# paulmillr/noble-bls12-381

Measured on AMD Instinct MI355X. Metric: pairings/sec, higher is better.
Workload: dtype int64; 1 GPU; batch of 4096 independent BLS12-381 pairings per GPU (Miller loop + final exponentiation, inputs pre-validated, bit-exact vs reference), inputs/outputs resident in HBM; batch_per_gpu=4096, batches_in_flight=12

## Files before the change

include/nbls.h:

```cpp
#ifndef NBLS_H
#define NBLS_H
#include <stddef.h>
#include <stdint.h>
#ifdef __cplusplus
extern "C" {
#endif

typedef struct nbls_ctx nbls_ctx;

#define NBLS_OK 0
#define NBLS_EINVAL (-1)
#define NBLS_EHIP (-2)
#define NBLS_ENOSUP (-3)
#define NBLS_ENOGPU (-4)
#define NBLS_EDECODE (-5)

int nbls_init(int device_id, nbls_ctx** out);
void nbls_destroy(nbls_ctx* ctx);
const char* nbls_strerror(int code);
int nbls_last_hip_error(nbls_ctx* ctx);

int nbls_pairing_batch(nbls_ctx* ctx, size_t n, const uint8_t* g1_aff, const uint8_t* g2_aff, int with_final_exp, int validate,
                       uint8_t* out_fp12, int8_t* status);
int nbls_pairing_batch_dev(nbls_ctx* ctx, size_t n, const void* d_g1_aff, const void* d_g2_aff, int with_final_exp,
// ... 184 lines not shown
typedef struct nbls_kzg_fk20 nbls_kzg_fk20;
int  nbls_kzg_fk20_create(nbls_ctx* ctx, const nbls_kzg_monomial* monomial, unsigned log2_cell, nbls_kzg_fk20** out);
void nbls_kzg_fk20_destroy(nbls_kzg_fk20* fk);
int  nbls_kzg_fk20_params(const nbls_kzg_fk20* fk, unsigned* log2_n, unsigned* log2_cell);
int  nbls_kzg_compute_cells_and_proofs_fk20(nbls_ctx* ctx, const nbls_kzg_fk20* fk, size_t n, const uint8_t* blobs, uint8_t* out_cells,
                                            uint8_t* out_proofs48 , int8_t* status );
int  nbls_kzg_recover_cells_and_proofs_fk20(nbls_ctx* ctx, const nbls_kzg_fk20* fk, size_t n, const uint32_t* cell_offsets, const uint32_t* cell_index, const uint8_t* cells,
                                            uint8_t* out_cells, uint8_t* out_proofs48 , int8_t* status );

#define NBLS_ST_G16_C 30
typedef struct nbls_groth16_vk nbls_groth16_vk;
int  nbls_groth16_vk_create(nbls_ctx* ctx, size_t m, const uint8_t* alpha_g1_48, const uint8_t* beta_g2_96, const uint8_t* gamma_g2_96, const uint8_t* delta_g2_96,
                            const uint8_t* ic48 , int8_t* status , nbls_groth16_vk** out);
void nbls_groth16_vk_destroy(nbls_groth16_vk* vk);
int  nbls_groth16_vk_inputs(const nbls_groth16_vk* vk, size_t* m);
int  nbls_groth16_verify(nbls_ctx* ctx, const nbls_groth16_vk* vk, size_t n, const uint8_t* proofs192, const uint8_t* inputs32 , const uint8_t* seed32 ,
                         int* all_ok, int8_t* status );
int  nbls_groth16_prepare_inputs(nbls_ctx* ctx, const nbls_groth16_vk* vk, size_t n, const uint8_t* inputs32, uint8_t* out48 , int8_t* status );
int  nbls_groth16_input_sums(nbls_ctx* ctx, size_t n, size_t m, const uint8_t* inputs32, const uint8_t* weights32 , const int8_t* pre ,
                             uint8_t* out32 , int8_t* status );

int nbls_verify_batch_partial_dev(nbls_ctx* ctx, size_t n, const void* d_sig96 , const void* d_uniform256, const void* d_pk48,
                                  void* d_out_fp12, int* zero_flag, int8_t* pk_status , void* stream);

int nbls_miller_product_partial(nbls_ctx* ctx, size_t n, const uint8_t* g1_aff, const uint8_t* g2_aff, int validate, void** d_partial, int8_t* status);
int nbls_verify_batch_partial(nbls_ctx* ctx, size_t n, const uint8_t* sig96 , const uint8_t* msgs, const uint32_t* offsets, const uint8_t* pk48,
                              const uint8_t* dst, size_t dst_len, void** d_partial, int* zero_flag, int8_t* pk_status );
int nbls_miller_product_partial_into(nbls_ctx* ctx, size_t n, const uint8_t* g1_aff, const uint8_t* g2_aff, int validate, void* d_dst576, int8_t* status);
int nbls_verify_batch_partial_into(nbls_ctx* ctx, size_t n, const uint8_t* sig96 , const uint8_t* msgs, const uint32_t* offsets, const uint8_t* pk48,
                                   const uint8_t* dst, size_t dst_len, void* d_dst576, int* zero_flag, int8_t* pk_status );
const char* nbls_config_describe(void);
#define NBLS_ABI_VERSION 5
int nbls_abi_version(void);
int nbls_context_device(nbls_ctx* ctx);

int nbls_hw_queues(int* set_by_library);
typedef struct nbls_pool nbls_pool;
int nbls_pool_init(int device_id, int depth , nbls_pool** out);
void nbls_pool_destroy(nbls_pool* p);
int nbls_pool_depth(const nbls_pool* p);
nbls_ctx* nbls_pool_context(nbls_pool* p, int i);
int nbls_pool_next_slot(nbls_pool* p);
int nbls_pool_pairing_batch_dev(nbls_pool* p, size_t n, const void* d_g1, const void* d_g2, int with_final_exp, void* d_out, int* slot);
int nbls_pool_synchronize(nbls_pool* p);

typedef struct nbls_multi nbls_multi;
int nbls_init_multi(int n_devices, const int* device_ids, nbls_multi** out);
void nbls_destroy_multi(nbls_multi* m);
int nbls_multi_device_count(const nbls_multi* m);
nbls_ctx* nbls_multi_context(nbls_multi* m, int i);
int nbls_multi_peer_access(const nbls_multi* m, int i);
int nbls_multi_pairing_batch(nbls_multi* m, size_t n, const uint8_t* g1_aff, const uint8_t* g2_aff, int with_final_exp, int validate,
                             uint8_t* out_fp12, int8_t* status);
int nbls_multi_miller_product(nbls_multi* m, size_t n, const uint8_t* g1_aff, const uint8_t* g2_aff, int final_exp, int validate,
                              uint8_t* out_fp12, int8_t* status);
int nbls_multi_verify_batch(nbls_multi* m, size_t n, const uint8_t* sig96, const uint8_t* msgs, const uint32_t* offsets, const uint8_t* pk48,
                            const uint8_t* dst, size_t dst_len, int* ok);

int nbls_program_stats(nbls_ctx* ctx, int prog, uint32_t* out8);
int nbls_device_synchronize(nbls_ctx* ctx);
int nbls_placement_probe(nbls_ctx* ctx, size_t n, uint64_t* out_blocks);
int nbls_field_kernel_raw(nbls_ctx* ctx, int kind, int form, size_t n, const uint8_t* in_raw, uint8_t* out_raw);
#define NBLS_N_PROGRAMS 128
#define NBLS_TUNE_SPLIT_MILLER_MIN 1
#define NBLS_TUNE_HALVES_MIN 2
#define NBLS_TUNE_EXPC_MIN 3
#define NBLS_TUNE_CHAIN_MAX 4
#define NBLS_TUNE_VERIFY_CHUNKS 5
#define NBLS_TUNE_VERIFY_LAST_PCT 6
#define NBLS_TUNE_VERIFY_PIPE_MIN 7
#define NBLS_TUNE_SAC_MAX 8
#define NBLS_TUNE_PT_LS2_MAX 9
#define NBLS_TUNE_WIDE_MAX 10
#define NBLS_TUNE_H2C_NORM_MIN 11
#define NBLS_TUNE_INV_WIDE_MAX 12
#define NBLS_TUNE_LS_MAX 13
#define NBLS_TUNE_LS2_MAX 14
#define NBLS_TUNE_POLY_SLAB 15
#define NBLS_TUNE_MSMB_WINDOW 16
#define NBLS_TUNE_MSMB_BIG 17
#define NBLS_TUNE_MSMB_SLAB 18
#define NBLS_TUNE_CELLS_CHUNK 20
#define NBLS_TUNE_G16_CHUNK 22
int nbls_set_tuning(nbls_ctx* ctx, int key, long long value);
int nbls_program_count(void);
const char* nbls_program_name(int prog);
const char* nbls_program_kernel(nbls_ctx* ctx, int prog);
const char* nbls_extra_program_kernel(nbls_ctx* ctx, const char* name);
long long nbls_extra_program_launches(nbls_ctx* ctx, const char* name);
int nbls_aot_kernel_private_bytes(int k);
int nbls_timing_enable(nbls_ctx* ctx, int on);
int nbls_timing_read(nbls_ctx* ctx, float* ms , uint32_t* counts );

#ifdef __cplusplus
}
#endif
#endif
```

noble-bls12-381_amd/csrc/aot.h:

```cpp
#pragma once
#include <string>
#include <vector>
#include "vm.h"
#include "programs.h"

#define NBLS_AOT_PARTS 8
#define NBLS_AOT_KERNELS(X)                                                  \
  X(0, expx, P_EXPX, P_FE_MID1, P_FE_MID2, P_COUNT)                          \
  X(0, acc_fe, P_ACC_FE, P_ACC_RAW, P_ACC_BYTES, P_COUNT)                    \
  X(0, lines_pq, P_LINES_PQ, P_COUNT, P_COUNT, P_COUNT)                      \
  X(0, acc4_raw, P_ACC4_RAW, P_ACC8_RAW, P_ACC2_RAW, P_COUNT)                \
  X(1, fe_easy, P_FE_EASY, P_COUNT, P_COUNT, P_COUNT)                        \
  X(1, fe_final, P_FE_FINAL, P_COUNT, P_COUNT, P_COUNT)                      \
  X(1, miller_fe, P_MILLER_FE, P_MILLER_RAW, P_MILLER_BYTES, P_COUNT)        \
  X(1, mul2, P_MUL2, P_MUL2S, P_COUNT, P_COUNT)                             \
  X(1, norm, P_NORM_RAW, P_NORM_BYTES, P_RAW_TO_BYTES, P_COUNT)              \
  X(2, h2c_a, P_H2C_A, P_COUNT, P_COUNT, P_COUNT)                            \
  X(2, h2c_b, P_H2C_B1, P_H2C_B2, P_COUNT, P_COUNT)                          \
  X(2, h2c_c1, P_H2C_C1, P_H2C_C0, P_COUNT, P_COUNT)                         \
  X(2, h2c_c2, P_H2C_C2, P_COUNT, P_COUNT, P_COUNT)                          \
  X(2, g1_dec, P_G1_DEC_A, P_G1_DEC_B, P_COUNT, P_COUNT)                     \
  X(2, g2_dec, P_G2_DEC_A, P_G2_DEC_B, P_COUNT, P_COUNT)                     \
  X(2, g2_to_affine, P_G2_TO_AFFINE, P_G2_NORM, P_G2_TO_PROJ, P_G2_ADD2)     \
  X(3, g2_mul, P_G2_MUL, P_G2_MUL_W3, P_G2_MUL_GLS, P_G2_MUL_SAC)         \
  X(3, g1_mul, P_G1_MUL, P_G1_MUL_W3, P_G1_MUL_FIXED, P_G1_MUL64)               \
  X(4, g1_validate, P_G1_VALIDATE, P_COUNT, P_COUNT, P_COUNT)                \
  X(4, g2_validate, P_G2_VALIDATE, P_COUNT, P_COUNT, P_COUNT)                \
  X(4, g1_sum, P_G1_TO_PROJ, P_G1_ADD2, P_G1_NORM, P_G1_TO_AFFINE)           \
  X(5, g1_msm, P_G1_ADD_AB, P_G1_HORNER, P_G1_SHIFTADD, P_G1_MSM_PREP)       \
  X(5, g2_msm, P_G2_ADD_AB, P_G2_HORNER, P_G2_SHIFTADD, P_G2_MSM_PREP)       \
  X(6, lines_q, P_LINES_Q, P_ACC_Q, P_LINES_BYTES, P_LINES_FROM_BYTES)       \
  X(6, miller_raw2, P_MILLER_RAW2, P_COUNT, P_COUNT, P_COUNT)                \
  X(6, g2_dec192, P_G2_DEC_A192, P_G2_DEC_B192, P_G2_DEC_B_HEX, P_G2_SWAP)   \
  X(6, from_raw, P_G1_FROM_RAW, P_G2_FROM_RAW, P_G1_COMPRESS, P_G2_COMPRESS) \
  X(7, h2c1, P_H2C1_A, P_H2C1_B, P_ENC1_A, P_ENC1_B)                         \
  X(7, g1_clear, P_G1_CLEAR, P_COUNT, P_COUNT, P_COUNT)                      \
  X(7, enc2, P_ENC2_A, P_ENC2_B, P_COUNT, P_COUNT)                            \
  X(4, h2c_n, P_H2C_NA, P_H2C_NM, P_H2C_NB, P_COUNT)

#define NBLS_AOT_LS_KERNELS(X)                                                              \
  X(7, expx_ls, P_EXPX_LS, P_COUNT, P_COUNT, P_COUNT)                                      \
  X(3, miller_ls, P_MILLER_FE_LS, P_MILLER_RAW_LS, P_MILLER_BYTES_LS, P_COUNT)

#define NBLS_AOT_LS2_KERNELS(X)                                                             \
  X(4, expx_ls2, P_EXPX_LS2, P_COUNT, P_COUNT, P_COUNT)                                    \
  X(5, miller_ls2, P_MILLER_FE_LS2, P_MILLER_RAW_LS2, P_MILLER_BYTES_LS2, P_COUNT)                    \
  X(6, g2pt_ls2, P_H2C_C1_LS2, P_H2C_C2_LS2, P_G2_MUL_SAC_LS2, P_COUNT)

#define NBLS_AOT_EXTRA_KERNELS(X)                \
  X(1, poly_g1, XP_POLY_G1_16, XP_POLY_G1_256)  \
  X(7, poly_g2, XP_POLY_G2_16, XP_POLY_G2_256)  \
  X(2, dbladd_g1, XP_DBLADD_G1, XP_COUNT)       \
  X(3, dbladd_g2, XP_DBLADD_G2, XP_COUNT)       \
  X(5, lines_fe, XP_LINES_FE, XP_COUNT)

namespace nbls {

static const uint32_t AF_MULTSH = 1;
static const uint32_t AF_MULT3 = 2;
static const uint32_t AF_OFFS = 4;
static const uint32_t AF_WRED = 8;
static const uint32_t AF_HALVE = 16;
struct AotSig { uint32_t kind, p0, flags, t, sh0, sh1; };
static inline bool operator==(const AotSig& a, const AotSig& b) { return a.kind == b.kind && a.p0 == b.p0 && a.flags == b.flags && a.t == b.t && a.sh0 == b.sh0 && a.sh1 == b.sh1; }
struct AotStep { uint32_t x, y; };
static const int AOT_DOT_HDR = 2;
static inline uint32_t aot_dot_hdr_quads(uint32_t t) { return (AOT_DOT_HDR + t + 3) / 4; }
struct AotProgram {
  std::vector<AotSig> sigs;
  std::vector<uint32_t> sig_count;
  std::vector<AotStep> steps;
  std::vector<uint32_t> descs;
  uint32_t lds_bytes = 0;
};
static const int AOT_MAX_SEGS = 8;
struct AotSeg {
  const AotStep* steps; const uint32_t* descs; const uint32_t* consts;
  uint32_t nsteps, nconst, inst_bytes, slot_bytes, shared_consts, pad;
  IOBuf bufs[MAX_BUFS];
};
struct AotArgs {
  AotSeg seg[AOT_MAX_SEGS];
  uint32_t nseg, W, G, n_items, fair, pad;
  const uint32_t* qp_table; const uint32_t* item_index; const uint32_t* n_items_dev;
};
struct AotLayout;
std::string aot_translate(const Program& p, AotProgram& out);
std::string aot_translate_with(const Program& p, AotProgram& out, const AotLayout* layout);

}

// ... 7 lines not shown
```

noble-bls12-381_amd/csrc/aot_gen.cpp:

```cpp
#include <algorithm>
#include <cstdio>
#include <cstdlib>
#include <string>
#include <vector>
#include "aot.h"
#include "aot_layout.h"
#include "config.h"
using namespace nbls;
namespace nbls { const AotLayoutEntry* aot_layout_table(size_t* n) { *n = 0; return nullptr; } }

static int gen_layout(const char* path, long iters, const std::vector<std::string>& only) {
  FILE* f = fopen(path, "w");
  if (!f) { perror(path); return 1; }
  fprintf(f, "// aot_layout.inc -- GENERATED by `aot_gen --layout` (make -C csrc layout; aot_layout.cpp: search over per-instance slot permutations against the LDS bank model); do not edit.\n");
  fprintf(f, "// AOT_LAYOUT_POS(program, place of slot s of instance g at [g * slots + s]) ; AOT_LAYOUT_ROW(program, instances, slots, steps, hash of the compiled program)\n");
  const ProgId hot[] = {P_EXPX, P_FE_MID1, P_FE_MID2, P_ACC_FE, P_ACC_RAW, P_ACC_BYTES, P_LINES_PQ, P_ACC4_RAW, P_ACC8_RAW, P_ACC2_RAW, P_FE_EASY, P_FE_FINAL, P_MILLER_FE, P_MILLER_RAW, P_MILLER_BYTES,
                        P_MUL2, P_MUL2S, P_NORM_RAW, P_NORM_BYTES, P_LINES_Q, P_ACC_Q, P_MILLER_RAW2,
                        P_H2C_A, P_H2C_B1, P_H2C_B2, P_H2C_C0, P_H2C_C1, P_H2C_C2, P_G1_DEC_B, P_G2_DEC_B, P_G1_VALIDATE, P_G2_VALIDATE, P_G2_TO_AFFINE};
  auto place = [&](const Program& p) {
    if (!only.empty() && std::find(only.begin(), only.end(), p.name) == only.end()) return;
    if (!p.shared_consts || p.slots < 2) return;
    const AotLdsCost c0 = aot_layout_cost(p, AotLayout());
    if (c0.cycles == c0.floor) return;
    const long n = std::max<long>(iters / 2, std::min<long>(iters, iters * 1000 / (long)(c0.floor / 14 + 1)));
    const AotLayout l = aot_layout_search(p, n, 0x6e626c73u);
    if (l.empty()) return;
    const AotLdsCost c1 = aot_layout_cost(p, l);
    fprintf(f, "// %s: %u instances x %u slots of %u B; LDS read cycles per wavefront %lu -> %lu (conflicts %.3f -> %.3f of them), %ld swaps tried\n", p.name.c_str(), p.G, p.slots, p.slot_bytes, c0.cycles, c1.cycles,
            (double)(c0.cycles - c0.floor) / c0.cycles, (double)(c1.cycles - c1.floor) / c1.cycles, n);
    fprintf(f, "AOT_LAYOUT_POS(%s", p.name.c_str());
    for (uint32_t g = 0; g < p.G; g++) for (uint32_t s = 0; s < p.slots; s++) fprintf(f, ", %u", (unsigned)l.pos[g][s]);
    fprintf(f, ")\nAOT_LAYOUT_ROW(%s, %u, %u, %zu, 0x%08xu)\n", p.name.c_str(), p.G, p.slots, p.steps.size(), aot_program_hash(p));
    fflush(f);
  };
  for (ProgId id : hot) place(get_program(id));
  place(get_extra_program(XP_LINES_FE));
  fclose(f);
  return 0;
}
static int gen_hist() {
  auto emit = [&](const char* kernel, const std::vector<const Program*>& progs) {
    std::vector<AotSig> sigs; std::vector<std::vector<unsigned>> cnt(progs.size());
    for (size_t q = 0; q < progs.size(); q++) {
      AotProgram ap;
      if (!aot_translate(*progs[q], ap).empty()) continue;
      for (size_t i = 0; i < ap.sigs.size(); i++) {
        size_t k = 0; while (k < sigs.size() && !(sigs[k] == ap.sigs[i])) k++;
        if (k == sigs.size()) sigs.push_back(ap.sigs[i]);
        cnt[q].resize(std::max(cnt[q].size(), k + 1), 0); cnt[q][k] += ap.sig_count[i];
      }
    }
    for (size_t q = 0; q < progs.size(); q++) {
      printf("%s %s %u %zu", kernel, progs[q]->name.c_str(), progs[q]->G, progs[q]->steps.size());
      for (size_t k = 0; k < sigs.size(); k++) printf(" %u", k < cnt[q].size() ? cnt[q][k] : 0u);
      printf("\n");
    }
  };
#define HIST(PART, NAME, P0, P1, P2, P3) { std::vector<const Program*> progs; for (ProgId id : {P0, P1, P2, P3}) if (id != P_COUNT) progs.push_back(&get_program(id)); emit(#NAME, progs); }
  NBLS_AOT_KERNELS(HIST)
#undef HIST
#define HIST(PART, NAME, E0, E1) { std::vector<const Program*> progs; for (ExtraProg id : {E0, E1}) if (id != XP_COUNT) progs.push_back(&get_extra_program(id)); emit(#NAME, progs); }
  NBLS_AOT_EXTRA_KERNELS(HIST)
#undef HIST
  return 0;
}
int main(int argc, char** argv) {
  if (argc > 2 && std::string(argv[1]) == "--layout") return gen_layout(argv[2], argc > 3 ? atol(argv[3]) : 60000, std::vector<std::string>(argv + std::min(argc, 4), argv + argc));
  if (argc > 1 && std::string(argv[1]) == "--hist") return gen_hist();
  const char* path = argc > 1 ? argv[1] : "aot_sigs.inc";
  FILE* f = fopen(path, "w");
  if (!f) { perror(path); return 1; }
  fprintf(f, "// aot_sigs.inc -- GENERATED by aot_gen (aot_gen.cpp) from the compiled step programs; do not edit.\n");
  fprintf(f, "// X(id, kind, p0, flags, t, shape[0], shape[1], steps with this signature) -- aot.h AotSig: K_DOT (12): p0 product rounds, flags AF_*, t merged post-added terms;\n");
  fprintf(f, "// K_LIN (2): p0 added, t subtracted terms; K_LOAD (0) / K_STORE (3) / K_LOADW (4) / K_STOREW (5)\n");
  int rc = 0;
  auto emit = [&](const char* kernel, const std::vector<const Program*>& progs) {
    std::vector<AotSig> sigs; std::vector<unsigned> cnt; std::string names; size_t nsteps = 0, kb = 0;
    for (const Program* pp : progs) {
      const Program& p = *pp;
      AotProgram ap;
      const std::string e = aot_translate(p, ap);
      if (!e.empty()) { fprintf(stderr, "aot_gen: %s\n", e.c_str()); rc = 1; }
      for (size_t i = 0; i < ap.sigs.size(); i++) {
        size_t k = 0; while (k < sigs.size() && !(sigs[k] == ap.sigs[i])) k++;
        if (k == sigs.size()) { sigs.push_back(ap.sigs[i]); cnt.push_back(0); }
        cnt[k] += ap.sig_count[i];
      }
      names += (names.empty() ? "" : " + ") + p.name; nsteps += p.steps.size(); kb += ap.descs.size() * 4 / 1024;
    }
    fprintf(f, "// %s: %zu steps, %zu signatures, %zu KB of descriptors\n#define AOT_SIGS_%s(X)", names.c_str(), nsteps, sigs.size(), kb, kernel);
    for (size_t k = 0; k < sigs.size(); k++)
      fprintf(f, " \\\n  X(%zu, %u, %u, 0x%02x, %u, 0x%08xu, 0x%08xu, %u)", k, sigs[k].kind, sigs[k].p0, sigs[k].flags, sigs[k].t, sigs[k].sh0, sigs[k].sh1, cnt[k]);
    fprintf(f, "\n");
  };
#define GEN(PART, NAME, P0, P1, P2, P3)                                                            \
  {                                                                                                \
    std::vector<const Program*> progs;                                                             \
    for (ProgId id : {P0, P1, P2, P3}) if (id != P_COUNT) progs.push_back(&get_program(id));       \
    emit(#NAME, progs);                                                                            \
  }
  NBLS_AOT_KERNELS(GEN)
  NBLS_AOT_LS_KERNELS(GEN)
  NBLS_AOT_LS2_KERNELS(GEN)
#undef GEN
#define GEN(PART, NAME, E0, E1)                                                                    \
  {                                                                                                \
    std::vector<const Program*> progs;                                                             \
    for (ExtraProg id : {E0, E1}) if (id != XP_COUNT) progs.push_back(&get_extra_program(id));     \
    emit(#NAME, progs);                                                                            \
  }
  NBLS_AOT_EXTRA_KERNELS(GEN)
#undef GEN
  fclose(f);
  std::string ppath = path; { size_t k = ppath.rfind("aot_sigs.inc"); if (k != std::string::npos) ppath.replace(k, 12, "aot_parts.inc"); else ppath += ".parts"; }
  f = fopen(ppath.c_str(), "w");
  if (!f) { perror(ppath.c_str()); return 1; }
  fprintf(f, "// aot_parts.inc -- GENERATED by aot_gen from NBLS_AOT_KERNELS (aot.h); do not edit.\n");
  for (int part = 0; part < NBLS_AOT_PARTS; part++) {
    fprintf(f, "#if NBLS_AOT_PART == %d\n", part);
#define PARTS(PART, NAME, P0, P1, P2, P3) if (PART == part) fprintf(f, "AOT_KERNEL_BODY(%s)\n", #NAME);
    NBLS_AOT_KERNELS(PARTS)
#undef PARTS
#define PARTS(PART, NAME, P0, P1, P2, P3) if (PART == part) fprintf(f, "AOT_KERNEL_BODY_LS(%s)\n", #NAME);
    NBLS_AOT_LS_KERNELS(PARTS)
#undef PARTS
#define PARTS(PART, NAME, P0, P1, P2, P3) if (PART == part) fprintf(f, "AOT_KERNEL_BODY_LS2(%s)\n", #NAME);
    NBLS_AOT_LS2_KERNELS(PARTS)
#undef PARTS
#define PARTS(PART, NAME, E0, E1) if (PART == part) fprintf(f, "AOT_KERNEL_BODY(%s)\n", #NAME);
    NBLS_AOT_EXTRA_KERNELS(PARTS)
#undef PARTS
    fprintf(f, "#endif\n");
  }
  fclose(f);
  return rc;
}
```

noble-bls12-381_amd/csrc/aot_kernel.hip:

```cpp
#include <hip/hip_runtime.h>
#include <atomic>
#include <mutex>
#include "aot.h"
#include "aot_exec.h"
#include "aot_sigs.inc"

namespace nbls {

struct DevDesc {
  V4 q0, q1, q2;
  const V4* blk;
  __device__ __forceinline__ V4 quad(const u32 i) const { return i == 0 ? q0 : i == 1 ? q1 : i == 2 ? q2 : blk[64 * i]; }
};

__device__ __forceinline__ u32 aot_lane() {
  u32 l;
  asm volatile("v_mbcnt_lo_u32_b32 %0, -1, 0\n\tv_mbcnt_hi_u32_b32 %0, -1, %0" : "=v"(l));
  return l;
}
template <class Dispatch>
__device__ __forceinline__ void aot_body(const AotArgs& ka, Dispatch&& dispatch) {
  extern __shared__ __attribute__((aligned(16))) char smem[];
  char* lds = smem;
  const u32 lane = threadIdx.x;
// ... 49 lines not shown
#define NBLS_AOT_PART 0
#endif
#define AOT_DECL(PART, NAME, P0, P1, P2, P3) extern "C" __global__ void nbls_aot_##NAME(AotArgs ka);
NBLS_AOT_KERNELS(AOT_DECL)
NBLS_AOT_LS_KERNELS(AOT_DECL)
NBLS_AOT_LS2_KERNELS(AOT_DECL)
#define AOT_DECL_EXTRA(PART, NAME, E0, E1) extern "C" __global__ void nbls_aot_##NAME(AotArgs ka);
NBLS_AOT_EXTRA_KERNELS(AOT_DECL_EXTRA)
#define AOT_KERNEL_BODY(NAME) AOT_KERNEL_BODY_(NAME, AOT_CASE, NBLS_AOT_OCC)
#define AOT_KERNEL_BODY_LS(NAME) AOT_KERNEL_BODY_(NAME, AOT_CASE_LS, __attribute__((amdgpu_waves_per_eu(1, 2))))
#define AOT_KERNEL_BODY_LS2(NAME) AOT_KERNEL_BODY_(NAME, AOT_CASE_LS2, __attribute__((amdgpu_waves_per_eu(1, 2))))
#define AOT_KERNEL_BODY_(NAME, CASE, OCC)                                                                                                 \
  extern "C" __global__ void __launch_bounds__(64) OCC nbls_aot_##NAME(AotArgs ka) {                                           \
    aot_body(ka, [&](u32 sig, const DevDesc& d, char* lds, u32 item, bool live, const IOBuf* bufs) __attribute__((always_inline)) { \
      switch (sig) { AOT_SIGS_##NAME(CASE) default: break; }                                                                   \
    });                                                                                                                        \
  }
#include "aot_parts.inc"

#define AOT_ROW(ID, KIND, P0, FLAGS, T, SH0, SH1, CNT) {KIND, P0, FLAGS, T, SH0, SH1},
}

#if NBLS_AOT_PART == 0
namespace nbls {
#define AOT_TABLE(PART, NAME, P0, P1, P2, P3) static const AotSig sigs_##NAME[] = {AOT_SIGS_##NAME(AOT_ROW)};
NBLS_AOT_KERNELS(AOT_TABLE)
NBLS_AOT_LS_KERNELS(AOT_TABLE)
NBLS_AOT_LS2_KERNELS(AOT_TABLE)
#define AOT_TABLE_EXTRA(PART, NAME, E0, E1) static const AotSig sigs_##NAME[] = {AOT_SIGS_##NAME(AOT_ROW)};
NBLS_AOT_EXTRA_KERNELS(AOT_TABLE_EXTRA)
struct AotKernel { int prog_id[4]; const void* fn; const AotSig* sigs; unsigned nsigs; const char* name; };
#define AOT_ENTRY(PART, NAME, P0, P1, P2, P3) {{(int)P0, (int)P1, (int)P2, (int)P3}, (const void*)nbls_aot_##NAME, sigs_##NAME, (unsigned)(sizeof(sigs_##NAME) / sizeof(AotSig)), "nbls_aot_" #NAME},
#define AOT_XP(E) ((int)E == (int)XP_COUNT ? (int)P_COUNT : (int)P_COUNT + 1 + (int)E)
#define AOT_ENTRY_EXTRA(PART, NAME, E0, E1) {{AOT_XP(E0), AOT_XP(E1), (int)P_COUNT, (int)P_COUNT}, (const void*)nbls_aot_##NAME, sigs_##NAME, (unsigned)(sizeof(sigs_##NAME) / sizeof(AotSig)), "nbls_aot_" #NAME},
static const AotKernel g_kernels[] = {NBLS_AOT_KERNELS(AOT_ENTRY) NBLS_AOT_LS_KERNELS(AOT_ENTRY) NBLS_AOT_LS2_KERNELS(AOT_ENTRY) NBLS_AOT_EXTRA_KERNELS(AOT_ENTRY_EXTRA)};
static const int g_nkernels = (int)(sizeof(g_kernels) / sizeof(g_kernels[0]));

}

extern "C" int nbls_aot_index(int prog_id) {
  if (prog_id < 0 || prog_id >= (int)nbls::P_COUNT) return -1;
  for (int k = 0; k < nbls::g_nkernels; k++) for (int j = 0; j < 4; j++) if (nbls::g_kernels[k].prog_id[j] == prog_id) return k;
  return -1;
}
extern "C" int nbls_aot_extra_index(int extra_prog) {
  if (extra_prog < 0 || extra_prog >= (int)nbls::XP_COUNT) return -1;
  for (int k = 0; k < nbls::g_nkernels; k++) for (int j = 0; j < 4; j++) if (nbls::g_kernels[k].prog_id[j] == (int)nbls::P_COUNT + 1 + extra_prog) return k;
  return -1;
}
extern "C" int nbls_aot_private_bytes(int k) {
  if (k < 0 || k >= nbls::g_nkernels) return -1;
  hipFuncAttributes a;
  if (hipFuncGetAttributes(&a, nbls::g_kernels[k].fn) != hipSuccess) { (void)hipGetLastError(); return -2; }
  return (int)a.localSizeBytes;
}
extern "C" const char* nbls_aot_name(int k) { return k >= 0 && k < nbls::g_nkernels ? nbls::g_kernels[k].name : nullptr; }
extern "C" int nbls_aot_bind(int k, nbls::AotProgram* ap) {
  using namespace nbls;
  if (k < 0 || k >= g_nkernels || !ap) return -1;
  const AotKernel& K = g_kernels[k];
  std::vector<unsigned> map(ap->sigs.size());
  for (size_t i = 0; i < ap->sigs.size(); i++) {
    unsigned id = 0;
    while (id < K.nsigs && !(K.sigs[id] == ap->sigs[i])) id++;
    if (id == K.nsigs) return -1;
    map[i] = id;
  }
  for (auto& s : ap->steps) s.x = (s.x & ~0xffu) | map[s.x & 0xffu];
  return 0;
}
extern "C" int nbls_aot_launch(int k, const nbls::AotArgs* ka, unsigned lds_bytes, void* stream) {
  using namespace nbls;
  if (k < 0 || k >= g_nkernels) return -1;
  if (ka->n_items == 0) return 0;
  const unsigned blocks = (ka->n_items + ka->G - 1) / ka->G;
  static std::atomic<bool> attr_set[64];
  static std::mutex attr_mu;
  {
    int dev = 0;
    if (hipGetDevice(&dev) != hipSuccess || dev < 0 || dev >= 64) dev = 0;
    if (!attr_set[dev].load(std::memory_order_acquire)) {
      std::lock_guard<std::mutex> g(attr_mu);
      if (!attr_set[dev].load(std::memory_order_relaxed)) {
        for (int i = 0; i < g_nkernels; i++) (void)hipFuncSetAttribute(g_kernels[i].fn, hipFuncAttributeMaxDynamicSharedMemorySize, 160 * 1024);
        attr_set[dev].store(true, std::memory_order_release);
      }
    }
  }
  AotArgs a = *ka;
  a.fair = (blocks > 1024 && blocks <= 4096) ? 1u : 0u;
  void* args[] = {&a};
  const hipError_t e = hipLaunchKernel(g_kernels[k].fn, dim3(blocks), dim3(64), args, lds_bytes, (hipStream_t)stream);
  return e == hipSuccess ? (int)hipGetLastError() : (int)e;
}
#endif
```

noble-bls12-381_amd/csrc/aot_layout.inc:

```
AOT_LAYOUT_POS(expx, 10, 17, 29, 4, 3, 14, 6, 19, 5, 12, 11, 18, 24, 7, 9, 16, 26, 23, 22, 21, 0, 28, 1, 13, 8, 27, 2, 25, 15, 20, 1, 13, 26, 25, 17, 10, 23, 18, 9, 15, 3, 24, 29, 4, 22, 6, 21, 19, 2, 12, 0, 11, 7, 16, 8, 27, 14, 20, 28, 5, 24, 12, 6, 3, 8, 21, 16, 17, 4, 9, 18, 14, 1, 0, 10, 19, 22, 13, 27, 29, 23, 28, 26, 15, 25, 7, 5, 2, 11, 20, 29, 0, 5, 4, 11, 22, 24, 7, 12, 14, 9, 10, 23, 19, 2, 1, 13, 16, 8, 6, 15, 25, 18, 27, 17, 20, 28, 26, 21, 3, 16, 14, 25, 10, 19, 5, 22, 3, 18, 15, 20, 27, 11, 23, 13, 12, 0, 6, 24, 28, 2, 9, 21, 7, 4, 26, 1, 17, 8, 29)
AOT_LAYOUT_ROW(expx, 5, 30, 97, 0x7173e202u)
AOT_LAYOUT_POS(fe_mid1, 12, 24, 3, 26, 35, 6, 15, 9, 22, 31, 25, 16, 20, 17, 8, 5, 29, 7, 34, 14, 28, 23, 2, 33, 10, 27, 1, 19, 18, 0, 13, 21, 30, 11, 32, 4, 2, 23, 32, 30, 24, 17, 29, 6, 1, 12, 11, 19, 7, 14, 21, 10, 0, 22, 28, 13, 25, 20, 16, 3, 31, 33, 8, 26, 34, 27, 35, 15, 9, 4, 18, 5, 6, 4, 26, 13, 9, 31, 12, 14, 23, 28, 22, 17, 2, 35, 27, 24, 19, 33, 25, 16, 3, 34, 1, 20, 30, 8, 11, 21, 0, 5, 32, 10, 15, 29, 7, 18, 6, 2, 14, 4, 28, 21, 13, 10, 26, 23, 9, 32, 20, 25, 19, 0, 18, 30, 16, 31, 8, 12, 35, 29, 33, 27, 7, 22, 24, 5, 1, 11, 15, 3, 34, 17, 8, 17, 26, 27, 23, 34, 32, 0, 13, 7, 31, 33, 9, 22, 21, 15, 25, 3, 11, 6, 5, 29, 4, 2, 16, 10, 14, 19, 35, 12, 18, 28, 20, 30, 1, 24)
AOT_LAYOUT_ROW(fe_mid1, 5, 36, 11, 0x4d52c8d6u)
AOT_LAYOUT_POS(fe_mid2, 4, 2, 3, 13, 10, 7, 9, 11, 24, 26, 25, 21, 1, 27, 20, 14, 19, 18, 8, 32, 29, 6, 16, 35, 31, 22, 30, 12, 28, 33, 23, 5, 0, 34, 15, 17, 11, 29, 17, 4, 21, 12, 10, 34, 3, 32, 35, 14, 2, 0, 27, 25, 20, 28, 6, 23, 8, 26, 19, 5, 15, 16, 31, 1, 9, 30, 7, 24, 33, 13, 22, 18, 11, 33, 22, 3, 8, 13, 24, 12, 9, 15, 2, 28, 20, 34, 5, 31, 18, 25, 17, 26, 6, 7, 1, 32, 23, 21, 16, 10, 19, 27, 0, 14, 30, 35, 29, 4, 5, 27, 22, 0, 25, 23, 4, 2, 3, 34, 10, 20, 35, 33, 12, 26, 28, 7, 16, 19, 17, 32, 24, 15, 11, 29, 31, 13, 30, 8, 6, 1, 21, 18, 14, 9, 31, 2, 19, 21, 12, 20, 9, 7, 4, 25, 17, 10, 5, 14, 30, 16, 22, 13, 11, 0, 26, 6, 34, 29, 3, 18, 33, 8, 35, 15, 1, 28, 23, 32, 24, 27)
AOT_LAYOUT_ROW(fe_mid2, 5, 36, 11, 0x62a97a64u)
AOT_LAYOUT_POS(acc_fe, 22, 8, 3, 10, 20, 15, 0, 13, 18, 12, 14, 11, 9, 2, 16, 19, 7, 6, 5, 4, 1, 21, 23, 17, 18, 22, 15, 9, 17, 11, 20, 10, 5, 8, 0, 12, 14, 13, 3, 7, 2, 16, 19, 1, 4, 21, 6, 23, 0, 3, 8, 15, 11, 17, 23, 21, 5, 7, 6, 9, 4, 13, 12, 14, 1, 20, 2, 22, 16, 18, 10, 19, 16, 2, 18, 4, 11, 17, 6, 23, 10, 12, 9, 3, 8, 13, 14, 15, 0, 21, 19, 5, 20, 7, 22, 1, 12, 20, 11, 0, 18, 21, 6, 7, 9, 14, 13, 19, 2, 17, 3, 15, 10, 16, 5, 1, 22, 23, 4, 8)
AOT_LAYOUT_ROW(acc_fe, 5, 24, 173, 0xd36919acu)
AOT_LAYOUT_POS(acc_raw, 10, 1, 4, 13, 3, 22, 20, 21, 5, 12, 8, 0, 17, 7, 16, 2, 11, 6, 14, 9, 19, 18, 23, 15, 7, 1, 23, 6, 3, 0, 8, 21, 15, 9, 10, 22, 11, 13, 14, 16, 18, 17, 20, 19, 12, 2, 4, 5, 19, 18, 5, 10, 17, 2, 12, 7, 9, 20, 22, 23, 11, 4, 14, 13, 3, 15, 16, 1, 6, 8, 0, 21, 0, 21, 5, 9, 20, 8, 6, 1, 10, 14, 23, 4, 13, 17, 12, 15, 16, 3, 2, 11, 19, 7, 22, 18, 20, 11, 16, 8, 5, 10, 22, 15, 7, 14, 3, 21, 12, 0, 6, 19, 1, 2, 17, 18, 4, 9, 23, 13)
AOT_LAYOUT_ROW(acc_raw, 5, 24, 166, 0xd41b21c8u)
AOT_LAYOUT_POS(acc_bytes, 10, 1, 4, 13, 3, 22, 20, 21, 5, 12, 8, 0, 17, 7, 16, 2, 11, 6, 14, 9, 19, 18, 23, 15, 7, 1, 23, 6, 3, 0, 8, 21, 15, 9, 10, 22, 11, 13, 14, 16, 18, 17, 20, 19, 12, 2, 4, 5, 19, 18, 5, 10, 17, 2, 12, 7, 9, 20, 22, 23, 11, 4, 14, 13, 3, 15, 16, 1, 6, 8, 0, 21, 0, 21, 5, 9, 20, 8, 6, 1, 10, 14, 23, 4, 13, 17, 12, 15, 16, 3, 2, 11, 19, 7, 22, 18, 20, 11, 16, 8, 5, 10, 22, 15, 7, 14, 3, 21, 12, 0, 6, 19, 1, 2, 17, 18, 4, 9, 23, 13)
AOT_LAYOUT_ROW(acc_bytes, 5, 24, 167, 0x04619a33u)
AOT_LAYOUT_POS(lines_pq, 16, 2, 17, 24, 8, 14, 22, 6, 11, 9, 10, 23, 5, 21, 19, 3, 25, 0, 20, 18, 13, 1, 15, 12, 7, 4, 16, 15, 13, 3, 14, 23, 11, 2, 0, 25, 8, 17, 20, 10, 19, 4, 21, 1, 12, 5, 9, 18, 6, 7, 22, 24, 16, 1, 20, 8, 4, 25, 6, 9, 3, 11, 5, 12, 24, 23, 13, 2, 14, 19, 15, 0, 10, 21, 18, 17, 7, 22, 13, 22, 21, 10, 24, 5, 18, 9, 8, 20, 16, 19, 15, 25, 14, 2, 12, 1, 7, 3, 23, 0, 6, 4, 11, 17, 2, 17, 6, 16, 0, 10, 19, 7, 23, 25, 21, 11, 20, 13, 22, 14, 12, 1, 24, 4, 3, 5, 8, 9, 18, 15, 3, 20, 21, 0, 22, 15, 19, 6, 5, 17, 10, 16, 12, 25, 11, 13, 23, 18, 9, 1, 14, 24, 7, 8, 2, 4)
AOT_LAYOUT_ROW(lines_pq, 6, 26, 307, 0x7c311802u)
AOT_LAYOUT_POS(acc4_raw, 23, 0, 18, 10, 27, 6, 8, 11, 22, 25, 5, 19, 4, 16, 14, 28, 13, 15, 9, 2, 20, 7, 1, 21, 17, 26, 24, 29, 3, 12, 16, 24, 5, 18, 3, 11, 7, 14, 2, 25, 28, 13, 19, 12, 1, 20, 10, 9, 17, 0, 8, 21, 15, 6, 23, 29, 27, 4, 22, 26, 13, 17, 2, 6, 4, 19, 7, 22, 8, 28, 11, 14, 9, 15, 23, 29, 10, 5, 16, 25, 1, 12, 24, 21, 18, 20, 0, 26, 27, 3, 1, 7, 16, 10, 14, 9, 5, 28, 25, 6, 0, 27, 19, 29, 17, 12, 22, 2, 26, 21, 4, 24, 15, 3, 13, 23, 11, 20, 8, 18, 29, 12, 7, 1, 5, 15, 10, 6, 21, 13, 18, 2, 16, 25, 4, 22, 26, 0, 9, 19, 24, 20, 14, 8, 27, 28, 3, 17, 23, 11)
AOT_LAYOUT_ROW(acc4_raw, 5, 30, 472, 0xa9d029e3u)
AOT_LAYOUT_POS(acc8_raw, 1, 13, 4, 12, 0, 5, 22, 11, 8, 21, 16, 10, 15, 17, 14, 23, 2, 3, 9, 6, 19, 18, 20, 7, 20, 17, 1, 3, 4, 7, 22, 0, 15, 2, 14, 9, 12, 13, 5, 18, 11, 10, 21, 23, 19, 6, 16, 8, 10, 19, 13, 14, 18, 20, 21, 23, 3, 0, 2, 6, 16, 9, 12, 8, 22, 17, 7, 4, 1, 5, 15, 11, 19, 16, 6, 14, 9, 1, 5, 7, 18, 4, 23, 2, 11, 12, 10, 15, 13, 8, 0, 3, 17, 21, 22, 20, 19, 18, 9, 7, 4, 21, 6, 14, 20, 5, 8, 10, 11, 13, 16, 15, 17, 2, 0, 3, 12, 22, 23, 1)
AOT_LAYOUT_ROW(acc8_raw, 5, 24, 879, 0x655d1f0bu)
AOT_LAYOUT_POS(acc2_raw, 10, 1, 2, 12, 4, 11, 6, 14, 23, 13, 20, 3, 7, 5, 17, 0, 19, 21, 18, 15, 8, 16, 22, 9, 5, 0, 16, 23, 17, 4, 8, 7, 11, 1, 22, 15, 12, 14, 10, 2, 3, 9, 6, 20, 18, 21, 13, 19, 4, 18, 17, 0, 13, 23, 5, 19, 21, 22, 10, 11, 12, 15, 9, 8, 14, 2, 1, 3, 20, 6, 16, 7, 22, 21, 18, 17, 11, 9, 16, 23, 7, 0, 10, 4, 3, 12, 13, 15, 20, 2, 8, 1, 5, 6, 14, 19, 9, 20, 7, 12, 11, 21, 6, 16, 13, 14, 4, 3, 22, 0, 18, 10, 19, 1, 5, 15, 23, 8, 2, 17)
AOT_LAYOUT_ROW(acc2_raw, 5, 24, 267, 0xb30cd74du)
AOT_LAYOUT_POS(fe_easy, 10, 1, 36, 18, 38, 37, 12, 6, 29, 40, 9, 14, 24, 25, 33, 8, 11, 20, 22, 39, 2, 35, 15, 23, 3, 16, 41, 19, 21, 0, 26, 4, 5, 28, 30, 27, 13, 32, 31, 17, 34, 7, 5, 2, 31, 33, 6, 17, 32, 26, 25, 15, 10, 39, 12, 37, 23, 8, 13, 38, 29, 14, 0, 20, 9, 11, 27, 1, 22, 30, 16, 40, 3, 35, 34, 24, 19, 21, 41, 36, 7, 4, 18, 28, 19, 32, 35, 33, 10, 40, 15, 29, 25, 6, 24, 5, 1, 37, 8, 18, 7, 17, 41, 23, 22, 14, 11, 39, 31, 20, 36, 27, 12, 9, 26, 2, 16, 13, 34, 3, 28, 4, 38, 0, 21, 30, 31, 28, 10, 24, 34, 4, 27, 39, 32, 38, 3, 2, 20, 5, 40, 29, 1, 25, 21, 16, 30, 15, 19, 37, 41, 14, 8, 22, 0, 35, 33, 6, 12, 18, 11, 26, 9, 7, 23, 36, 13, 17)
AOT_LAYOUT_ROW(fe_easy, 4, 42, 24, 0x4d06dc2eu)
AOT_LAYOUT_POS(fe_final, 21, 38, 36, 13, 42, 16, 40, 22, 46, 14, 26, 7, 37, 8, 17, 18, 9, 28, 0, 10, 35, 33, 34, 15, 31, 4, 45, 24, 5, 19, 3, 39, 44, 25, 12, 29, 47, 41, 20, 27, 43, 11, 32, 1, 2, 6, 30, 23, 43, 23, 21, 26, 24, 31, 1, 33, 7, 39, 13, 12, 47, 29, 46, 15, 40, 10, 6, 44, 16, 14, 11, 9, 2, 18, 36, 34, 3, 45, 41, 4, 17, 37, 22, 38, 32, 27, 5, 30, 8, 25, 42, 28, 19, 20, 35, 0, 6, 5, 38, 8, 11, 22, 3, 23, 16, 24, 44, 21, 14, 27, 15, 12, 7, 47, 43, 25, 10, 4, 32, 30, 36, 31, 42, 9, 0, 26, 18, 13, 1, 34, 19, 40, 33, 20, 2, 17, 41, 46, 37, 35, 28, 29, 45, 39, 33, 8, 21, 41, 14, 45, 38, 2, 13, 39, 6, 4, 43, 5, 10, 9, 12, 22, 46, 15, 28, 47, 34, 36, 26, 0, 11, 31, 19, 35, 17, 24, 29, 40, 32, 18, 44, 23, 1, 25, 3, 16, 7, 20, 27, 42, 30, 37, 44, 31, 11, 35, 7, 12, 4, 17, 15, 30, 13, 47, 0, 26, 36, 34, 45, 29, 16, 8, 21, 14, 33, 39, 43, 18, 24, 46, 37, 42, 28, 3, 1, 9, 41, 23, 27, 2, 6, 32, 40, 22, 5, 25, 10, 19, 38, 20)
AOT_LAYOUT_ROW(fe_final, 5, 48, 59, 0x73c61872u)
AOT_LAYOUT_POS(miller_fe, 32, 33, 19, 8, 7, 37, 5, 29, 24, 6, 14, 22, 4, 16, 36, 27, 26, 25, 0, 23, 20, 2, 28, 13, 3, 12, 34, 11, 9, 30, 1, 31, 18, 10, 17, 35, 15, 21, 12, 37, 16, 30, 17, 6, 33, 11, 14, 9, 29, 25, 34, 32, 2, 23, 3, 20, 28, 1, 18, 19, 15, 5, 24, 31, 26, 7, 36, 13, 21, 27, 10, 35, 4, 8, 0, 22, 32, 6, 18, 19, 27, 37, 17, 10, 12, 13, 20, 24, 28, 8, 4, 30, 23, 35, 22, 11, 0, 1, 16, 36, 25, 2, 29, 26, 31, 15, 33, 9, 5, 14, 7, 3, 34, 21, 25, 3, 30, 37, 21, 34, 5, 29, 8, 12, 10, 15, 24, 31, 28, 6, 36, 17, 19, 20, 0, 9, 7, 4, 16, 23, 26, 14, 27, 11, 18, 32, 33, 22, 13, 1, 35, 2)
AOT_LAYOUT_ROW(miller_fe, 4, 38, 349, 0xd1b982e6u)
AOT_LAYOUT_POS(miller_raw, 32, 27, 36, 26, 7, 28, 23, 18, 2, 19, 25, 24, 16, 33, 30, 4, 21, 10, 37, 35, 0, 31, 9, 11, 12, 8, 1, 14, 29, 6, 34, 15, 3, 5, 13, 22, 20, 17, 11, 0, 3, 31, 17, 34, 18, 23, 7, 35, 21, 9, 30, 29, 14, 8, 16, 32, 27, 1, 36, 13, 6, 24, 19, 22, 26, 15, 28, 37, 33, 2, 4, 25, 12, 20, 10, 5, 28, 34, 16, 33, 27, 0, 3, 24, 30, 22, 18, 19, 26, 4, 10, 14, 13, 25, 5, 11, 17, 36, 6, 2, 1, 32, 20, 8, 7, 15, 31, 37, 21, 29, 23, 35, 9, 12, 32, 3, 36, 17, 5, 9, 37, 33, 20, 34, 10, 14, 8, 22, 35, 4, 15, 1, 30, 21, 19, 31, 26, 23, 29, 25, 16, 7, 6, 12, 2, 13, 0, 24, 18, 11, 27, 28)
AOT_LAYOUT_ROW(miller_raw, 4, 38, 342, 0x07887de8u)
AOT_LAYOUT_POS(miller_bytes, 26, 1, 6, 35, 7, 5, 36, 21, 34, 32, 37, 31, 28, 3, 33, 4, 29, 15, 25, 23, 16, 12, 22, 14, 8, 27, 10, 9, 20, 13, 2, 19, 11, 17, 18, 24, 0, 30, 26, 3, 18, 21, 1, 5, 33, 16, 14, 36, 19, 31, 11, 30, 22, 28, 8, 34, 32, 17, 20, 27, 35, 23, 25, 15, 10, 0, 12, 24, 2, 37, 29, 6, 13, 9, 4, 7, 1, 37, 25, 7, 11, 28, 3, 22, 29, 9, 24, 35, 32, 13, 26, 34, 15, 17, 4, 27, 20, 16, 8, 5, 36, 18, 0, 6, 14, 31, 23, 12, 10, 19, 30, 33, 2, 21, 10, 34, 20, 14, 5, 28, 37, 24, 8, 2, 35, 16, 17, 4, 15, 33, 27, 32, 22, 21, 31, 13, 3, 9, 6, 25, 29, 11, 7, 1, 12, 30, 18, 26, 23, 0, 19, 36)
AOT_LAYOUT_ROW(miller_bytes, 4, 38, 343, 0x27bc5877u)
AOT_LAYOUT_POS(fp12_mul2, 2, 25, 30, 6, 28, 10, 11, 29, 32, 5, 35, 12, 16, 21, 4, 26, 0, 13, 22, 15, 18, 14, 9, 33, 27, 1, 7, 24, 34, 19, 3, 20, 8, 31, 17, 23, 7, 29, 20, 27, 14, 12, 23, 15, 18, 0, 19, 30, 3, 1, 6, 16, 25, 35, 31, 11, 8, 4, 13, 21, 10, 33, 5, 34, 24, 32, 28, 26, 2, 22, 17, 9, 35, 12, 15, 32, 7, 31, 19, 1, 30, 13, 25, 27, 9, 18, 0, 23, 24, 33, 29, 5, 10, 4, 22, 34, 6, 14, 2, 20, 11, 16, 17, 8, 3, 21, 28, 26, 15, 4, 32, 0, 8, 1, 31, 3, 7, 22, 30, 5, 11, 23, 35, 12, 13, 20, 33, 25, 24, 6, 26, 2, 17, 29, 34, 14, 28, 27, 16, 18, 9, 21, 10, 19)
AOT_LAYOUT_ROW(fp12_mul2, 4, 36, 9, 0x431cfebau)
AOT_LAYOUT_POS(fp12_mul2s, 2, 25, 30, 6, 28, 10, 11, 29, 32, 5, 35, 12, 16, 21, 4, 26, 0, 13, 22, 15, 18, 14, 9, 33, 27, 1, 7, 24, 34, 19, 3, 20, 8, 31, 17, 23, 7, 29, 20, 27, 14, 12, 23, 15, 18, 0, 19, 30, 3, 1, 6, 16, 25, 35, 31, 11, 8, 4, 13, 21, 10, 33, 5, 34, 24, 32, 28, 26, 2, 22, 17, 9, 35, 12, 15, 32, 7, 31, 19, 1, 30, 13, 25, 27, 9, 18, 0, 23, 24, 33, 29, 5, 10, 4, 22, 34, 6, 14, 2, 20, 11, 16, 17, 8, 3, 21, 28, 26, 15, 4, 32, 0, 8, 1, 31, 3, 7, 22, 30, 5, 11, 23, 35, 12, 13, 20, 33, 25, 24, 6, 26, 2, 17, 29, 34, 14, 28, 27, 16, 18, 9, 21, 10, 19)
AOT_LAYOUT_ROW(fp12_mul2s, 4, 36, 9, 0xf99001aau)
AOT_LAYOUT_POS(norm_raw, 6, 0, 5, 11, 8, 10, 1, 3, 9, 2, 7, 4, 7, 5, 11, 8, 10, 4, 9, 2, 3, 1, 0, 6, 2, 1, 10, 3, 0, 7, 11, 6, 9, 8, 4, 5, 10, 4, 0, 9, 5, 6, 3, 1, 2, 11, 8, 7)
AOT_LAYOUT_ROW(norm_raw, 4, 12, 8, 0x663d5f87u)
AOT_LAYOUT_POS(norm_bytes, 2, 9, 11, 1, 3, 8, 10, 0, 7, 5, 6, 4, 2, 8, 3, 4, 11, 9, 10, 5, 1, 7, 6, 0, 1, 10, 8, 11, 7, 2, 3, 9, 5, 0, 6, 4, 11, 3, 4, 0, 5, 9, 10, 2, 6, 1, 7, 8)
AOT_LAYOUT_ROW(norm_bytes, 4, 12, 10, 0x4c284411u)
AOT_LAYOUT_POS(lines_q, 17, 5, 6, 18, 15, 19, 16, 22, 3, 9, 13, 7, 1, 11, 23, 20, 2, 21, 4, 12, 8, 14, 10, 0, 16, 8, 11, 0, 10, 2, 23, 13, 3, 9, 20, 19, 17, 14, 1, 18, 6, 5, 22, 21, 12, 4, 7, 15, 2, 8, 1, 0, 22, 14, 7, 15, 10, 4, 20, 16, 18, 21, 11, 3, 17, 12, 9, 19, 23, 13, 5, 6, 6, 16, 17, 4, 20, 13, 22, 18, 8, 10, 23, 21, 7, 15, 12, 1, 14, 9, 19, 2, 5, 0, 11, 3, 16, 21, 8, 1, 14, 4, 6, 18, 19, 20, 10, 22, 0, 17, 9, 13, 7, 23, 15, 12, 11, 3, 2, 5, 0, 22, 21, 16, 15, 19, 8, 4, 17, 2, 10, 1, 3, 13, 14, 20, 6, 5, 11, 12, 7, 18, 23, 9)
AOT_LAYOUT_ROW(lines_q, 6, 24, 310, 0xc51c7bb5u)
AOT_LAYOUT_POS(acc_q, 5, 10, 26, 18, 8, 6, 14, 22, 11, 28, 2, 12, 15, 20, 17, 3, 9, 27, 16, 31, 7, 4, 25, 13, 23, 30, 21, 24, 1, 0, 29, 19, 26, 27, 0, 9, 4, 1, 29, 8, 5, 15, 25, 23, 11, 21, 24, 14, 18, 3, 12, 7, 28, 16, 19, 2, 10, 6, 13, 22, 31, 20, 17, 30, 2, 10, 24, 17, 0, 13, 3, 26, 4, 7, 1, 31, 12, 16, 6, 9, 29, 30, 20, 21, 15, 5, 14, 11, 25, 19, 27, 23, 28, 18, 22, 8, 26, 10, 29, 14, 20, 23, 18, 31, 22, 24, 28, 13, 11, 3, 8, 30, 15, 19, 17, 9, 12, 1, 4, 16, 5, 0, 7, 25, 27, 6, 2, 21, 10, 26, 12, 11, 8, 16, 1, 23, 25, 5, 20, 14, 30, 22, 9, 18, 28, 2, 27, 6, 29, 7, 21, 3, 31, 24, 0, 17, 4, 13, 19, 15)
AOT_LAYOUT_ROW(acc_q, 5, 32, 202, 0xff0ad85bu)
AOT_LAYOUT_POS(miller_raw2, 18, 29, 19, 48, 44, 31, 11, 7, 67, 3, 58, 60, 51, 56, 33, 2, 8, 66, 42, 9, 4, 23, 6, 43, 50, 39, 54, 49, 53, 45, 25, 59, 28, 5, 26, 14, 55, 41, 16, 27, 30, 65, 68, 17, 47, 52, 36, 38, 15, 61, 10, 63, 24, 0, 12, 62, 35, 20, 34, 57, 40, 21, 64, 13, 32, 1, 22, 46, 37, 66, 35, 22, 57, 42, 54, 60, 62, 26, 46, 28, 44, 2, 40, 18, 27, 36, 10, 39, 11, 64, 25, 8, 59, 0, 29, 16, 55, 67, 65, 31, 9, 38, 61, 24, 68, 37, 45, 33, 51, 19, 7, 21, 63, 15, 41, 4, 50, 53, 23, 56, 49, 48, 34, 1, 3, 58, 20, 14, 43, 32, 5, 12, 17, 13, 47, 52, 6, 30, 29, 54, 49, 58, 2, 17, 9, 61, 53, 25, 44, 59, 5, 68, 8, 19, 14, 31, 57, 30, 60, 11, 20, 24, 32, 56, 23, 34, 3, 55, 0, 10, 38, 43, 18, 63, 27, 51, 35, 48, 26, 41, 50, 6, 13, 45, 64, 15, 36, 33, 40, 47, 39, 4, 62, 7, 37, 52, 21, 28, 46, 65, 42, 67, 16, 12, 22, 66, 1, 35, 64, 28, 48, 18, 20, 52, 44, 16, 24, 58, 41, 56, 26, 42, 29, 4, 63, 13, 40, 21, 67, 6, 2, 9, 34, 43, 23, 57, 19, 66, 0, 32, 15, 36, 31, 27, 55, 7, 49, 12, 53, 22, 60, 61, 33, 50, 51, 10, 65, 14, 11, 45, 62, 8, 39, 38, 5, 37, 46, 54, 17, 3, 59, 25, 1, 30, 68, 47)
AOT_LAYOUT_ROW(miller_raw2, 4, 69, 536, 0x0a10926cu)
AOT_LAYOUT_POS(h2c_a, 23, 10, 21, 7, 8, 5, 14, 24, 1, 19, 27, 16, 3, 18, 6, 26, 15, 0, 12, 2, 17, 22, 20, 11, 4, 9, 13, 25, 1, 16, 12, 8, 13, 25, 18, 5, 6, 22, 24, 14, 9, 3, 15, 21, 20, 17, 0, 11, 7, 23, 10, 2, 27, 4, 19, 26, 19, 13, 26, 7, 12, 15, 1, 6, 0, 23, 2, 3, 11, 18, 17, 16, 22, 14, 27, 9, 20, 4, 21, 5, 25, 10, 8, 24, 22, 0, 4, 13, 9, 18, 5, 23, 6, 10, 17, 15, 3, 12, 7, 11, 1, 21, 27, 16, 19, 25, 26, 20, 8, 24, 14, 2, 27, 20, 12, 22, 16, 23, 13, 9, 25, 17, 1, 19, 15, 3, 11, 2, 26, 24, 14, 8, 4, 5, 21, 6, 7, 10, 0, 18, 16, 5, 21, 1, 20, 11, 4, 6, 10, 27, 12, 2, 19, 23, 0, 8, 3, 22, 24, 13, 7, 26, 18, 9, 15, 25, 14, 17, 15, 2, 10, 7, 14, 21, 18, 8, 13, 26, 1, 23, 9, 5, 19, 16, 0, 25, 11, 3, 20, 27, 17, 12, 6, 24, 4, 22, 5, 18, 9, 11, 8, 22, 20, 10, 6, 23, 2, 16, 13, 0, 14, 21, 15, 1, 7, 4, 19, 27, 26, 12, 3, 24, 25, 17)
AOT_LAYOUT_ROW(h2c_a, 8, 28, 24, 0x9b31d2b6u)
AOT_LAYOUT_POS(h2c_b1, 24, 3, 7, 2, 14, 21, 23, 0, 13, 11, 8, 4, 27, 15, 5, 18, 20, 1, 25, 26, 19, 12, 6, 17, 16, 22, 9, 10, 2, 5, 20, 1, 21, 9, 13, 25, 16, 22, 27, 15, 24, 12, 4, 10, 17, 8, 14, 0, 3, 23, 26, 18, 7, 11, 19, 6, 24, 23, 3, 6, 20, 7, 4, 2, 11, 13, 12, 17, 10, 21, 15, 27, 8, 19, 0, 26, 5, 25, 14, 16, 1, 9, 18, 22, 23, 4, 9, 12, 5, 27, 2, 3, 18, 26, 21, 17, 8, 22, 6, 1, 13, 19, 11, 25, 20, 24, 10, 0, 7, 15, 16, 14, 15, 24, 9, 23, 16, 7, 8, 3, 18, 14, 12, 13, 5, 1, 22, 19, 20, 25, 4, 2, 0, 21, 27, 10, 17, 11, 6, 26, 7, 12, 11, 8, 9, 13, 24, 15, 27, 3, 1, 17, 10, 2, 21, 22, 0, 25, 5, 14, 23, 19, 26, 20, 16, 6, 4, 18, 13, 1, 25, 6, 0, 14, 26, 24, 5, 18, 19, 10, 8, 23, 27, 20, 9, 12, 16, 4, 21, 3, 2, 17, 11, 15, 7, 22, 13, 26, 23, 6, 14, 21, 9, 5, 4, 1, 3, 15, 24, 0, 12, 22, 25, 27, 2, 16, 19, 7, 10, 11, 8, 17, 20, 18)
AOT_LAYOUT_ROW(h2c_b1, 8, 28, 50, 0x13589acbu)
AOT_LAYOUT_POS(h2c_b2, 2, 1, 6, 19, 8, 4, 7, 18, 15, 17, 14, 16, 10, 5, 9, 3, 0, 13, 11, 12, 2, 11, 4, 14, 16, 19, 10, 9, 17, 6, 0, 18, 3, 5, 7, 1, 13, 12, 8, 15, 9, 16, 3, 13, 5, 6, 7, 4, 19, 1, 10, 15, 18, 2, 12, 0, 11, 14, 17, 8, 5, 11, 0, 16, 19, 13, 1, 4, 17, 6, 3, 15, 7, 8, 18, 14, 12, 2, 10, 9, 13, 14, 12, 11, 1, 3, 17, 10, 18, 9, 6, 7, 4, 5, 2, 15, 8, 16, 19, 0, 1, 14, 18, 11, 15, 8, 6, 13, 7, 9, 4, 2, 5, 3, 12, 17, 19, 0, 10, 16, 1, 3, 12, 4, 10, 9, 7, 8, 17, 18, 19, 13, 6, 0, 14, 15, 2, 11, 16, 5, 1, 19, 17, 14, 18, 0, 7, 16, 15, 4, 8, 10, 6, 11, 3, 12, 5, 9, 13, 2)
AOT_LAYOUT_ROW(h2c_b2, 8, 20, 16, 0x42647d7fu)
AOT_LAYOUT_POS(h2c_c0, 20, 8, 18, 19, 22, 12, 4, 14, 13, 17, 1, 7, 5, 23, 9, 6, 10, 21, 16, 3, 2, 15, 0, 11, 17, 18, 21, 20, 19, 8, 22, 23, 11, 16, 13, 0, 2, 9, 5, 6, 1, 10, 3, 12, 15, 14, 4, 7, 19, 11, 3, 5, 9, 7, 13, 12, 17, 23, 15, 6, 8, 16, 10, 20, 22, 1, 18, 2, 14, 0, 21, 4, 6, 9, 4, 13, 12, 11, 17, 23, 22, 15, 3, 21, 0, 10, 16, 19, 8, 7, 5, 14, 2, 20, 1, 18, 1, 13, 9, 0, 12, 19, 11, 8, 15, 6, 17, 4, 16, 5, 7, 2, 3, 14, 20, 18, 22, 10, 23, 21, 16, 1, 13, 19, 3, 0, 2, 15, 9, 7, 21, 11, 22, 8, 4, 12, 14, 6, 5, 23, 18, 10, 17, 20, 3, 18, 16, 9, 17, 19, 5, 0, 7, 8, 4, 6, 21, 11, 2, 14, 20, 13, 22, 12, 10, 1, 15, 23, 10, 11, 3, 22, 18, 20, 9, 5, 21, 16, 19, 6, 2, 15, 13, 12, 4, 0, 23, 17, 14, 7, 1, 8)
AOT_LAYOUT_ROW(h2c_c0, 8, 24, 19, 0x8dd6efe9u)
AOT_LAYOUT_POS(h2c_c1, 5, 18, 17, 3, 6, 4, 1, 12, 8, 11, 7, 10, 16, 14, 9, 0, 19, 2, 15, 13, 11, 16, 19, 18, 0, 3, 8, 10, 14, 9, 17, 7, 5, 4, 13, 15, 2, 12, 1, 6, 8, 7, 16, 5, 4, 0, 3, 17, 13, 10, 14, 12, 2, 11, 15, 18, 1, 19, 6, 9, 14, 5, 18, 10, 17, 0, 6, 3, 7, 4, 8, 1, 15, 13, 2, 11, 12, 9, 16, 19, 5, 16, 15, 6, 18, 8, 19, 12, 1, 13, 14, 10, 7, 17, 3, 2, 9, 0, 4, 11, 12, 7, 4, 10, 5, 19, 16, 18, 15, 11, 9, 8, 0, 6, 17, 13, 2, 3, 1, 14, 11, 2, 5, 19, 16, 8, 13, 3, 10, 4, 0, 1, 9, 15, 18, 12, 7, 6, 14, 17, 6, 1, 2, 17, 12, 4, 14, 13, 8, 18, 11, 19, 10, 15, 0, 7, 16, 9, 3, 5)
AOT_LAYOUT_ROW(h2c_c1, 8, 20, 230, 0x09f22878u)
AOT_LAYOUT_POS(h2c_c2, 4, 12, 9, 3, 7, 13, 8, 1, 14, 19, 11, 10, 18, 2, 17, 16, 5, 0, 15, 6, 3, 19, 10, 8, 1, 13, 2, 14, 17, 6, 9, 11, 5, 16, 0, 7, 18, 15, 4, 12, 13, 1, 19, 9, 15, 0, 11, 8, 12, 17, 16, 6, 4, 5, 18, 14, 3, 2, 10, 7, 18, 10, 4, 14, 17, 2, 9, 3, 15, 0, 6, 12, 11, 7, 19, 5, 8, 13, 1, 16, 12, 1, 13, 2, 15, 5, 9, 6, 7, 4, 17, 10, 11, 3, 0, 8, 16, 14, 18, 19, 18, 14, 3, 11, 2, 13, 16, 17, 12, 9, 8, 6, 10, 0, 15, 5, 1, 7, 19, 4, 4, 16, 17, 9, 8, 19, 10, 7, 6, 3, 14, 0, 12, 18, 1, 15, 11, 13, 5, 2, 14, 7, 15, 4, 9, 13, 19, 12, 5, 6, 11, 3, 17, 0, 18, 10, 2, 16, 8, 1)
AOT_LAYOUT_ROW(h2c_c2, 8, 20, 236, 0x89ef5217u)
AOT_LAYOUT_POS(g1_dec_b, 0, 1, 2, 3, 4, 5, 6, 7, 8, 9, 10, 11, 12, 13, 14, 0, 1, 2, 3, 4, 5, 6, 7, 8, 9, 10, 11, 12, 13, 14, 0, 1, 2, 3, 4, 5, 6, 7, 8, 9, 10, 11, 12, 13, 14, 0, 1, 2, 3, 4, 5, 6, 7, 8, 9, 10, 11, 12, 13, 14, 0, 1, 2, 3, 4, 5, 6, 7, 8, 9, 10, 11, 12, 13, 14, 0, 1, 2, 3, 4, 5, 6, 7, 8, 9, 10, 11, 12, 13, 14, 0, 1, 2, 3, 4, 5, 6, 7, 8, 9, 10, 11, 12, 13, 14, 0, 1, 2, 3, 4, 5, 6, 7, 8, 9, 10, 11, 12, 13, 14, 0, 1, 2, 3, 4, 5, 6, 7, 8, 9, 10, 11, 12, 13, 14, 0, 1, 2, 3, 4, 5, 6, 7, 8, 9, 10, 11, 12, 13, 14, 0, 1, 2, 3, 4, 5, 6, 7, 8, 9, 10, 11, 12, 13, 14, 0, 1, 2, 3, 4, 5, 6, 7, 8, 9, 10, 11, 12, 13, 14, 0, 1, 2, 3, 4, 5, 6, 7, 8, 9, 10, 11, 12, 13, 14, 0, 1, 2, 3, 4, 5, 6, 7, 8, 9, 10, 11, 12, 13, 14, 0, 1, 2, 3, 4, 5, 6, 7, 8, 9, 10, 11, 12, 13, 14, 0, 1, 2, 3, 4, 5, 6, 7, 8, 9, 10, 11, 12, 13, 14)
AOT_LAYOUT_ROW(g1_dec_b, 16, 15, 450, 0xb824faddu)
AOT_LAYOUT_POS(g2_dec_b, 22, 21, 24, 3, 12, 13, 11, 15, 2, 7, 16, 4, 19, 20, 6, 0, 1, 17, 14, 23, 8, 10, 18, 9, 5, 12, 17, 2, 14, 24, 16, 7, 1, 23, 3, 6, 13, 21, 4, 11, 15, 22, 18, 20, 19, 10, 9, 8, 5, 0, 22, 21, 0, 7, 18, 1, 13, 23, 24, 19, 20, 17, 11, 2, 15, 14, 8, 4, 6, 3, 12, 5, 10, 9, 16, 16, 4, 10, 7, 20, 17, 9, 6, 21, 3, 14, 22, 1, 23, 12, 5, 11, 15, 24, 19, 18, 2, 0, 13, 8, 16, 5, 10, 3, 1, 2, 15, 6, 13, 14, 18, 7, 23, 21, 0, 24, 9, 22, 12, 17, 20, 4, 19, 11, 8, 20, 18, 6, 23, 14, 9, 3, 17, 12, 11, 2, 5, 1, 19, 22, 7, 0, 10, 8, 15, 24, 13, 4, 21, 16, 8, 2, 14, 13, 10, 1, 11, 21, 22, 9, 7, 15, 3, 5, 12, 18, 6, 4, 0, 17, 24, 19, 20, 23, 16, 20, 3, 10, 19, 9, 21, 14, 24, 7, 22, 6, 15, 11, 17, 18, 5, 4, 13, 12, 23, 16, 8, 2, 1, 0)
AOT_LAYOUT_ROW(g2_dec_b, 8, 25, 269, 0xbafec16du)
AOT_LAYOUT_POS(g1_validate, 0, 1, 2, 3, 4, 5, 6, 7, 8, 9, 10, 11, 12, 0, 1, 2, 3, 4, 5, 6, 7, 8, 9, 10, 11, 12, 0, 1, 2, 3, 4, 5, 6, 7, 8, 9, 10, 11, 12, 0, 1, 2, 3, 4, 5, 6, 7, 8, 9, 10, 11, 12, 0, 1, 2, 3, 4, 5, 6, 7, 8, 9, 10, 11, 12, 0, 1, 2, 3, 4, 5, 6, 7, 8, 9, 10, 11, 12, 0, 1, 2, 3, 4, 5, 6, 7, 8, 9, 10, 11, 12, 0, 1, 2, 3, 4, 5, 6, 7, 8, 9, 10, 11, 12, 0, 1, 2, 3, 4, 5, 6, 7, 8, 9, 10, 11, 12, 0, 1, 2, 3, 4, 5, 6, 7, 8, 9, 10, 11, 12, 0, 1, 2, 3, 4, 5, 6, 7, 8, 9, 10, 11, 12, 0, 1, 2, 3, 4, 5, 6, 7, 8, 9, 10, 11, 12, 0, 1, 2, 3, 4, 5, 6, 7, 8, 9, 10, 11, 12, 0, 1, 2, 3, 4, 5, 6, 7, 8, 9, 10, 11, 12, 0, 1, 2, 3, 4, 5, 6, 7, 8, 9, 10, 11, 12, 0, 1, 2, 3, 4, 5, 6, 7, 8, 9, 10, 11, 12)
AOT_LAYOUT_ROW(g1_validate, 16, 13, 436, 0xec0c0236u)
AOT_LAYOUT_POS(g2_validate, 16, 3, 10, 8, 18, 14, 7, 5, 19, 20, 21, 11, 22, 13, 6, 15, 1, 0, 9, 4, 12, 17, 2, 23, 20, 4, 1, 2, 5, 16, 21, 17, 22, 7, 12, 15, 8, 19, 3, 6, 18, 23, 14, 13, 10, 0, 11, 9, 1, 23, 14, 21, 0, 15, 6, 20, 5, 13, 19, 17, 10, 16, 12, 22, 3, 4, 2, 7, 9, 11, 8, 18, 9, 20, 13, 19, 3, 5, 8, 11, 4, 7, 22, 12, 10, 14, 21, 6, 2, 17, 23, 0, 15, 18, 1, 16, 20, 13, 11, 10, 16, 1, 5, 6, 21, 12, 17, 15, 22, 0, 4, 8, 23, 3, 9, 18, 14, 19, 7, 2, 4, 18, 12, 20, 2, 15, 9, 3, 8, 10, 19, 6, 22, 13, 23, 14, 1, 21, 5, 11, 7, 17, 0, 16, 7, 1, 19, 15, 13, 10, 8, 4, 3, 9, 12, 20, 14, 23, 18, 11, 2, 16, 5, 6, 0, 22, 17, 21, 21, 18, 0, 1, 17, 8, 3, 13, 6, 23, 20, 11, 7, 19, 5, 2, 14, 10, 12, 4, 9, 16, 22, 15)
AOT_LAYOUT_ROW(g2_validate, 8, 24, 230, 0x9f57251au)
AOT_LAYOUT_POS(g2_to_affine, 0, 1, 5, 6, 7, 2, 4, 3, 0, 2, 7, 3, 6, 1, 5, 4, 4, 3, 2, 7, 6, 1, 5, 0, 7, 1, 6, 5, 2, 0, 3, 4, 4, 7, 1, 2, 0, 5, 3, 6, 1, 0, 6, 7, 5, 2, 3, 4, 3, 2, 4, 0, 5, 6, 7, 1, 3, 5, 2, 1, 7, 0, 6, 4)
AOT_LAYOUT_ROW(g2_to_affine, 8, 8, 9, 0xfdb5a3b2u)
AOT_LAYOUT_POS(lines_fe, 4, 7, 3, 15, 20, 0, 14, 23, 12, 25, 6, 11, 19, 13, 22, 17, 1, 9, 2, 21, 5, 18, 8, 10, 24, 16, 21, 22, 11, 4, 20, 25, 12, 5, 8, 0, 10, 24, 23, 13, 1, 15, 16, 7, 18, 19, 6, 17, 3, 2, 14, 9, 18, 9, 12, 16, 3, 11, 20, 0, 23, 13, 10, 8, 21, 2, 14, 6, 5, 22, 7, 19, 25, 15, 17, 4, 24, 1, 7, 3, 20, 8, 1, 19, 5, 22, 15, 25, 17, 21, 2, 13, 9, 14, 16, 0, 18, 12, 4, 11, 24, 23, 10, 6, 6, 19, 23, 5, 14, 21, 4, 7, 24, 22, 12, 13, 10, 11, 3, 9, 17, 15, 18, 8, 20, 2, 25, 16, 0, 1, 23, 1, 14, 18, 2, 16, 12, 20, 24, 25, 4, 7, 10, 21, 17, 0, 19, 9, 11, 5, 15, 3, 6, 22, 8, 13)
AOT_LAYOUT_ROW(lines_fe, 6, 26, 286, 0x5d3bf329u)
```

noble-bls12-381_amd/csrc/aot_sigs.inc:

```
#define AOT_SIGS_expx(X) \
  X(0, 4, 0, 0x00, 0, 0x00000000u, 0x00000000u, 10) \
  X(1, 12, 1, 0x00, 0, 0x00000000u, 0x00000000u, 1) \
  X(2, 2, 2, 0x00, 0, 0x00000000u, 0x00000000u, 11) \
  X(3, 12, 3, 0x04, 1, 0x000a0a0bu, 0x00000000u, 2) \
  X(4, 12, 6, 0x04, 0, 0x020a0a0au, 0x00000002u, 5) \
  X(5, 2, 3, 0x08, 1, 0x00000000u, 0x00000000u, 5) \
  X(6, 12, 3, 0x04, 1, 0x000a0a0au, 0x00000000u, 7) \
  X(7, 12, 3, 0x0c, 1, 0x000a0a0bu, 0x00000000u, 61) \
  X(8, 12, 1, 0x04, 0, 0x00000002u, 0x00000000u, 1) \
  X(9, 5, 0, 0x00, 0, 0x00000000u, 0x00000000u, 5) \
  X(10, 12, 2, 0x0e, 1, 0x00000a0bu, 0x00000000u, 2) \
  X(11, 12, 6, 0x0e, 1, 0x020a0a0au, 0x00000202u, 1) \
  X(12, 2, 2, 0x00, 1, 0x00000000u, 0x00000000u, 1) \
  X(13, 12, 6, 0x04, 1, 0x020a0a0au, 0x00000002u, 2) \
  X(14, 2, 3, 0x00, 1, 0x00000000u, 0x00000000u, 2) \
  X(15, 2, 2, 0x08, 0, 0x00000000u, 0x00000000u, 2) \
  X(16, 12, 6, 0x0e, 1, 0x020a0a0au, 0x00000002u, 1)
#define AOT_SIGS_acc_fe(X) \
  X(0, 4, 0, 0x00, 0, 0x00000000u, 0x00000000u, 105) \
  X(1, 12, 5, 0x04, 0, 0x020a0a0au, 0x00000000u, 3) \
  X(2, 12, 7, 0x04, 0, 0x2a2a2f2fu, 0x000a2a2au, 186) \
  X(3, 12, 6, 0x04, 0, 0x020a0a0au, 0x00000002u, 198) \
  X(4, 2, 1, 0x00, 1, 0x00000000u, 0x00000000u, 3) \
  X(5, 12, 8, 0x04, 0, 0x2a2a2a2fu, 0x052a2a2au, 1) \
  X(6, 5, 0, 0x00, 0, 0x00000000u, 0x00000000u, 3) \
  X(7, 12, 1, 0x04, 1, 0x0000000au, 0x00000000u, 1) \
  X(8, 12, 5, 0x04, 0, 0x010a0a0au, 0x00000000u, 1) \
  X(9, 12, 8, 0x04, 0, 0x02020202u, 0x00000002u, 1) \
  X(10, 12, 2, 0x04, 1, 0x00000202u, 0x00000000u, 1) \
  X(11, 12, 2, 0x00, 0, 0x00000000u, 0x00000000u, 1) \
  X(12, 12, 1, 0x00, 0, 0x00000000u, 0x00000000u, 1) \
  X(13, 3, 0, 0x00, 0, 0x00000000u, 0x00000000u, 1)
#define AOT_SIGS_lines_pq(X) \
  X(0, 0, 0, 0x00, 0, 0x00000000u, 0x00000000u, 1) \
  X(1, 2, 2, 0x00, 0, 0x00000000u, 0x00000000u, 6) \
  X(2, 12, 1, 0x06, 0, 0x0000000au, 0x00000000u, 1) \
  X(3, 2, 3, 0x00, 0, 0x00000000u, 0x00000000u, 1) \
  X(4, 12, 2, 0x06, 0, 0x0000000au, 0x00000000u, 6) \
  X(5, 2, 4, 0x18, 3, 0x00000000u, 0x00000000u, 62) \
  X(6, 12, 2, 0x04, 0, 0x0000010au, 0x00000000u, 1) \
  X(7, 5, 0, 0x00, 0, 0x00000000u, 0x00000000u, 69) \
  X(8, 2, 1, 0x10, 0, 0x00000000u, 0x00000000u, 5) \
  X(9, 12, 2, 0x04, 1, 0x00000202u, 0x00000000u, 5) \
  X(10, 2, 1, 0x00, 1, 0x00000000u, 0x00000000u, 5) \
  X(11, 12, 4, 0x04, 0, 0x0000020au, 0x00000000u, 5) \
  X(12, 12, 2, 0x04, 0, 0x00000002u, 0x00000000u, 5) \
  X(13, 12, 2, 0x04, 2, 0x00000002u, 0x00000000u, 5) \
  X(14, 12, 4, 0x06, 0, 0x02020a0au, 0x00000000u, 5) \
  X(15, 2, 4, 0x08, 3, 0x00000000u, 0x00000000u, 5) \
  X(16, 12, 2, 0x04, 0, 0x00000a0au, 0x00000000u, 61) \
  X(17, 12, 2, 0x06, 0, 0x00000a0au, 0x00000000u, 57) \
  X(18, 2, 2, 0x08, 1, 0x00000000u, 0x00000000u, 1) \
  X(19, 12, 1, 0x04, 0, 0x00000002u, 0x00000000u, 1)
#define AOT_SIGS_acc4_raw(X) \
  X(0, 4, 0, 0x00, 0, 0x00000000u, 0x00000000u, 477) \
  X(1, 12, 5, 0x04, 0, 0x020a0a0au, 0x00000000u, 3) \
  X(2, 12, 6, 0x04, 0, 0x020a0a0au, 0x00000002u, 946) \
  X(3, 12, 7, 0x04, 0, 0x2a2a2f2fu, 0x000a2a2au, 186) \
  X(4, 2, 1, 0x00, 1, 0x00000000u, 0x00000000u, 3) \
  X(5, 5, 0, 0x00, 0, 0x00000000u, 0x00000000u, 3)
#define AOT_SIGS_fe_easy(X) \
  X(0, 4, 0, 0x00, 0, 0x00000000u, 0x00000000u, 1) \
  X(1, 12, 2, 0x0c, 1, 0x00000002u, 0x00000000u, 1) \
  X(2, 12, 8, 0x04, 0, 0x2a2a2a2fu, 0x052a2a2au, 1) \
  X(3, 12, 1, 0x04, 1, 0x0000000au, 0x00000000u, 1) \
  X(4, 12, 5, 0x04, 0, 0x010a0a0au, 0x00000000u, 1) \
  X(5, 12, 8, 0x04, 0, 0x02020202u, 0x00000002u, 1) \
  X(6, 12, 2, 0x04, 1, 0x00000202u, 0x00000000u, 1) \
  X(7, 12, 1, 0x04, 0, 0x00000002u, 0x00000000u, 1) \
  X(8, 12, 2, 0x04, 0, 0x00000002u, 0x00000000u, 2) \
  X(9, 12, 6, 0x04, 0, 0x020a0a0au, 0x00000202u, 1) \
  X(10, 2, 2, 0x00, 0, 0x00000000u, 0x00000000u, 3) \
  X(11, 12, 6, 0x04, 0, 0x020a0a0au, 0x00000002u, 1) \
  X(12, 2, 3, 0x00, 1, 0x00000000u, 0x00000000u, 2) \
  X(13, 12, 3, 0x04, 1, 0x000a0a0au, 0x00000000u, 2) \
  X(14, 12, 1, 0x00, 1, 0x00000000u, 0x00000000u, 1) \
  X(15, 12, 6, 0x04, 0, 0x0002020au, 0x00000000u, 1) \
  X(16, 5, 0, 0x00, 0, 0x00000000u, 0x00000000u, 2) \
  X(17, 2, 2, 0x08, 0, 0x00000000u, 0x00000000u, 1)
#define AOT_SIGS_fe_final(X) \
  X(0, 4, 0, 0x00, 0, 0x00000000u, 0x00000000u, 9) \
  X(1, 12, 6, 0x04, 0, 0x020a0a0au, 0x00000002u, 6) \
  X(2, 2, 2, 0x00, 0, 0x00000000u, 0x00000000u, 11) \
  X(3, 12, 3, 0x04, 1, 0x000a0a0au, 0x00000000u, 8) \
  X(4, 2, 3, 0x00, 1, 0x00000000u, 0x00000000u, 7) \
  X(5, 2, 2, 0x00, 1, 0x00000000u, 0x00000000u, 4) \
  X(6, 12, 2, 0x04, 0, 0x00000002u, 0x00000000u, 6) \
  X(7, 12, 6, 0x04, 0, 0x020a0a0au, 0x00000202u, 2) \
  X(8, 2, 3, 0x08, 1, 0x00000000u, 0x00000000u, 1) \
  X(9, 2, 1, 0x00, 1, 0x00000000u, 0x00000000u, 1) \
  X(10, 12, 1, 0x04, 0, 0x00000002u, 0x00000000u, 1) \
  X(11, 12, 1, 0x00, 0, 0x00000000u, 0x00000000u, 2) \
  X(12, 3, 0, 0x00, 0, 0x00000000u, 0x00000000u, 1)
#define AOT_SIGS_miller_fe(X) \
  X(0, 0, 0, 0x00, 0, 0x00000000u, 0x00000000u, 3) \
  X(1, 12, 1, 0x00, 0, 0x00000000u, 0x00000000u, 4) \
  X(2, 2, 3, 0x00, 1, 0x00000000u, 0x00000000u, 3) \
  X(3, 12, 2, 0x16, 1, 0x0000090au, 0x00000000u, 3) \
  X(4, 12, 2, 0x04, 1, 0x0000000au, 0x00000000u, 15) \
  X(5, 12, 2, 0x04, 1, 0x00000202u, 0x00000000u, 3) \
// ... 764 lines not shown
```

noble-bls12-381_amd/csrc/config.h:

```cpp
#pragma once
#include <string>
namespace nbls {
long env_long(const char* name, long dflt);
bool env_set(const char* name);
std::string env_describe();
}
```

noble-bls12-381_amd/csrc/nbls_internal.h:

```cpp
#pragma once
#include <hip/hip_runtime.h>
#include "config.h"
#include <cstdio>
#include <cstring>
#include <mutex>
#include <vector>
#include <initializer_list>
#include <new>
#include "nbls.h"
#include "programs.h"
#include "consts_gen.h"
#include "fp_inv.h"
#include "pow_exec.h"
#include "sha256.h"
#include "curve.h"
#include "bufs.h"
#include "verifier_frame.h"
#include <thread>

#include "launchers.h"
#include "wide_exec.h"
#include "aot.h"
#include <map>
#include <tuple>
// ... 76 lines not shown
static_assert(!(slot_bit(SB_VB_PAIRS) & MSM_MAIN.mask()), "verifyBatch keeps its pairs across the calls of its two-stage route: dev_msm on the main slots must not regrow them");
static_assert(!(M_THR_OWN & (DEC_MAIN.mask() | M_LADDER)), "combine_pipeline: the decoder and the ladder regrow their own slots between the stages that read the shares and the coefficients");
static_assert(!(M_POLY_OWN & DEC_MAIN.mask()), "poly_pipeline: the decoder regrows its own slots while the staged coefficients and the decoded points are held");
static_assert(!((M_POLY_OWN & ~slot_bit(SB_STAGED)) & (M_THR_OWN | M_RLC_MAIN | M_RLC_SIDE | M_RLC_SIDE2 | M_VB_MAIN | M_LADDER | MSM_MAIN.mask())),
              "poly_pipeline keeps to slots of its own: no other chain's buffers are regrown or overwritten by it");
static_assert(!(M_MSMB_OWN & (MSM_MAIN.mask() | M_POLY_OWN | M_THR_OWN | M_RLC_MAIN | M_RLC_SIDE | M_RLC_SIDE2 | M_VB_MAIN | M_LADDER)),
              "msm_batch_pipeline: its big groups run through dev_msm on the main slots between its slabs, which must regrow nothing the call still holds");
static_assert(!(M_KZG_OWN & (DEC_MAIN.mask() | MSM_RLC.mask() | M_LADDER)), "kzg_pipeline: the decoder, the MSMs (on the slots of MSM_RLC: MSM_MAIN holds SB_STAGED) and the ladders of the per-item pass regrow their slots while the call holds its own");
static_assert(!((M_KZG_OWN & ~slot_bit(SB_STAGED)) & (M_MSMB_OWN | M_POLY_OWN | M_THR_OWN | M_RLC_MAIN | M_RLC_SIDE | M_RLC_SIDE2 | M_VB_MAIN | MSM_MAIN.mask())), "kzg_pipeline keeps to slots of its own");
static_assert(!(M_KZGP_OWN & (M_MSMB_OWN | DEC_MAIN.mask())), "kzg_prove_pipeline: the batched MSM sizes its two slots while the staged blobs and the quotient rows are held; nbls_kzg_setup_create decodes on the main slots");
static_assert(!((M_KZGP_OWN & ~slot_bit(SB_STAGED)) & (M_KZG_OWN | M_POLY_OWN | M_THR_OWN | M_RLC_MAIN | M_RLC_SIDE | M_RLC_SIDE2 | M_VB_MAIN | M_LADDER | MSM_MAIN.mask() | MSM_RLC.mask())),
              "kzg_prove_pipeline keeps to slots of its own");
static_assert(!(M_KZGC_OWN & (M_MSMB_OWN | DEC_MAIN.mask())), "cells_pipeline: the batched MSM runs chunk after chunk while the staged blobs, the coefficients and the results are held; nbls_kzg_monomial_create decodes on the main slots");
static_assert(!((M_KZGC_OWN & ~slot_bit(SB_STAGED)) & (M_KZGP_OWN | M_KZG_OWN | M_POLY_OWN | M_THR_OWN | M_RLC_MAIN | M_RLC_SIDE | M_RLC_SIDE2 | M_VB_MAIN | M_LADDER | MSM_MAIN.mask() | MSM_RLC.mask())),
              "cells_pipeline keeps to slots of its own");
static_assert(!(M_KZGR_OWN & (M_MSMB_OWN | DEC_MAIN.mask())), "the recovery front end of cells_pipeline: as cells_pipeline, whose chunks it runs");
static_assert(!(slot_bit(SB_KZGR_Z) & (M_KZGC_OWN | M_KZGV_OWN | M_KZGP_OWN | M_KZG_OWN | M_POLY_OWN | M_THR_OWN | M_RLC_MAIN | M_RLC_SIDE | M_RLC_SIDE2 | M_VB_MAIN | M_LADDER | MSM_MAIN.mask() | MSM_RLC.mask())),
              "the recovery front end keeps to a slot of its own");
static_assert(!(M_KZGF_OWN & (M_MSMB_OWN | DEC_MAIN.mask())), "the FK20 proofs loop: both passes run on the batched MSM's two slots, chunk after chunk, while the scalars of pass A and the points of pass B are held");
static_assert(!(slots(SB_KZGF_SCALARS, SB_KZGF_POINTS) & (M_KZGR_OWN | M_KZGV_OWN | M_KZGP_OWN | M_KZG_OWN | M_POLY_OWN | M_THR_OWN | M_RLC_MAIN | M_RLC_SIDE | M_RLC_SIDE2 | M_VB_MAIN | M_LADDER | MSM_MAIN.mask() | MSM_RLC.mask())),
              "the FK20 proofs loop keeps to slots of its own");
static_assert(!(M_KZGV_OWN & (DEC_MAIN.mask() | MSM_RLC.mask() | M_LADDER | M_MSMB_OWN)),
              "verify_cells_pipeline: the decoder, the MSMs (on the slots of MSM_RLC: MSM_MAIN holds SB_STAGED), the batched MSM and the ladder of the per-cell pass regrow their slots while the call holds the staged block and its own");
static_assert(!((M_KZGV_OWN & ~slot_bit(SB_STAGED)) & (M_KZGC_OWN | M_KZGP_OWN | M_KZG_OWN | M_POLY_OWN | M_THR_OWN | M_RLC_MAIN | M_RLC_SIDE | M_RLC_SIDE2 | M_VB_MAIN | MSM_MAIN.mask())),
              "verify_cells_pipeline keeps to slots of its own");
constexpr SlotMask M_G16_OWN = slots(SB_STAGED, SB_G16_POINTS, SB_G16_SCALARS, SB_G16_PAIRS, SB_G16_OUT, SB_G16_ITEMS);
static_assert(!(M_G16_OWN & (DEC_MAIN.mask() | MSM_RLC.mask() | M_LADDER | M_MSMB_OWN)),
              "groth16_pipeline: the decoders, the MSMs (on the slots of MSM_RLC: MSM_MAIN holds SB_STAGED), the ladder and the batched MSM of the per-proof pass regrow their slots while the call holds the staged block and its own");
static_assert(!((M_G16_OWN & ~slot_bit(SB_STAGED)) & (M_KZGV_OWN | M_KZGF_OWN | M_KZGR_OWN | M_KZGC_OWN | M_KZGP_OWN | M_KZG_OWN | M_POLY_OWN | M_THR_OWN | M_RLC_MAIN | M_RLC_SIDE | M_RLC_SIDE2 | M_VB_MAIN | MSM_MAIN.mask())),
              "groth16_pipeline keeps to slots of its own");
#define EXPORT extern "C" __attribute__((visibility("default")))
extern std::recursive_mutex g_null_mu;

static const size_t EXPC_MIN_DEFAULT = (size_t)1 << 40;
struct DevProgram {
  Step* steps = nullptr; u32* descs = nullptr; u32* consts = nullptr;
  const Program* p = nullptr;
  bool wide_ok = false;
  int aot = -1; AotStep* aot_steps = nullptr; u32* aot_descs = nullptr; u32 aot_lds = 0;
  mutable unsigned long long launches = 0;
};

size_t ls_max();
size_t ls2_max();
struct nbls_ctx {
  int device = 0;
  hipStream_t stream = nullptr;
  std::recursive_mutex mu;
  DevProgram prog[P_COUNT];
  std::vector<uint8_t> dst_host; uint8_t* dst_dev = nullptr;
  std::map<std::tuple<int, int, int, int>, DevProgram> tower;
  DevProgram extra[XP_COUNT];
  size_t poly_slab = 0;
  size_t msmb_window = 0, msmb_big = 0, msmb_slab = 0;
  size_t cells_chunk = 0;
  size_t g16_chunk = 0;
  uint8_t *F = nullptr, *N = nullptr, *NI = nullptr, *io_g1 = nullptr, *io_g2 = nullptr, *io_f12 = nullptr, *one12 = nullptr;
  uint8_t* T[7] = {nullptr, nullptr, nullptr, nullptr, nullptr, nullptr, nullptr};
  uint8_t* sb[NSB] = {nullptr}; size_t sb_cap[NSB] = {0};
  struct IoBlock { void* p; size_t cap; bool busy; }; std::vector<IoBlock> io_pool; size_t io_pool_bytes = 0;
  uint8_t* nib[4] = {nullptr, nullptr, nullptr, nullptr}; int nnib[4] = {0, 0, 0, 0};
  uint8_t* neg_g1 = nullptr;
  uint8_t* gen_g1 = nullptr;
  uint8_t* g1_fixed = nullptr;
  hipStream_t side = nullptr; hipEvent_t ev_fork = nullptr, ev_join = nullptr; uint8_t* side_scratch = nullptr;
  hipStream_t half_stream = nullptr; hipEvent_t ev_half_fork = nullptr, ev_half_join = nullptr;
  size_t halves_min = env_long("NBLS_HALVES_MIN", 16384) > 0 ? (size_t)env_long("NBLS_HALVES_MIN", 16384) : (size_t)-1;
  std::vector<hipEvent_t> pipe_ev; hipEvent_t ev_pipe_done = nullptr; std::vector<hipStream_t> pipe_streams;
  long verify_chunks = env_long("NBLS_VERIFY_CHUNKS", 2), verify_last_pct = env_long("NBLS_VERIFY_LAST_PCT", 25), verify_pipe_min = env_long("NBLS_VERIFY_PIPE_MIN", 32768);
  hipStream_t side2 = nullptr; hipEvent_t ev_join2 = nullptr;
  uint8_t* ident_g1 = nullptr; uint8_t* ident_g2 = nullptr;
  size_t cap_F = 0, cap_io = 0;
  size_t split_min = SPLIT_MILLER_MIN;
  size_t acc8_min = (size_t)env_long("NBLS_ACC8_MIN", (long)1 << 40);
  uint8_t *KS = nullptr, *KD = nullptr, *Kflag = nullptr; uint32_t *Klist = nullptr, *Kcount = nullptr;
  size_t expc_min = (size_t)env_long("NBLS_EXPC_MIN", (long)EXPC_MIN_DEFAULT);
  size_t pt_ls2_max = (size_t)env_long("NBLS_PT_LS2_MAX", 4096);
  size_t sac_max = (size_t)env_long("NBLS_G2_SAC_MAX", 6144);
  size_t wide_max = (size_t)env_long("NBLS_WIDE_MAX", 0);
  size_t h2c_norm_min = (size_t)env_long("NBLS_H2C_NORM_MIN", 32768);
  size_t inv_wide_max = (size_t)env_long("NBLS_INV_WIDE_MAX", 4096);
  size_t ls_max = ::ls_max(), ls2_max = ::ls2_max();
  size_t chain_max = (size_t)env_long("NBLS_CHAIN_MAX", 8192);
  u32* qp_table = nullptr;
  uint8_t* kzg_tables[26 + 13 * 7] = {nullptr};
  uint8_t* unit_lines = nullptr;
  uint8_t* partial = nullptr;
  uint8_t* L = nullptr; size_t cap_L = 0;
  hipStream_t last_stream = nullptr; hipEvent_t ev_last = nullptr; bool ev_last_set = false;
  uint8_t* pinned_out = nullptr; size_t pinned_out_cap = 0;
  uint8_t* pinned = nullptr; size_t pinned_cap = 0;
  int last_hip = 0;
  bool timing = false;
  std::vector<std::pair<int, std::pair<hipEvent_t, hipEvent_t>>> tev;
  std::vector<hipEvent_t> ev_pool;
};

#define HIPCHK(call) do { hipError_t e_ = (call); if (e_ != hipSuccess) { ctx->last_hip = (int)e_; return NBLS_EHIP; } } while (0)
#define LAUNCHCHK(call) do { int e_ = (call); if (e_) { ctx->last_hip = e_; return NBLS_EHIP; } } while (0)

struct StreamOrder {
  nbls_ctx* ctx; hipStream_t s;
  StreamOrder(nbls_ctx* c, hipStream_t st) : ctx(c), s(st) {
    if (!ctx->ev_last) hipEventCreateWithFlags(&ctx->ev_last, hipEventDisableTiming);
    if (ctx->ev_last && ctx->ev_last_set && ctx->last_stream != s) hipStreamWaitEvent(s, ctx->ev_last, 0);
  }
  ~StreamOrder() { if (ctx->ev_last && hipEventRecord(ctx->ev_last, s) == hipSuccess) { ctx->ev_last_set = true; ctx->last_stream = s; } }
};

struct ForkGuard {
  bool armed = true; void* keys = nullptr; size_t key_bytes = 0;
  ~ForkGuard() { if (armed) { (void)hipDeviceSynchronize(); if (keys) (void)hipMemset(keys, 0, key_bytes); } }
};
struct Window {
  size_t first = 0;
  int half = 0;
  bool beside = false;
};
struct HostIO {
  nbls_ctx* ctx; std::vector<size_t> mine; hipStream_t s = nullptr; std::vector<std::pair<void*, size_t>> secrets; bool wiped = false;
  ~HostIO() {
    if (!mine.empty()) (void)hipStreamSynchronize(s ? s : ctx->stream);
    if (!wiped) for (auto& k : secrets) (void)hipMemset(k.first, 0, k.second);
    for (size_t i : mine) ctx->io_pool[i].busy = false;
  }
  void secret(void* p, size_t n) { if (p && n) secrets.push_back({p, n}); }
  int wipe(hipStream_t st) { for (auto& k : secrets) if (hipMemsetAsync(k.first, 0, k.second, st) != hipSuccess) return NBLS_EHIP; wiped = true; return NBLS_OK; }
  void* alloc(size_t n) {
    if (!n) n = 1;
    auto& pool = ctx->io_pool;
    size_t best = (size_t)-1;
    for (size_t i = 0; i < pool.size(); i++)
      if (!pool[i].busy && pool[i].p && pool[i].cap >= n && pool[i].cap / 4 <= n && (best == (size_t)-1 || pool[i].cap < pool[best].cap)) best = i;
    if (best != (size_t)-1) { pool[best].busy = true; mine.push_back(best); return pool[best].p; }
    static const size_t cap_bytes = (size_t)env_long("NBLS_IO_POOL_MB", 1024) << 20;
    const size_t cap = n + n / 8 + 256;
    for (size_t i = 0; i < pool.size() && ctx->io_pool_bytes + cap > cap_bytes; i++)
      if (!pool[i].busy && pool[i].p) { hipFree(pool[i].p); ctx->io_pool_bytes -= pool[i].cap; pool[i].p = nullptr; pool[i].cap = 0; }
    void* p = nullptr;
    if (hipMalloc(&p, cap) != hipSuccess) { (void)hipGetLastError(); return nullptr; }
    ctx->io_pool_bytes += cap;
    size_t slot = (size_t)-1;
    for (size_t i = 0; i < pool.size(); i++) if (!pool[i].p) { slot = i; break; }
    if (slot == (size_t)-1) { pool.push_back({nullptr, 0, false}); slot = pool.size() - 1; }
    pool[slot] = {p, cap, true};
    mine.push_back(slot);
    return p;
  }
};
#define LOCKED(ctx) std::lock_guard<std::recursive_mutex> g_((ctx)->mu); HIPCHK(hipSetDevice((ctx)->device)); hipStream_t s = (ctx)->stream; StreamOrder order_((ctx), s)
static inline hipStream_t call_stream(nbls_ctx* ctx, void* stream) { return stream ? (hipStream_t)stream : ctx->stream; }
#define DEV_ENTER(ctx, stream) std::lock_guard<std::recursive_mutex> g_((ctx)->mu); HIPCHK(hipSetDevice((ctx)->device)); hipStream_t s = call_stream((ctx), (stream)); StreamOrder order_((ctx), s)
#define WHOLE_CALL(ctx) std::lock_guard<std::recursive_mutex> whole_call_((ctx) ? (ctx)->mu : g_null_mu)

struct VerifyIn;
bool checked_mode();
bool aot_enabled();
int upload_program(nbls_ctx* ctx, DevProgram& d, const Program& p, const int k);
int upload(nbls_ctx* ctx, ProgId id);
int upload_extra(nbls_ctx* ctx, ExtraProg id);
void free_program(DevProgram& d);
bool wide_applies(const nbls_ctx* ctx, const DevProgram& d, int id, size_t n);
hipEvent_t timing_event(nbls_ctx* ctx);
void aot_seg(AotSeg& g, const DevProgram& d, const IOBuf* bufs);
void kernel_args(KernelArgs& ka, const nbls_ctx* ctx, const DevProgram& d, size_t n);
int run_dev(nbls_ctx* ctx, const DevProgram& d, int id, size_t n, const BufList& bufs, hipStream_t s, const uint32_t* n_dev, const uint32_t* item_index);
// ... 147 lines not shown
```

noble-bls12-381_amd/csrc/nbls_multi.cpp:

```cpp
#include <hip/hip_runtime.h>
#include <condition_variable>
#include <cstdio>
#include <cstdlib>
#include <cstring>
#include <deque>
#include <functional>
#include <mutex>
#include <thread>
#include <vector>
#include "nbls.h"
#include "config.h"

#define EXPORT extern "C" __attribute__((visibility("default")))

struct GatherLanes;
struct CallBuffers {
  std::vector<uint8_t*> part;
  uint8_t* gather = nullptr;
  GatherLanes* lanes = nullptr;
};
struct Worker {
  std::thread th; std::mutex mu; std::condition_variable cv; std::deque<std::function<void()>> q; bool stop = false;
  void run() {
    for (;;) {
// ... 103 lines not shown
  return NBLS_OK;
}
EXPORT int nbls_multi_peer_access(const nbls_multi* m, int i) { return m && i >= 0 && i < (int)m->peer.size() ? m->peer[i] : -1; }
EXPORT int nbls_multi_device_count(const nbls_multi* m) { return m ? (int)m->ctx.size() : 0; }
EXPORT nbls_ctx* nbls_multi_context(nbls_multi* m, int i) { return m && i >= 0 && i < (int)m->ctx.size() ? m->ctx[i] : nullptr; }

static void shard(size_t n, size_t G, size_t g, size_t* lo, size_t* hi) { const size_t q = n / G, r = n % G; *lo = g * q + (g < r ? g : r); *hi = *lo + q + (g < r ? 1 : 0); }

template <class F> static int on_every_device(nbls_multi* m, size_t G, F f) {
  std::vector<int> rc(G, 0);
  std::mutex mu; std::condition_variable cv; size_t pending = G > 1 ? G - 1 : 0;
  for (size_t g = 1; g < G; g++) m->workers[g]->post([&, g] { rc[g] = f(g); std::lock_guard<std::mutex> l(mu); if (--pending == 0) cv.notify_one(); });
  rc[0] = f(0);
  { std::unique_lock<std::mutex> l(mu); cv.wait(l, [&] { return pending == 0; }); }
  for (size_t g = 0; g < G; g++) if (rc[g] && rc[g] != NBLS_EDECODE) return rc[g];
  for (size_t g = 0; g < G; g++) if (rc[g]) return rc[g];
  return NBLS_OK;
}

EXPORT int nbls_multi_pairing_batch(nbls_multi* m, size_t n, const uint8_t* g1, const uint8_t* g2, int with_final_exp, int validate, uint8_t* out, int8_t* status) {
  if (!m || m->ctx.empty() || (n && (!g1 || !g2 || !out))) return NBLS_EINVAL;
  const size_t G = m->ctx.size();
  return on_every_device(m, G, [&](size_t g) {
    size_t lo, hi; shard(n, G, g, &lo, &hi);
    if (hi == lo) return (int)NBLS_OK;
    return nbls_pairing_batch(m->ctx[g], hi - lo, g1 + lo * 96, g2 + lo * 192, with_final_exp, validate, out + lo * 576, status ? status + lo : nullptr);
  });
}

static int finish(nbls_multi* m, CallBuffers* b, size_t G, int final_exp, uint8_t* out) {
  if (hipSetDevice(m->dev[0]) != hipSuccess) return NBLS_EHIP;
  GatherLanes* L = b->lanes;
  for (size_t g = 0; g < G; g++) {
    const hipError_t e = g == 0 || m->dev[g] == m->dev[0] ? hipMemcpyAsync(b->gather + 576 * g, b->part[g], 576, hipMemcpyDeviceToDevice, L->s[g])
                                                           : hipMemcpyPeerAsync(b->gather + 576 * g, m->dev[0], b->part[g], m->dev[g], 576, L->s[g]);
    if (e != hipSuccess || hipEventRecord(L->e[g], L->s[g]) != hipSuccess || hipStreamWaitEvent(L->fin, L->e[g], 0) != hipSuccess) { (void)hipDeviceSynchronize(); return NBLS_EHIP; }
  }
  uint8_t* res = b->gather + 576 * m->dev.size();
  int r = nbls_fp12_product_final_dev(m->ctx[0], G, b->gather, final_exp, res, L->fin);
  if (r) { (void)hipDeviceSynchronize(); return r; }
  if (hipMemcpyAsync(out, res, 576, hipMemcpyDeviceToHost, L->fin) != hipSuccess || hipStreamSynchronize(L->fin) != hipSuccess) return NBLS_EHIP;
  return NBLS_OK;
}

EXPORT int nbls_multi_miller_product(nbls_multi* m, size_t n, const uint8_t* g1, const uint8_t* g2, int final_exp, int validate, uint8_t* out, int8_t* status) {
  if (!m || m->ctx.empty() || !out || (n && (!g1 || !g2))) return NBLS_EINVAL;
  const size_t G = m->ctx.size();
  SetLease lease(m);
  if (!lease.b) return NBLS_EHIP;
  CallBuffers* b = lease.b;
  int r = on_every_device(m, G, [&](size_t g) {
    size_t lo, hi; shard(n, G, g, &lo, &hi);
    void* p = b->part[g];
    return nbls_miller_product_partial_into(m->ctx[g], hi - lo, g1 + lo * 96, g2 + lo * 192, validate, p, status ? status + lo : nullptr);
  });
  if (r) { if (r == NBLS_EDECODE) memset(out, 0, 576); return r; }
  return finish(m, b, G, final_exp, out);
}

EXPORT int nbls_multi_verify_batch(nbls_multi* m, size_t n, const uint8_t* sig96, const uint8_t* msgs, const uint32_t* offsets, const uint8_t* pk48,
                                   const uint8_t* dst, size_t dst_len, int* ok) {
  if (!m || m->ctx.empty() || !ok || !n || !sig96 || !offsets || !pk48 || !dst) return NBLS_EINVAL;
  size_t G = m->ctx.size();
  if (G > n) G = n;
  SetLease lease(m);
  if (!lease.b) return NBLS_EHIP;
  CallBuffers* b = lease.b;
  std::vector<int> zero(G, 0);
  int r = on_every_device(m, G, [&](size_t g) {
    size_t lo, hi; shard(n, G, g, &lo, &hi);
    void* p = b->part[g];
    return nbls_verify_batch_partial_into(m->ctx[g], hi - lo, g == 0 ? sig96 : nullptr, msgs, offsets + lo, pk48 + lo * 48, dst, dst_len, p, &zero[g], nullptr);
  });
  if (r) return r;
  for (int z : zero) if (z) { *ok = 0; return NBLS_OK; }
  uint8_t e[576];
  r = finish(m, b, G, 1, e);
  if (r) return r;
  bool one = e[47] == 1; for (int i = 0; i < 576 && one; i++) if (i != 47 && e[i]) one = false;
  *ok = one ? 1 : 0;
  return NBLS_OK;
}

static int g_queues_set_by_library = 0;
__attribute__((constructor)) static void nbls_on_load() {
  if (getenv("NBLS_KEEP_HW_QUEUES")) return;
  if (!getenv("GPU_MAX_HW_QUEUES")) { setenv("GPU_MAX_HW_QUEUES", "22", 0); g_queues_set_by_library = 1; }
}
EXPORT int nbls_hw_queues(int* set_by_library) {
  if (set_by_library) *set_by_library = g_queues_set_by_library;
  const char* v = getenv("GPU_MAX_HW_QUEUES");
  return v && *v ? atoi(v) : 0;
}
struct nbls_pool { std::vector<nbls_ctx*> ctx; std::mutex mu; size_t next = 0; int device = 0; };
EXPORT void nbls_pool_destroy(nbls_pool* p) { if (!p) return; for (nbls_ctx* c : p->ctx) nbls_destroy(c); delete p; }
EXPORT int nbls_pool_init(int device_id, int depth, nbls_pool** out) {
  if (!out || depth < 1 || depth > 64) return NBLS_EINVAL;
  {
    const int q = nbls_hw_queues(nullptr), eff = q > 0 ? q : 4;
    static bool warned = false;
    if (depth > eff && !warned) {
      warned = true;
      fprintf(stderr, "nbls: pool of %d contexts on %d hardware queues (GPU_MAX_HW_QUEUES %s): streams will share queues and their kernels serialise; "
                      "set GPU_MAX_HW_QUEUES >= depth (<= 22) before the first HIP call of the process\n",
              depth, eff, q > 0 ? "as set" : "unset");
    }
  }
  nbls_pool* p = new nbls_pool(); p->device = device_id;
  for (int i = 0; i < depth; i++) {
    nbls_ctx* c = nullptr;
    const int r = nbls_init(device_id, &c);
    if (r) { nbls_pool_destroy(p); return r; }
    p->ctx.push_back(c);
    if (depth > 1) {
      nbls_set_tuning(c, NBLS_TUNE_SPLIT_MILLER_MIN, 0);
      if (nbls::env_long("NBLS_PIPELINE_CHAIN", 0) != 1) nbls_set_tuning(c, NBLS_TUNE_CHAIN_MAX, 0);
      nbls_set_tuning(c, NBLS_TUNE_LS_MAX, 0); nbls_set_tuning(c, NBLS_TUNE_LS2_MAX, 0);
      nbls_set_tuning(c, NBLS_TUNE_INV_WIDE_MAX, 256);
    }
  }
  *out = p;
  return NBLS_OK;
}
EXPORT int nbls_pool_depth(const nbls_pool* p) { return p ? (int)p->ctx.size() : 0; }
EXPORT nbls_ctx* nbls_pool_context(nbls_pool* p, int i) { return p && i >= 0 && i < (int)p->ctx.size() ? p->ctx[i] : nullptr; }
EXPORT int nbls_pool_pairing_batch_dev(nbls_pool* p, size_t n, const void* d_g1, const void* d_g2, int with_final_exp, void* d_out, int* slot) {
  if (!p || p->ctx.empty()) return NBLS_EINVAL;
  size_t k;
  { std::lock_guard<std::mutex> l(p->mu); k = p->next++ % p->ctx.size(); }
  if (slot) *slot = (int)k;
  return nbls_pairing_batch_dev(p->ctx[k], n, d_g1, d_g2, with_final_exp, d_out, nullptr);
}
EXPORT int nbls_pool_next_slot(nbls_pool* p) { if (!p || p->ctx.empty()) return -1; std::lock_guard<std::mutex> l(p->mu); return (int)(p->next % p->ctx.size()); }
EXPORT int nbls_pool_synchronize(nbls_pool* p) { return p && !p->ctx.empty() ? nbls_device_synchronize(p->ctx[0]) : NBLS_EINVAL; }
```

noble-bls12-381_amd/csrc/pipelines_pairing.cpp:

```cpp
#include "nbls_internal.h"

int reduce_product(nbls_ctx* ctx, size_t n, uint8_t** result, hipStream_t s) {
  for (size_t d = 1; d < n; d *= 2) {
    const size_t pairs = ((n + d - 1) / d) / 2;
    if (!pairs) continue;
    const int r = run(ctx, P_MUL2S, pairs, {B(3, ctx->F, 2 * d * F12), B(4, ctx->F + d * F12, 2 * d * F12), B(5, ctx->F, 2 * d * F12)}, s);
    if (r) return r;
  }
  *result = ctx->F;
  return NBLS_OK;
}
int expx(nbls_ctx* ctx, const Window& w, size_t n, uint8_t* in, uint8_t* out, hipStream_t s) {
  int r;
  if (n < ctx->expc_min) return run(ctx, ls_variant(ctx, P_EXPX, n), n, {B(3, in, F12), B(5, out, F12)}, s);
  const size_t KSB = (size_t)EXPC_SQ_ELEMS * RAW, KDB = (size_t)EXPC_DEC_ELEMS * RAW;
  if ((r = ensure_expc_scratch(ctx))) return r;
  uint8_t *KS = ctx->KS + w.first * KSB, *KD = ctx->KD + w.first * KDB, *N = ctx->N + w.first * RAW, *NI = ctx->NI + w.first * RAW, *flag = ctx->Kflag + w.first;
  if ((r = run(ctx, P_EXPC_SQ, n, {B(3, in, F12), B(5, KS, KSB)}, s))) return r;
  if ((r = run(ctx, P_EXPC_DEC_A, n, {B(3, KS, KSB), B(4, N, RAW), B(5, KD, KDB)}, s))) return r;
  if ((r = run_inv(ctx, n, N, NI, s))) return r;
  if ((r = run(ctx, P_EXPC_DEC_B, n, {B(3, KS, KSB), B(4, NI, RAW), B(6, KD, KDB), B(5, out, F12), B(7, flag, 1)}, s))) return r;
  uint32_t* count = ctx->Kcount + w.half;
  uint32_t* list = ctx->Klist + w.first;
  LAUNCHCHK(nbls_flag_compact_launch((unsigned)n, flag, list, count, s));
  return run(ctx, P_EXPX, n, {B(3, in, F12), B(5, out, F12)}, s, count, list);
}
int final_exp_pipeline(nbls_ctx* ctx, const Window& w, size_t n, uint8_t* f_raw, void* d_out, hipStream_t s) {
  int r;
  uint8_t *N = ctx->N + w.first * RAW, *NI = ctx->NI + w.first * RAW, *T[7];
  for (int k = 0; k < 7; k++) T[k] = ctx->T[k] + w.first * F12;
  if ((r = run_inv(ctx, n, N, NI, s))) return r;
  if ((r = run(ctx, P_FE_EASY, n, {B(3, f_raw, F12), B(4, NI, RAW), B(5, T[0], F12)}, s))) return r;
  const ChainLink mid[7] = {{P_EXPX, {B(3, T[0], F12), B(5, T[1], F12)}},
                            {P_FE_MID1, {B(3, T[0], F12), B(5, T[1], F12), B(6, T[2], F12)}},
                            {P_EXPX, {B(3, T[2], F12), B(5, T[3], F12)}},
                            {P_EXPX, {B(3, T[3], F12), B(5, T[4], F12)}},
                            {P_EXPX, {B(3, T[4], F12), B(5, T[6], F12)}},
                            {P_FE_MID2, {B(3, T[6], F12), B(5, T[1], F12), B(6, T[5], F12)}},
                            {P_EXPX, {B(3, T[5], F12), B(5, T[6], F12)}}};
  if (n < ctx->expc_min && n < ctx->chain_max && !w.beside && ls_variant(ctx, P_EXPX, n) == P_EXPX && !wide_applies(ctx, ctx->prog[P_EXPX], (int)P_EXPX, n)) {
    if ((r = run_chain(ctx, n, mid, 7, s))) return r;
  } else for (const ChainLink& l : mid) {
    if ((r = l.id == P_EXPX ? expx(ctx, w, n, (uint8_t*)l.bufs.a[0].ptr, (uint8_t*)l.bufs.a[1].ptr, s) : run(ctx, l.id, n, l.bufs, s))) return r;
  }
  return run(ctx, P_FE_FINAL, n, {B(0, T[0], F12), B(1, T[1], F12), B(2, T[2], F12), B(3, T[3], F12), B(4, T[4], F12), B(5, T[5], F12), B(6, T[6], F12), B(7, d_out, 576)}, s);
}
int finish_single(nbls_ctx* ctx, const Window& w, uint8_t* f_raw, int final_exp, void* d_out, hipStream_t s) {
  int r;
  if (!final_exp) return run(ctx, P_RAW_TO_BYTES, 1, {B(3, f_raw, F12), B(2, d_out, 576)}, s);
  if ((r = run(ctx, P_NORM_RAW, 1, {B(3, f_raw, F12), B(4, ctx->N + w.first * RAW, RAW)}, s))) return r;
  return final_exp_pipeline(ctx, w, 1, f_raw, d_out, s);
}
static int finish_product(nbls_ctx* ctx, size_t m, int final_exp, void* d_out, hipStream_t s) {
  int r;
  uint8_t* res = ctx->F;
  if (m == 0) HIPCHK(hipMemcpyAsync(ctx->F, ctx->one12, F12, hipMemcpyDeviceToDevice, s));
  else if ((r = reduce_product(ctx, m, &res, s))) return r;
  return finish_single(ctx, Window(), res, final_exp, d_out, s);
}

EXPORT int nbls_pairing_batch_dev(nbls_ctx* ctx, size_t n, const void* d_g1, const void* d_g2, int with_final_exp, void* d_out, void* stream) {
  if (!ctx || (n && (!d_g1 || !d_g2 || !d_out))) return NBLS_EINVAL;
  if (n == 0) return NBLS_OK;
  DEV_ENTER(ctx, stream);
  if (n >= ctx->halves_min && n <= LINES_CHUNK) {
    int r;
    if ((r = ensure_lines(ctx, n))) return r;
    if (with_final_exp && (r = ensure_scratch(ctx, n))) return r;
    if ((r = ensure_half_stream(ctx))) return r;
    static const size_t split_pct = (size_t)std::min<long>(99, std::max<long>(1, env_long("NBLS_HALVES_SPLIT_PCT", 55)));
    const size_t h = ((n * split_pct / 100) + 63) & ~(size_t)63;
    if (h > 0 && h < n) {
      HIPCHK(hipEventRecord(ctx->ev_half_fork, s)); HIPCHK(hipStreamWaitEvent(ctx->half_stream, ctx->ev_half_fork, 0));
      ForkGuard fork_guard;
      Window first, second; first.beside = second.beside = true; second.first = h; second.half = 1;
      r = pairing_core(ctx, first, h, d_g1, d_g2, with_final_exp, d_out, s, true);
      if (!r) r = pairing_core(ctx, second, n - h, (const uint8_t*)d_g1 + h * 96, (const uint8_t*)d_g2 + h * 192, with_final_exp, (uint8_t*)d_out + h * 576, ctx->half_stream, true);
      HIPCHK(hipEventRecord(ctx->ev_half_join, ctx->half_stream)); HIPCHK(hipStreamWaitEvent(s, ctx->ev_half_join, 0));
      if (!r) fork_guard.armed = false;
      return r;
    }
  }
  return pairing_core(ctx, Window(), n, d_g1, d_g2, with_final_exp, d_out, s, false);
}
int pairing_core(nbls_ctx* ctx, const Window& w, size_t n, const void* d_g1, const void* d_g2, int with_final_exp, void* d_out, hipStream_t s, bool two_programs) {
  int r;
  static const int fused_mode = (int)env_long("NBLS_FUSED_MILLER", -1);
  const bool fused = fused_mode >= 0 ? fused_mode != 0 : (!two_programs && n < ctx->split_min);
  if (fused) {
    if (!with_final_exp) return run(ctx, ls_variant(ctx, P_MILLER_BYTES, n), n, {B(0, d_g1, 96), B(1, d_g2, 192), B(2, d_out, 576)}, s);
    if ((r = ensure_scratch(ctx, n))) return r;
    if ((r = run(ctx, ls_variant(ctx, P_MILLER_FE, n), n, {B(0, d_g1, 96), B(1, d_g2, 192), B(3, ctx->F + w.first * F12, F12), B(4, ctx->N + w.first * RAW, RAW)}, s))) return r;
    return final_exp_pipeline(ctx, w, n, ctx->F + w.first * F12, d_out, s);
  }
  if ((r = ensure_lines(ctx, n))) return r;
  if (with_final_exp && (r = ensure_scratch(ctx, n))) return r;
  const bool lines_fe = with_final_exp && lines_fe_enabled();
  if (lines_fe && (r = upload_extra(ctx, XP_LINES_FE))) return r;
  uint8_t *L = ctx->L + w.first * LINE_BYTES, *F = with_final_exp ? ctx->F + w.first * F12 : nullptr, *N = with_final_exp ? ctx->N + w.first * RAW : nullptr;
  for (size_t o = 0; o < n; o += LINES_CHUNK) {
    const size_t c = n - o < LINES_CHUNK ? n - o : LINES_CHUNK;
    const uint8_t *g1 = (const uint8_t*)d_g1 + o * 96, *g2 = (const uint8_t*)d_g2 + o * 192;
    if (lines_fe) r = run_dev(ctx, ctx->extra[XP_LINES_FE], (int)P_LINES_PQ, c, {B(0, g1, 96), B(1, g2, 192), B(3, L, LINE_BYTES)}, s, nullptr, nullptr);
    else r = run(ctx, P_LINES_PQ, c, {B(0, g1, 96), B(1, g2, 192), B(3, L, LINE_BYTES)}, s);
    if (r) return r;
    if (!with_final_exp) r = run(ctx, P_ACC_BYTES, c, {B(3, L, LINE_BYTES), B(2, (uint8_t*)d_out + o * 576, 576)}, s);
    else r = run(ctx, P_ACC_FE, c, {B(3, L, LINE_BYTES), B(5, F + o * F12, F12), B(4, N + o * RAW, RAW)}, s);
    if (r) return r;
  }
  if (!with_final_exp) return NBLS_OK;
  return final_exp_pipeline(ctx, w, n, F, d_out, s);
}

static const size_t PIN_STAGE_MAX = 1u << 20, VALIDATE_BESIDE_MAX = 1024;
static int stage_points(nbls_ctx* ctx, size_t n, const uint8_t* g1, const uint8_t* g2, bool validate, void* d_st, hipStream_t s) {
  int r;
  if ((r = ensure_io(ctx, n ? n : 1)) || !n) return r;
  const uint8_t *h1 = g1, *h2 = g2;
  if (n * 288 <= PIN_STAGE_MAX) {
    if ((r = ensure_pinned(ctx, n * 288))) return r;
    memcpy(ctx->pinned, g1, n * 96); memcpy(ctx->pinned + n * 96, g2, n * 192);
    h1 = ctx->pinned; h2 = ctx->pinned + n * 96;
  }
  HIPCHK(hipMemcpyAsync(ctx->io_g1, h1, n * 96, hipMemcpyHostToDevice, s));
  HIPCHK(hipMemcpyAsync(ctx->io_g2, h2, n * 192, hipMemcpyHostToDevice, s));
  if (!validate) return NBLS_OK;
  if (n > VALIDATE_BESIDE_MAX) {
    if ((r = dev_validate(ctx, false, n, ctx->io_g1, d_st, s))) return r;
// ... 309 lines not shown
```

noble-bls12-381_amd/csrc/programs.cpp:

```cpp
#include "programs.h"
#include "config.h"
#include <mutex>
#include "aot.h"
#include "tower.h"
#include "curve.h"
#include "codec.h"
#include "vm_exec.h"

namespace nbls {

static SFp12 trace_miller(const SFp& Px, const SFp& Py, const SFp2& Qx, const SFp2& Qy) {
  SFp2 Rx = Qx, Ry = Qy, Rz = fp2_one();
  SFp12 f = fp12_one();
  for (int i = 62; i >= 0; i--) {
    SFp2 t0 = sqr(Ry), t1 = sqr(Rz);
    SFp2 t2 = mat(mul_by_b(scale(t1, 3)));
    SFp2 t3 = scale(t2, 3);
    SFp2 t4 = mat(sqr(Ry + Rz) - t1 - t0);
    SFp2 e0 = t2 - t0, e1 = scale(sqr(Rx), 3), e2 = -t4;
    SFp2 nRx = mul(halve(t0 - t3), mul(Rx, Ry));
    SFp2 nRy = sqr(halve(t0 + t3)) - scale(sqr(t2), 3);
    SFp2 nRz = mul(t0, t4);
    Rx = mat(nRx); Ry = mat(nRy); Rz = mat(nRz);
    f = mat(mul_by_014(f, e0, mul_fp(e1, Px), mul_fp(e2, Py)));
// ... 107 lines not shown
    SFp2 nY = mat(SFp2{mul(scale(tp, 2), scale(tm3, 2)) - mul(c0.c0 + c0.c1, c0.c0 - c0.c1), mul(scale(t03.c0, 2), t03.c1 + t0.c1) - mul(scale(c0.c0, 2), c0.c1)});
    SFp2 nE = mat(mul(scale(t03, 2), scale(w2, 2)));
    T = nT; Y = nY; E = nE;
    if ((NBLS_X >> i) & 1) {
      const SFp2 Rx = scale(T, 2);
      SFp2 Ry = mat(scale(Y, 6));
      SFp2 a0 = mat(scale(Y, 6) - mul(Qy, E)), a1 = mat(Rx - mul(Qx, E));
      emit(mat(mul(a0, Qx) - mul(a1, Qy)), -mul_fp(a0, Px), mul_fp(a1, scale(Pyh, 2)));
      SFp2 a2 = mat(sqr(a1)), a3 = mat(mul(a2, a1)), a4 = mat(mul(a2, Rx));
      SFp2 a5 = mat(a3 - scale(a4, 2) + mul(sqr(a0), E));
      nT = mat(scale(mul(a1, a5), 3)); nY = mat(mul(a4 - a5, a0) - mul(a3, Ry)); nE = mat(scale(mul(E, a3), 6));
      T = nT; Y = nY; E = nE;
    }
  }
}
static SFp2 load_line_coef(int buf, int off) { return {inputw(buf, off), inputw(buf, off + 48)}; }
static SFp12 trace_acc(int m, int buf, const std::vector<SFp>* Px = nullptr, const std::vector<SFp>* Py = nullptr) {
  SFp12 f = fp12_one();
  int j = 0;
  auto step = [&](int jj) {
    for (int t = 0; t < m; t++) {
      const int off = 48 * LINE_ELEMS * t + 48 * 6 * jj;
      SFp2 c0 = load_line_coef(buf, off), c1 = load_line_coef(buf, off + 96), c2 = load_line_coef(buf, off + 192);
      if (Px) { c1 = mat(mul_fp(c1, (*Px)[t])); c2 = mat(mul_fp(c2, (*Py)[t])); }
      f = mat(mul_by_014(f, c0, c1, c2));
    }
  };
  for (int i = 62; i >= 0; i--) {
    step(j++);
    if ((NBLS_X >> i) & 1) step(j++);
    if (i != 0) f = mat(sqr(f));
  }
  return conj(f);
}

struct InvChain { SFp6 t; SFp2 T0, T1, T2, d; SFp n; };
static InvChain inv_chain(const SFp12& f) {
  InvChain c;
  c.t = mat(sqr(f.c0) - mulnr(sqr(f.c1)));
  c.T0 = mat(sqr(c.t.c0) - mulnr(mul(c.t.c2, c.t.c1)));
  c.T1 = mat(mulnr(sqr(c.t.c2)) - mul(c.t.c0, c.t.c1));
  c.T2 = mat(sqr(c.t.c1) - mul(c.t.c0, c.t.c2));
  c.d = mat(mulnr(mul(c.t.c2, c.T1) + mul(c.t.c1, c.T2)) + mul(c.t.c0, c.T0));
  c.n = sqr(c.d.c0) + sqr(c.d.c1);
  return c;
}
static SFp12 inv_finish(const SFp12& f, const InvChain& c, const SFp& ninv) {
  SFp2 dinv = {mul(c.d.c0, ninv), -mul(c.d.c1, ninv)};
  SFp6 tinv = mat(SFp6{mul(dinv, c.T0), mul(dinv, c.T1), mul(dinv, c.T2)});
  return {mul(f.c0, tinv), -mul(f.c1, tinv)};
}

static SFp12 trace_fe_easy(const SFp12& f, const SFp12& finv) {
  SFp12 t0 = mat(mul(frob(f, 6), finv));
  return mul(frob(t0, 2), t0);
}
static SFp12 trace_fe_final(const SFp12& t1, const SFp12& t2, const SFp12& t3, const SFp12& t4, const SFp12& t5, const SFp12& t6, const SFp12& t7) {
  SFp12 a = mat(frob(mul(t2, t5), 2));
  SFp12 b = mat(frob(mul(t4, t1), 3));
  SFp12 c = mat(frob(mul(t6, conj(t1)), 1));
  SFp12 d = mat(mul(mat(mul(t7, conj(t3))), t1));
  return mul(mat(mul(mat(mul(a, b)), c)), d);
}
template <class Load>
static SFp12 trace_fe_final_chain(Load t) {
  SFp12 m = mat(frob(mat(mul(t(4), t(1))), 1));
  m = mat(mul(m, t(2))); m = mat(mul(m, t(5)));
  m = mat(frob(m, 1));
  m = mat(mul(m, t(6))); m = mat(mul(m, conj(t(1))));
  m = mat(frob(m, 1));
  m = mat(mul(m, t(7))); m = mat(mul(m, conj(t(3))));
  return mul(m, t(1));
}

static void load_points(SFp& Px, SFp& Py, SFp2& Qx, SFp2& Qy) {
  Px = input(0, 0); Py = input(0, 48);
  Qx = input_fp2(1, 0); Qy = input_fp2(1, 96);
}

static int env_int(const char* name, int dflt) { return (int)env_long(name, dflt); }
static const int MILLER_W = env_int("NBLS_MILLER_W", 16);
static const int G1_W = env_int("NBLS_G1_W", 4), G2_W = env_int("NBLS_G2_W", 8), G2MUL_W = env_int("NBLS_G2MUL_W", 8), G1MUL_W = env_int("NBLS_G1MUL_W", 4);
static const int EXPX_W = env_int("NBLS_EXPX_W", 12);
static const int LINES_W = env_int("NBLS_LINES_W", 10), ACC_W = env_int("NBLS_ACC_W", 12), ACC_WINDOW = env_int("NBLS_ACC_WINDOW", 330);

static bool aot_listed(ProgId id) {
#define AOT_HAS(PART, NAME, P0, P1, P2, P3) if (id == P0 || id == P1 || id == P2 || id == P3) return true;
  NBLS_AOT_KERNELS(AOT_HAS)
#undef AOT_HAS
  return false;
}
static Program build(ProgId id) {
  Builder B;
  if (aot_listed(id) && env_int("NBLS_AOT_SHARED_CONSTS", 1)) B.shared_consts = 1;
  if (id == P_MILLER_BYTES || id == P_MILLER_RAW || id == P_MILLER_FE) B.max_dot = env_int("NBLS_MILLER_MAXDOT", 6);
  if (id == P_EXPX) B.max_dot = env_int("NBLS_EXPX_MAXDOT", 8);
  const bool ls2 = id == P_MILLER_BYTES_LS2 || id == P_MILLER_RAW_LS2 || id == P_MILLER_FE_LS2 || id == P_EXPX_LS2 || id == P_H2C_C1_LS2 || id == P_H2C_C2_LS2 || id == P_G2_MUL_SAC_LS2;
  const bool ls = ls2 || id == P_MILLER_BYTES_LS || id == P_MILLER_RAW_LS || id == P_MILLER_FE_LS || id == P_EXPX_LS;
  if (ls) { B.lane_split = ls2 ? 2 : 4; B.max_dot = env_int("NBLS_LS_MAXDOT", 8); }
  switch (id) {
    case P_MILLER_BYTES: case P_MILLER_BYTES_LS: case P_MILLER_BYTES_LS2: {
      SFp Px, Py; SFp2 Qx, Qy; load_points(Px, Py, Qx, Qy);
      output_fp12(trace_miller(Px, Py, Qx, Qy), 2, 0);
      return B.compile(ls2 ? "miller_bytes_ls2" : ls ? "miller_bytes_ls" : "miller_bytes", ls ? 16 : MILLER_W);
    }
    case P_MILLER_RAW: case P_MILLER_RAW_LS: case P_MILLER_RAW_LS2: {
      SFp Px, Py; SFp2 Qx, Qy; load_points(Px, Py, Qx, Qy);
      outputw_fp12(trace_miller(Px, Py, Qx, Qy), 3, 0);
      return B.compile(ls2 ? "miller_raw_ls2" : ls ? "miller_raw_ls" : "miller_raw", ls ? 16 : MILLER_W);
    }
    case P_MILLER_RAW2: {
      std::vector<SFp> Px, Py; std::vector<SFp2> Qx, Qy;
      for (int j = 0; j < 2; j++) { Px.push_back(input(0, 96 * j)); Py.push_back(input(0, 96 * j + 48)); Qx.push_back(input_fp2(1, 192 * j)); Qy.push_back(input_fp2(1, 192 * j + 96)); }
      outputw_fp12(trace_miller_shared(Px, Py, Qx, Qy), 3, 0);
      B.sched_window = env_int("NBLS_MILLER2_WINDOW", 450);
      return B.compile("miller_raw2", MILLER_W);
    }
    case P_MILLER_FE: case P_MILLER_FE_LS: case P_MILLER_FE_LS2: {
      SFp Px, Py; SFp2 Qx, Qy; load_points(Px, Py, Qx, Qy);
      SFp12 f = mat(trace_miller(Px, Py, Qx, Qy));
      outputw_fp12(f, 3, 0);
      outputw(inv_chain(f).n, 4, 0);
      return B.compile(ls2 ? "miller_fe_ls2" : ls ? "miller_fe_ls" : "miller_fe", ls ? 16 : MILLER_W);
    }
    case P_NORM_RAW: {
      SFp12 f = inputw_fp12(3, 0);
      outputw(inv_chain(f).n, 4, 0);
      return B.compile("norm_raw", 16);
    }
    case P_NORM_BYTES: {
      SFp12 f = mat(input_fp12(2, 0));
      outputw_fp12(f, 3, 0);
      outputw(inv_chain(f).n, 4, 0);
      return B.compile("norm_bytes", 16);
    }
    case P_FE_EASY: {
      SFp12 f = inputw_fp12(3, 0);
      SFp ninv = inputw(4, 0);
      InvChain c = inv_chain(f);
      SFp12 finv = mat(inv_finish(f, c, ninv));
      outputw_fp12(trace_fe_easy(f, finv), 5, 0);
      return B.compile("fe_easy", env_int("NBLS_FE_EASY_W", 16));
    }
    case P_EXPX: case P_EXPX_LS: case P_EXPX_LS2: {
      if (env_int("NBLS_EXPX_RELOAD", 1)) {
        B.sched_window = env_int("NBLS_EXPX_WINDOW", 150);
        outputw_fp12(conj(cyclotomic_exp_x(inputw_fp12(3, 0), [&]() { return inputw_fp12(3, 0); })), 5, 0);
      } else outputw_fp12(conj(cyclotomic_exp_x(inputw_fp12(3, 0))), 5, 0);
      return B.compile(ls2 ? "expx_ls2" : ls ? "expx_ls" : "expx", ls ? 12 : EXPX_W);
    }
    case P_EXPC_SQ: {
      auto ld = [&](int i) { return SFp2{inputw(3, 96 * i), inputw(3, 96 * i + 48)}; };
      SCyc4 a = {ld(3), ld(2), ld(1), ld(5)};
      const SFp three = SFp(B.small_const(3));
      auto m3 = [&](const SFp2& v) { return SFp2{mul(v.c0, three), mul(v.c1, three)}; };
      SCyc4 z = mat(SCyc4{m3(a.g2), m3(a.g3), m3(a.g4), m3(a.g5)});
      int slot = 0;
      for (int k = 1; k <= EXPC_TOP; k++) {
        z = mat(compressed_sqr_tripled(z));
        if ((NBLS_X >> k) & 1) {
          const SFp2* c[4] = {&z.g2, &z.g3, &z.g4, &z.g5};
          for (int e = 0; e < 4; e++) { outputw(c[e]->c0, 5, (8 * slot + 2 * e) * 48); outputw(c[e]->c1, 5, (8 * slot + 2 * e + 1) * 48); }
          slot++;
        }
      }
      B.store_batch = 8;
// ... 484 lines not shown
      case T_FROB: r = frob(a, param); break;
      case T_CONJ: r = conj(a); break;
      case T_MULNR: r = mulnr(a); break;
      case T_MUL_BY_B: r = mul_by_b(a); break;
      default: return Program();
    }
    output_fp2(r, 7, 0);
    return B.compile(name, 4);
  }
  if (field == 6) {
    SFp6 a = in_fp6(0, 0);
    if (op == T_INV) {
      Inv6 c = inv6_chain(a);
      if (part == 0) outputw(sqr(c.d.c0) + sqr(c.d.c1), 4, 0);
      else out_fp6(inv6_finish(c, inputw(5, 0)), 7, 0);
      return B.compile(name, 8);
    }
    SFp6 r;
    switch (op) {
      case T_ADD: r = a + in_fp6(1, 0); break;
      case T_SUB: r = a - in_fp6(1, 0); break;
      case T_NEG: r = -a; break;
      case T_MUL: r = mul(a, in_fp6(1, 0)); break;
      case T_SQR: r = sqr(a); break;
      case T_FROB: r = frob(a, param); break;
      case T_MULNR: r = mulnr(a); break;
      case T_MUL_BY_1: r = mul_by_1(a, input_fp2(1, 0)); break;
      case T_MUL_BY_01: r = mul_by_01(a, input_fp2(1, 0), input_fp2(2, 0)); break;
      default: return Program();
    }
    out_fp6(r, 7, 0);
    return B.compile(name, 8);
  }
  if (field == 12) {
    SFp12 a = mat(input_fp12(0, 0));
    if (op == T_INV) {
      InvChain c = inv_chain(a);
      if (part == 0) outputw(c.n, 4, 0);
      else output_fp12(inv_finish(a, c, inputw(5, 0)), 7, 0);
      return B.compile(name, 16);
    }
    SFp12 r;
    switch (op) {
      case T_ADD: { SFp12 b = input_fp12(1, 0); r = {a.c0 + b.c0, a.c1 + b.c1}; break; }
      case T_SUB: { SFp12 b = input_fp12(1, 0); r = {a.c0 - b.c0, a.c1 - b.c1}; break; }
      case T_NEG: r = {-a.c0, -a.c1}; break;
      case T_MUL: r = mul(a, mat(input_fp12(1, 0))); break;
      case T_SQR: r = sqr(a); break;
      case T_FROB: r = frob(a, param); break;
      case T_CONJ: r = conj(a); break;
      case T_MUL_BY_014: r = mul_by_014(a, input_fp2(1, 0), input_fp2(2, 0), input_fp2(3, 0)); break;
      case T_CYC_SQR: r = cyclotomic_sqr(a); break;
      case T_CYC_EXP: r = cyclotomic_exp_x(a); break;
      default: return Program();
    }
    output_fp12(r, 7, 0);
    return B.compile(name, op == T_CYC_EXP ? 12 : 16);
  }
  (void)W;
  return Program();
}
}
const Program* get_tower_program(int field, int op, int param, int part) {
  static std::map<std::tuple<int, int, int, int>, Program> cache;
  static std::mutex mu;
  std::lock_guard<std::mutex> g(mu);
  if (!(field == 1 || field == 2 || field == 6 || field == 12) || op < 0 || op >= T_COUNT || part < 0 || part > 1 || (part == 1 && op != T_INV)) return nullptr;
  if (op != T_FROB) param = 0; else if (param < 0 || param > 11) return nullptr;
  auto key = std::make_tuple(field, op, param, part);
  auto it = cache.find(key);
  if (it == cache.end()) it = cache.emplace(key, build_tower(field, op, param, part)).first;
  return it->second.steps.empty() ? nullptr : &it->second;
}

static Program build_extra(ExtraProg id) {
  Builder B;
  if (env_int("NBLS_AOT_SHARED_CONSTS", 1)) B.shared_consts = 1;
  if (id == XP_LINES_FE) {
    SFp Px, Py; SFp2 Qx, Qy; load_points(Px, Py, Qx, Qy);
    B.light_max = MAX_DOT_PRODUCTS; B.neg_cap = 7.0; B.store_batch = 6;
    trace_lines_fe(Px, Py, Qx, Qy, 3);
    return B.compile("lines_fe", LINES_W);
  }
  if (id == XP_DBLADD_G1) {
    auto ld = [&](int buf) { return Pt<SFp>{inputw(buf, 0), inputw(buf, 48), inputw(buf, 96)}; };
    Pt<SFp> r = pt_add(pt_dbl(ld(3)), ld(4));
    outputw(r.x, 3, 0); outputw(r.y, 3, 48); outputw(r.z, 3, 96);
    return B.compile("dbladd_g1", 4);
  }
  if (id == XP_ENDO_G1) {
    SFp x = inputw(3, 0), y = inputw(3, 48), z = inputw(3, 96);
    outputw(x, 5, 0); outputw(y, 5, 48); outputw(z, 5, 96);
    outputw(mul(x, fp_const(NBLS_BETA)), 5, 144); outputw(-y, 5, 192); outputw(z, 5, 240);
    return B.compile("endo_g1", 4);
  }
  if (id == XP_DBLADD_G2) {
    auto ld = [&](int buf) { return Pt<SFp2>{{inputw(buf, 0), inputw(buf, 48)}, {inputw(buf, 96), inputw(buf, 144)}, {inputw(buf, 192), inputw(buf, 240)}}; };
    Pt<SFp2> r = pt_add(pt_dbl(ld(3)), ld(4));
    outputw(r.x.c0, 3, 0); outputw(r.x.c1, 3, 48); outputw(r.y.c0, 3, 96); outputw(r.y.c1, 3, 144); outputw(r.z.c0, 3, 192); outputw(r.z.c1, 3, 240);
    return B.compile("dbladd_g2", 8);
  }
  const bool g2 = id == XP_POLY_G2_16 || id == XP_POLY_G2_256, low16 = id == XP_POLY_G1_16 || id == XP_POLY_G2_16;
  const SFp k = low16 ? input_raw(2, 28, 4) : input_raw(2, 0, 32);
  const int nbits = low16 ? 16 : 256;
  if (!g2) {
    auto ld = [&](int buf) { return Pt<SFp>{inputw(buf, 0), inputw(buf, 48), inputw(buf, 96)}; };
    Pt<SFp> r = pt_add(pt_mul_ladder(ld(3), k, nbits, 2), ld(4));
    outputw(r.x, 3, 0); outputw(r.y, 3, 48); outputw(r.z, 3, 96);
    B.sched_window = env_int("NBLS_G1MUL_WINDOW", 200);
    return B.compile(low16 ? "poly_g1_16" : "poly_g1_256", G1MUL_W);
  }
  auto ld = [&](int buf) { return Pt<SFp2>{{inputw(buf, 0), inputw(buf, 48)}, {inputw(buf, 96), inputw(buf, 144)}, {inputw(buf, 192), inputw(buf, 240)}}; };
  Pt<SFp2> r = pt_add(pt_mul_ladder(ld(3), k, nbits, 2), ld(4));
  outputw(r.x.c0, 3, 0); outputw(r.x.c1, 3, 48); outputw(r.y.c0, 3, 96); outputw(r.y.c1, 3, 144); outputw(r.z.c0, 3, 192); outputw(r.z.c1, 3, 240);
  B.sched_window = env_int("NBLS_MUL_WINDOW", 300);
  return B.compile(low16 ? "poly_g2_16" : "poly_g2_256", G2MUL_W);
}
bool lines_fe_enabled() { static const bool on = env_long("NBLS_LINES_FE", 1) != 0; return on; }
const Program& get_extra_program(ExtraProg id) {
  static Program cache[XP_COUNT];
  static bool built[XP_COUNT];
  static std::mutex mu;
  std::lock_guard<std::mutex> g(mu);
  if (!built[id]) { cache[id] = build_extra(id); built[id] = true; }
  return cache[id];
}

const Program& get_program(ProgId id) {
  static Program cache[P_COUNT];
  static bool built[P_COUNT];
  static std::mutex mu;
  std::lock_guard<std::mutex> g(mu);
  if (!built[id]) { cache[id] = build(id); built[id] = true; }
  return cache[id];
}

void print_stats(const Program& p) {
  printf("%-14s W=%2u G=%u steps=%5zu (dot %4u, lin %4u, other %3u)  dot_ops=%6u products=%6u (product-slot fill %.2f)  lin_ops=%6u terms=%6u  slots=%4u  lds=%6u B  descs=%zu KB  operands: combined %u normalised %u; round operands %u: single %u sum %u diff %u mixed %u norm %u  est_valu=%.0fk\n",
         p.name.c_str(), p.W, p.G, p.steps.size(), p.n_dot_steps, p.n_lin_steps, p.n_other_steps, p.n_dot_ops, p.n_products,
         p.n_prod_slots ? (double)p.n_products / p.n_prod_slots : 0.0, p.n_lin_ops, p.n_lin_terms, p.slots, p.lds_bytes(), p.descs.size() * 4 / 1024, p.n_comb_operands, p.n_norm_operands, p.n_round_ops, p.n_op_mode[0], p.n_op_mode[1], p.n_op_mode[2], p.n_op_mode[3], p.n_op_norm, p.est_valu / 1e3);
}

}
```

noble-bls12-381_amd/csrc/programs.h:

```cpp
#pragma once
#include "trace.h"
namespace nbls {
enum ProgId {
  P_MILLER_BYTES = 0,
  P_MILLER_RAW,
  P_MILLER_FE,
  P_NORM_RAW,
  P_NORM_BYTES,
  P_FE_EASY,
  P_EXPX,
  P_FE_MID1,
  P_FE_MID2,
  P_FE_FINAL,
  P_MUL2,
  P_RAW_TO_BYTES,
  P_G1_VALIDATE,
  P_G2_VALIDATE,
  P_G1_DEC_A,
  P_G1_DEC_B,
  P_G2_DEC_A,
  P_G2_DEC_B,
  P_H2C_A,
  P_H2C_B,
  P_G1_TO_PROJ, P_G1_ADD2, P_G1_NORM, P_G1_TO_AFFINE,
  P_G2_TO_PROJ, P_G2_ADD2, P_G2_NORM, P_G2_TO_AFFINE,
  P_T_SWU, P_T_ISO, P_T_CLEAR,
  P_H2C_C,
  P_MILLER_RAW2,
  P_G1_COMPRESS, P_G2_COMPRESS,
  P_H2C1_A, P_ENC1_A,
  P_H2C1_B, P_ENC1_B,
  P_G1_CLEAR,
  P_ENC2_A, P_ENC2_B,
  P_G1_MUL, P_G2_MUL,
  P_G1_ADD_AB, P_G2_ADD_AB,
  P_G1_HORNER, P_G2_HORNER,
  P_G1_SHIFTADD, P_G2_SHIFTADD,
  P_G1_MSM_PREP,
  P_G2_MSM_PREP,
  P_LINES_PQ,
  P_LINES_Q,
  P_LINES_BYTES,
  P_LINES_FROM_BYTES,
  P_ACC_BYTES,
  P_ACC_RAW,
  P_ACC_FE,
  P_ACC2_RAW,
  P_ACC_Q,
  P_G2_DEC_A192, P_G2_DEC_B192,
  P_G2_DEC_B_HEX,
  P_G1_FROM_RAW, P_G2_FROM_RAW,
  P_G2_SWAP,
  P_H2C_C1, P_H2C_C2,
  P_ACC4_RAW,
  P_MILLER_BYTES_LS, P_MILLER_RAW_LS, P_MILLER_FE_LS, P_EXPX_LS,
  P_EXPC_SQ,
  P_EXPC_DEC_A,
  P_EXPC_DEC_B,
  P_ACC8_RAW,
  P_H2C_C0,
  P_H2C_B1,
  P_H2C_B2,
  P_G1_MUL_W3, P_G2_MUL_W3,
  P_MUL2S,
  P_G1_MUL_FIXED,
  P_G2_MUL_GLS,
  P_MILLER_BYTES_LS2, P_MILLER_RAW_LS2, P_MILLER_FE_LS2, P_EXPX_LS2,
  P_G2_MUL_SAC,
  P_H2C_C1_LS2, P_H2C_C2_LS2, P_G2_MUL_SAC_LS2,
  P_H2C_NA,
  P_H2C_NM,
  P_H2C_NB,
  P_G1_MUL64,
  P_COUNT
};
static const int EXPC_POWERS = 3, EXPC_TOP = 57;
static const int EXPC_SQ_ELEMS = 8 * EXPC_POWERS, EXPC_DEC_ELEMS = 6 * EXPC_POWERS + 1;
static const int N_LINES = 68;
static const int LINE_ELEMS = 6 * N_LINES;
static const int MSM_WINDOW_BITS = 12;
const Program& get_program(ProgId id);
const Program* get_tower_program(int field, int op, int param, int part);
enum ExtraProg { XP_POLY_G1_16 = 0, XP_POLY_G1_256, XP_POLY_G2_16, XP_POLY_G2_256, XP_DBLADD_G1, XP_DBLADD_G2, XP_LINES_FE, XP_ENDO_G1, XP_COUNT };
static const int XP_NUMBERED = XP_DBLADD_G1;
const Program& get_extra_program(ExtraProg id);
bool lines_fe_enabled();
void print_stats(const Program& p);
}
```

noble-bls12-381_amd/csrc/runtime.cpp:

```cpp
#include "nbls_internal.h"

std::recursive_mutex g_null_mu;
bool checked_mode() {
#if defined(NBLS_CHECKED)
  return true;
#else
  static const bool on = env_long("NBLS_CHECKED", 0) != 0;
  return on;
#endif
}
bool aot_enabled() { static const bool on = env_long("NBLS_AOT", 1) != 0; return on; }
int upload(nbls_ctx* ctx, ProgId id) {
  DevProgram& d = ctx->prog[id];
  if (d.p) return NBLS_OK;
  return upload_program(ctx, d, get_program(id), aot_enabled() ? nbls_aot_index((int)id) : -1);
}
int upload_extra(nbls_ctx* ctx, ExtraProg id) {
  DevProgram& d = ctx->extra[id];
  if (d.p) return NBLS_OK;
  return upload_program(ctx, d, get_extra_program(id), aot_enabled() ? nbls_aot_extra_index((int)id) : -1);
}
void free_program(DevProgram& d) {
  for (void* p : {(void*)d.steps, (void*)d.descs, (void*)d.consts, (void*)d.aot_steps, (void*)d.aot_descs}) if (p) hipFree(p);
  d = DevProgram();
// ... 29 lines not shown

hipEvent_t timing_event(nbls_ctx* ctx) {
  if (!ctx->ev_pool.empty()) { hipEvent_t e = ctx->ev_pool.back(); ctx->ev_pool.pop_back(); return e; }
  hipEvent_t e = nullptr; hipEventCreate(&e); return e;
}
struct Timed {
  nbls_ctx* ctx; int id; hipStream_t s; hipEvent_t e0 = nullptr, e1 = nullptr;
  Timed(nbls_ctx* c, int slot, hipStream_t st) : ctx(c), id(slot), s(st) { if (ctx->timing) { e0 = timing_event(ctx); e1 = timing_event(ctx); hipEventRecord(e0, s); } }
  ~Timed() {
    if (!e0) return;
    hipEventRecord(e1, s);
    if (id >= 0) ctx->tev.push_back({id, {e0, e1}}); else { ctx->ev_pool.push_back(e0); ctx->ev_pool.push_back(e1); }
  }
};

void aot_seg(AotSeg& g, const DevProgram& d, const IOBuf* bufs) {
  g.steps = d.aot_steps; g.descs = d.aot_descs; g.consts = d.consts;
  g.nsteps = (u32)d.p->steps.size(); g.nconst = d.p->nconst; g.inst_bytes = d.p->inst_bytes(); g.slot_bytes = d.p->slot_bytes; g.shared_consts = d.p->shared_consts ? 1u : 0u;
  for (int k = 0; k < MAX_BUFS; k++) g.bufs[k] = bufs[k];
}
void kernel_args(KernelArgs& ka, const nbls_ctx* ctx, const DevProgram& d, size_t n) {
  memset(&ka, 0, sizeof ka);
  ka.steps = d.steps; ka.descs = d.descs; ka.consts = d.consts; ka.qp_table = ctx->qp_table;
  ka.nsteps = (u32)d.p->steps.size(); ka.nconst = d.p->nconst; ka.W = d.p->W; ka.G = d.p->G; ka.slot_bytes = d.p->slot_bytes; ka.inst_bytes = d.p->inst_bytes();
  ka.shared_consts = d.p->shared_consts ? 1u : 0u; ka.lsplit = d.p->lsplit; ka.n_items = (u32)n;
}
int run(nbls_ctx* ctx, ProgId id, size_t n, const BufList& bufs, hipStream_t s, const uint32_t* n_dev, const uint32_t* item_index) {
  int r = upload(ctx, id); if (r) return r;
  return run_dev(ctx, ctx->prog[id], (int)id, n, bufs, s, n_dev, item_index);
}
int run_dev(nbls_ctx* ctx, const DevProgram& d, int id, size_t n, const BufList& bufs, hipStream_t s, const uint32_t* n_dev, const uint32_t* item_index) {
  KernelArgs ka; kernel_args(ka, ctx, d, n);
  d.launches++;
  ka.n_items_dev = n_dev; ka.item_index = item_index;
  if (!bind_bufs(ka.bufs, bufs)) { if (checked_mode()) fprintf(stderr, "nbls (checked): %s: a buffer index outside [0, %d)\n", d.p->name.c_str(), MAX_BUFS); return NBLS_EINVAL; }
  if (checked_mode()) {
    for (int k = 0; k < MAX_BUFS; k++) {
      const u32 ext = d.p->buf_extent[k];
      if (!ext) continue;
      if (!ka.bufs[k].ptr || (ka.bufs[k].stride != 0 && ka.bufs[k].stride < ext)) {
        fprintf(stderr, "nbls (checked): %s: buffer %d: %s (stride %llu, the program touches %u bytes per item)\n", d.p->name.c_str(), k, ka.bufs[k].ptr ? "stride too small" : "not bound",
            (unsigned long long)ka.bufs[k].stride, ext);
        return NBLS_EINVAL;
      }
      hipDeviceptr_t base = nullptr; size_t size = 0;
      if (n && !item_index && hipMemGetAddressRange(&base, &size, (hipDeviceptr_t)ka.bufs[k].ptr) == hipSuccess) {
        const size_t end = (size_t)((uint8_t*)ka.bufs[k].ptr - (uint8_t*)base) + (n - 1) * ka.bufs[k].stride + ext;
        if (end > size) {
          fprintf(stderr, "nbls (checked): %s: buffer %d: %zu items of stride %llu (+%u) end %zu bytes into an allocation of %zu\n", d.p->name.c_str(), k, n,
              (unsigned long long)ka.bufs[k].stride, ext, end, size);
          return NBLS_EINVAL;
        }
      } else (void)hipGetLastError();
    }
  }
  int e;
  {
    Timed timed(ctx, id, s);
    if (wide_applies(ctx, d, id, n)) e = nbls_vm_wide_launch(&ka, d.p->inst_base(0) + d.p->inst_bytes(), s);
    else if (d.aot >= 0) {
      AotArgs a; memset(&a, 0, sizeof a);
      aot_seg(a.seg[0], d, ka.bufs);
      a.nseg = 1; a.W = ka.W; a.G = ka.G; a.n_items = ka.n_items; a.qp_table = ka.qp_table; a.item_index = ka.item_index; a.n_items_dev = ka.n_items_dev;
      e = nbls_aot_launch(d.aot, &a, d.aot_lds, s);
    } else e = nbls_vm_launch(&ka, d.p->lds_bytes(), s);
  }
  if (e) { ctx->last_hip = e; return NBLS_EHIP; }
  return NBLS_OK;
}
int run_inv_buf(nbls_ctx* ctx, size_t n, const void* in, void* out, hipStream_t s) {
  LAUNCHCHK(n <= ctx->inv_wide_max ? nbls_fp_inv_wide_launch((unsigned)n, in, out, s) : nbls_fp_inv_launch((unsigned)n, in, out, s));
  return NBLS_OK;
}
int run_inv(nbls_ctx* ctx, size_t n, const void* in, void* out, hipStream_t s) {
  Timed timed(ctx, (int)P_COUNT, s);
  return run_inv_buf(ctx, n, in, out, s);
}

bool chains_enabled() { static const bool on = env_long("NBLS_CHAIN", 1) != 0; return on; }
int run_chain(nbls_ctx* ctx, size_t n, const ChainLink* links, size_t count, hipStream_t s) {
  int r;
  bool fuse = chains_enabled() && !checked_mode() && count <= (size_t)AOT_MAX_SEGS;
  int k = -1; u32 W = 0, G = 0, lds = 0;
  for (const ChainLink* l = links; l < links + count; l++) {
    if ((r = upload(ctx, l->id))) return r;
    const DevProgram& d = ctx->prog[l->id];
    if (d.aot < 0 || (k >= 0 && (d.aot != k || d.p->W != W || d.p->G != G))) fuse = false;
    k = d.aot; W = d.p->W; G = d.p->G; lds = std::max(lds, d.aot_lds);
  }
  if (!fuse) { for (const ChainLink* l = links; l < links + count; l++) if ((r = run(ctx, l->id, n, l->bufs, s))) return r; return NBLS_OK; }
  AotArgs a; memset(&a, 0, sizeof a);
  for (const ChainLink* l = links; l < links + count; l++) {
    IOBuf bufs[MAX_BUFS];
    if (!bind_bufs(bufs, l->bufs)) return NBLS_EINVAL;
    aot_seg(a.seg[a.nseg++], ctx->prog[l->id], bufs);
  }
  a.W = W; a.G = G; a.n_items = (u32)n; a.qp_table = ctx->qp_table;
  int e;
  { Timed timed(ctx, (int)links->id, s); e = nbls_aot_launch(k, &a, lds, s); }
  if (e) { ctx->last_hip = e; return NBLS_EHIP; }
  return NBLS_OK;
}

int ensure_scratch(nbls_ctx* ctx, size_t n) {
  if (n <= ctx->cap_F) return NBLS_OK;
  size_t cap = n + n / 8 + 64;
  if (ctx->F) {
    hipFree(ctx->F); hipFree(ctx->N); hipFree(ctx->NI); for (auto& t : ctx->T) { hipFree(t); t = nullptr; } hipFree(ctx->KS); hipFree(ctx->KD); hipFree(ctx->Kflag);
    hipFree(ctx->Klist); hipFree(ctx->Kcount);
  }
  ctx->F = ctx->N = ctx->NI = ctx->KS = ctx->KD = ctx->Kflag = nullptr; ctx->Klist = ctx->Kcount = nullptr; ctx->cap_F = 0;
  HIPCHK(hipMalloc(&ctx->F, (cap + 2) * F12));
  HIPCHK(hipMalloc(&ctx->N, cap * RAW));
  HIPCHK(hipMalloc(&ctx->NI, cap * RAW));
  for (auto& t : ctx->T) HIPCHK(hipMalloc(&t, cap * F12));
  ctx->cap_F = cap;
  return NBLS_OK;
}
int ensure_expc_scratch(nbls_ctx* ctx) {
  if (ctx->Kcount) return NBLS_OK;
  const size_t cap = ctx->cap_F;
  auto fail = [&]() { for (void* p : {(void*)ctx->KS, (void*)ctx->KD, (void*)ctx->Kflag, (void*)ctx->Klist,
      (void*)ctx->Kcount}) if (p) hipFree(p); ctx->KS = ctx->KD = ctx->Kflag = nullptr; ctx->Klist = ctx->Kcount = nullptr; ctx->last_hip = (int)hipGetLastError(); return NBLS_EHIP; };
  if (ctx->KS) { hipFree(ctx->KS); ctx->KS = nullptr; } if (ctx->KD) { hipFree(ctx->KD); ctx->KD = nullptr; } if (ctx->Kflag) { hipFree(ctx->Kflag); ctx->Kflag = nullptr; }
  if (ctx->Klist) { hipFree(ctx->Klist); ctx->Klist = nullptr; }
  if (hipMalloc(&ctx->KS, cap * EXPC_SQ_ELEMS * RAW) != hipSuccess || hipMalloc(&ctx->KD, cap * EXPC_DEC_ELEMS * RAW) != hipSuccess || hipMalloc(&ctx->Kflag, cap) != hipSuccess ||
      hipMalloc(&ctx->Klist, cap * 4) != hipSuccess || hipMalloc(&ctx->Kcount, 8) != hipSuccess) return fail();
  return NBLS_OK;
}
int ensure_io(nbls_ctx* ctx, size_t n) {
  if (n <= ctx->cap_io) return NBLS_OK;
  size_t cap = n + 64;
  if (ctx->io_g1) { hipFree(ctx->io_g1); hipFree(ctx->io_g2); hipFree(ctx->io_f12); }
  ctx->io_g1 = ctx->io_g2 = ctx->io_f12 = nullptr; ctx->cap_io = 0;
  HIPCHK(hipMalloc(&ctx->io_g1, cap * 96));
  HIPCHK(hipMalloc(&ctx->io_g2, cap * 192));
  HIPCHK(hipMalloc(&ctx->io_f12, cap * 576));
  ctx->cap_io = cap;
  return NBLS_OK;
}

int ensure_lines(nbls_ctx* ctx, size_t n) {
  if (n > LINES_CHUNK + 3) n = LINES_CHUNK + 3;
  if (n <= ctx->cap_L) return NBLS_OK;
  size_t cap = n + n / 8 + 8; if (cap > LINES_CHUNK + 3) cap = LINES_CHUNK + 3;
  if (ctx->L) hipFree(ctx->L);
  ctx->L = nullptr; ctx->cap_L = 0;
  HIPCHK(hipMalloc(&ctx->L, cap * LINE_BYTES));
  ctx->cap_L = cap;
  return NBLS_OK;
}
int ensure_fork_event(nbls_ctx* ctx) {
  if (!ctx->ev_fork && hipEventCreateWithFlags(&ctx->ev_fork, hipEventDisableTiming) != hipSuccess) { ctx->last_hip = (int)hipGetLastError(); return NBLS_EHIP; }
  return NBLS_OK;
}
int ensure_side(nbls_ctx* ctx) {
  int r = ensure_fork_event(ctx); if (r) return r;
  if (!ctx->side && hipStreamCreateWithFlags(&ctx->side, hipStreamNonBlocking) != hipSuccess) { ctx->side = nullptr; ctx->last_hip = (int)hipGetLastError(); return NBLS_EHIP; }
  if (!ctx->ev_join && hipEventCreateWithFlags(&ctx->ev_join, hipEventDisableTiming) != hipSuccess) { ctx->last_hip = (int)hipGetLastError(); return NBLS_EHIP; }
  if (!ctx->side_scratch && hipMalloc(&ctx->side_scratch, (6 + 2 * POW_TAB) * RAW) != hipSuccess) { ctx->side_scratch = nullptr; ctx->last_hip = (int)hipGetLastError(); return NBLS_EHIP; }
  return NBLS_OK;
}
int ensure_side2(nbls_ctx* ctx) {
  int r = ensure_fork_event(ctx); if (r) return r;
  if (!ctx->side2 && hipStreamCreateWithFlags(&ctx->side2, hipStreamNonBlocking) != hipSuccess) { ctx->side2 = nullptr; ctx->last_hip = (int)hipGetLastError(); return NBLS_EHIP; }
  if (!ctx->ev_join2 && hipEventCreateWithFlags(&ctx->ev_join2, hipEventDisableTiming) != hipSuccess) { ctx->last_hip = (int)hipGetLastError(); return NBLS_EHIP; }
  return NBLS_OK;
}
int ensure_half_stream(nbls_ctx* ctx) {
  if (!ctx->half_stream && (hipStreamCreateWithFlags(&ctx->half_stream, hipStreamNonBlocking) != hipSuccess || hipEventCreateWithFlags(&ctx->ev_half_fork, hipEventDisableTiming) != hipSuccess ||
                            hipEventCreateWithFlags(&ctx->ev_half_join, hipEventDisableTiming) != hipSuccess)) { ctx->last_hip = (int)hipGetLastError(); return NBLS_EHIP; }
  return NBLS_OK;
}
int ensure_pinned(nbls_ctx* ctx, size_t bytes) {
  if (bytes <= ctx->pinned_cap) return NBLS_OK;
  if (ctx->pinned) { hipHostFree(ctx->pinned); ctx->pinned = nullptr; ctx->pinned_cap = 0; }
  const size_t cap = bytes + bytes / 4 + 4096;
  HIPCHK(hipHostMalloc((void**)&ctx->pinned, cap, hipHostMallocDefault));
  ctx->pinned_cap = cap;
  return NBLS_OK;
}
int ensure_pinned_out(nbls_ctx* ctx, size_t bytes) {
  if (bytes <= ctx->pinned_out_cap) return NBLS_OK;
// ... 129 lines not shown
```

noble-bls12-381_amd/csrc/tuning.cpp:

```cpp
#include "nbls_internal.h"

size_t ls_max() { static const size_t v = (size_t)env_long("NBLS_LS_MAX", 1024); return v; }
size_t ls2_max() { static const size_t v = (size_t)env_long("NBLS_LS2_MAX", 2048); return v; }
ProgId ls_variant(nbls_ctx* ctx, ProgId id, size_t n) {
  if (n <= ctx->wide_max && upload(ctx, id) == NBLS_OK && wide_applies(ctx, ctx->prog[id], (int)id, n)) return id;
  if (n <= ctx->ls_max) {
    switch (id) {
      case P_MILLER_BYTES: return P_MILLER_BYTES_LS;
      case P_MILLER_RAW: return P_MILLER_RAW_LS;
      case P_MILLER_FE: return P_MILLER_FE_LS;
      case P_EXPX: return P_EXPX_LS;
      default: return id;
    }
  }
  if (n <= ctx->ls2_max) {
    ProgId v = id;
    switch (id) {
      case P_MILLER_BYTES: v = P_MILLER_BYTES_LS2; break;
      case P_MILLER_RAW: v = P_MILLER_RAW_LS2; break;
      case P_MILLER_FE: v = P_MILLER_FE_LS2; break;
      case P_EXPX: v = P_EXPX_LS2; break;
      default: return id;
    }
    if (upload(ctx, v) == NBLS_OK && ctx->prog[v].aot >= 0) return v;
// ... 24 lines not shown
  HIPCHK(hipMemsetAsync(ctx->T[0], 0, n * F12, ctx->stream));
  int e = nbls_vm_launch(&ka, d.p->lds_bytes(), ctx->stream);
  if (e) { hipFree(dbg); ctx->last_hip = e; return NBLS_EHIP; }
  HIPCHK(hipMemcpyAsync(out_blocks, dbg, blocks * 40, hipMemcpyDeviceToHost, ctx->stream)); HIPCHK(hipStreamSynchronize(ctx->stream));
  hipFree(dbg);
  return NBLS_OK;
}
EXPORT int nbls_field_kernel_raw(nbls_ctx* ctx, int kind, int form, size_t n, const uint8_t* in_raw, uint8_t* out_raw) {
  if (!ctx || kind < 0 || kind > 4 || form < 0 || form > 2 || n > ((size_t)1 << 24) || (n && (!in_raw || !out_raw))) return NBLS_EINVAL;
  if (!n) return NBLS_OK;
  const bool is_fp2 = kind == 1 || kind == 2;
  const size_t bytes = n * (is_fp2 ? 2 : 1) * RAW;
  LOCKED(ctx); HostIO io{ctx}; void *d = io.alloc(bytes), *o = io.alloc(bytes); if (!d || !o) return NBLS_EHIP;
  HIPCHK(hipMemcpyAsync(d, in_raw, bytes, hipMemcpyHostToDevice, s));
  int r;
  if (kind == 4) {
    if (form == 0) { if ((r = run_inv_buf(ctx, n, d, o, s))) return r; }
    else LAUNCHCHK(form == 2 ? nbls_fp_inv_wide_launch((unsigned)n, d, o, s) : nbls_fp_inv_launch((unsigned)n, d, o, s));
  } else if (form == 0) { if ((r = run_pow(ctx, kind, n, d, o, s))) return r; }
  else {
    const int tail = kind == 1 ? 8 : kind == 2 ? 7 : 0;
    if (form == 2) LAUNCHCHK(nbls_pow_wide_launch((unsigned)n, d, o, ctx->nib[kind], ctx->nnib[kind], tail, s));
    else {
      uint8_t* tab; if ((r = need(ctx, SB_POW_TABLE, n * POW_TAB * (is_fp2 ? 2 : 1) * RAW, &tab))) return r;
      LAUNCHCHK(nbls_fp_pow_launch((unsigned)n, d, o, ctx->nib[kind], ctx->nnib[kind], tab, tail, s));
    }
  }
  HIPCHK(hipMemcpyAsync(out_raw, o, bytes, hipMemcpyDeviceToHost, s)); HIPCHK(hipStreamSynchronize(s));
  return NBLS_OK;
}
EXPORT int nbls_program_stats(nbls_ctx* ctx, int prog, uint32_t* o) {
  (void)ctx;
  if (prog < 0 || prog >= P_COUNT || !o) return NBLS_EINVAL;
  const Program& p = get_program((ProgId)prog);
  o[0] = (uint32_t)p.steps.size(); o[1] = p.n_dot_steps; o[2] = p.n_lin_steps; o[3] = p.n_dot_ops; o[4] = p.n_products; o[5] = p.n_lin_ops; o[6] = p.slots; o[7] = p.lds_bytes();
  return NBLS_OK;
}

EXPORT int nbls_timing_enable(nbls_ctx* ctx, int on) {
  if (!ctx) return NBLS_EINVAL;
  std::lock_guard<std::recursive_mutex> g(ctx->mu);
  for (auto& t : ctx->tev) { ctx->ev_pool.push_back(t.second.first); ctx->ev_pool.push_back(t.second.second); }
  ctx->tev.clear(); ctx->timing = on != 0; return NBLS_OK;
}
EXPORT int nbls_timing_read(nbls_ctx* ctx, float* ms, uint32_t* counts) {
  if (!ctx || !ms || !counts) return NBLS_EINVAL;
  std::lock_guard<std::recursive_mutex> g(ctx->mu);
  HIPCHK(hipSetDevice(ctx->device));
  for (int i = 0; i <= P_COUNT; i++) { ms[i] = 0; counts[i] = 0; }
  for (auto& t : ctx->tev) {
    HIPCHK(hipEventSynchronize(t.second.second));
    float m = 0; HIPCHK(hipEventElapsedTime(&m, t.second.first, t.second.second));
    ms[t.first] += m; counts[t.first]++;
    ctx->ev_pool.push_back(t.second.first); ctx->ev_pool.push_back(t.second.second);
  }
  ctx->tev.clear();
  return NBLS_OK;
}

EXPORT int nbls_set_tuning(nbls_ctx* ctx, int key, long long value) {
  if (!ctx) return NBLS_EINVAL;
  std::lock_guard<std::recursive_mutex> g(ctx->mu);
  switch (key) {
    case NBLS_TUNE_SPLIT_MILLER_MIN: if (value < 0) return NBLS_EINVAL; ctx->split_min = (size_t)value; return NBLS_OK;
    case NBLS_TUNE_HALVES_MIN: if (value < 0) return NBLS_EINVAL; ctx->halves_min = value == 0 ? (size_t)-1 : (size_t)value; return NBLS_OK;
    case NBLS_TUNE_EXPC_MIN: if (value < 0) return NBLS_EINVAL; ctx->expc_min = (size_t)value; return NBLS_OK;
    case NBLS_TUNE_CHAIN_MAX: if (value < 0) return NBLS_EINVAL; ctx->chain_max = (size_t)value; return NBLS_OK;
    case NBLS_TUNE_SAC_MAX: if (value < 0) return NBLS_EINVAL; ctx->sac_max = (size_t)value; return NBLS_OK;
    case NBLS_TUNE_PT_LS2_MAX: if (value < 0) return NBLS_EINVAL; ctx->pt_ls2_max = (size_t)value; return NBLS_OK;
    case NBLS_TUNE_WIDE_MAX: if (value < 0) return NBLS_EINVAL; ctx->wide_max = (size_t)value; return NBLS_OK;
    case NBLS_TUNE_H2C_NORM_MIN: if (value < 0) return NBLS_EINVAL; ctx->h2c_norm_min = (size_t)value; return NBLS_OK;
    case NBLS_TUNE_INV_WIDE_MAX: if (value < 0) return NBLS_EINVAL; ctx->inv_wide_max = (size_t)value; return NBLS_OK;
    case NBLS_TUNE_LS_MAX: if (value < 0) return NBLS_EINVAL; ctx->ls_max = (size_t)value; return NBLS_OK;
    case NBLS_TUNE_LS2_MAX: if (value < 0) return NBLS_EINVAL; ctx->ls2_max = (size_t)value; return NBLS_OK;
    case NBLS_TUNE_VERIFY_CHUNKS: if (value < 0 || value > 16) return NBLS_EINVAL; ctx->verify_chunks = (long)value; return NBLS_OK;
    case NBLS_TUNE_VERIFY_LAST_PCT: if (value < 1 || value > 100) return NBLS_EINVAL; ctx->verify_last_pct = (long)value; return NBLS_OK;
    case NBLS_TUNE_VERIFY_PIPE_MIN: if (value < 0) return NBLS_EINVAL; ctx->verify_pipe_min = (long)value; return NBLS_OK;
    case NBLS_TUNE_POLY_SLAB: if (value < 0) return NBLS_EINVAL; ctx->poly_slab = (size_t)value; return NBLS_OK;
    case NBLS_TUNE_MSMB_WINDOW: if (value != 0 && value != 4 && value != 6 && value != 8 && value != 10 && value != 12) return NBLS_EINVAL; ctx->msmb_window = (size_t)value; return NBLS_OK;
    case NBLS_TUNE_MSMB_BIG: if (value < 0) return NBLS_EINVAL; ctx->msmb_big = (size_t)value; return NBLS_OK;
    case NBLS_TUNE_MSMB_SLAB: if (value < 0) return NBLS_EINVAL; ctx->msmb_slab = (size_t)value; return NBLS_OK;
    case NBLS_TUNE_CELLS_CHUNK: if (value < 0) return NBLS_EINVAL; ctx->cells_chunk = (size_t)value; return NBLS_OK;
    case NBLS_TUNE_G16_CHUNK: if (value < 0) return NBLS_EINVAL; ctx->g16_chunk = (size_t)value; return NBLS_OK;
    default: return NBLS_EINVAL;
  }
}
EXPORT const char* nbls_program_kernel(nbls_ctx* ctx, int prog) {
  if (!ctx || prog < 0 || prog >= P_COUNT) return nullptr;
  std::lock_guard<std::recursive_mutex> g(ctx->mu);
  if (hipSetDevice(ctx->device) != hipSuccess || upload(ctx, (ProgId)prog)) return nullptr;
  const DevProgram& d = ctx->prog[prog];
  return d.aot >= 0 ? nbls_aot_name(d.aot) : d.p->lsplit == 4 ? "nbls_vm_kernel_ls4" : d.p->lsplit == 1 ? "nbls_vm_kernel" : "none (two-lane programs have no interpreter form)";
}
EXPORT const char* nbls_extra_program_kernel(nbls_ctx* ctx, const char* name) {
  if (!ctx || !name) return nullptr;
  std::lock_guard<std::recursive_mutex> g(ctx->mu);
  for (int i = 0; i < (int)XP_COUNT; i++) {
    if (get_extra_program((ExtraProg)i).name != name) continue;
    if (hipSetDevice(ctx->device) != hipSuccess || upload_extra(ctx, (ExtraProg)i)) return nullptr;
    const DevProgram& d = ctx->extra[i];
    return d.aot >= 0 ? nbls_aot_name(d.aot) : "nbls_vm_kernel";
  }
  return nullptr;
}
EXPORT long long nbls_extra_program_launches(nbls_ctx* ctx, const char* name) {
  if (!ctx || !name) return -1;
  std::lock_guard<std::recursive_mutex> g(ctx->mu);
  for (int i = 0; i < (int)XP_COUNT; i++) if (get_extra_program((ExtraProg)i).name == name) return (long long)ctx->extra[i].launches;
  return -1;
}
EXPORT int nbls_aot_kernel_private_bytes(int k) { return nbls_aot_private_bytes(k); }
EXPORT int nbls_program_count(void) { return (int)P_COUNT; }
EXPORT const char* nbls_program_name(int prog) { return prog >= 0 && prog < P_COUNT ? get_program((ProgId)prog).name.c_str() : nullptr; }
```

noble-bls12-381_amd/engine.py:

```python
import ctypes as C
import os
try:
    import numpy as _np
except ImportError:
    _np = None

_HERE = os.path.dirname(os.path.abspath(__file__))
ABI_VERSION = 5
PROGRAMS = []
DST_DEFAULT = b'BLS_SIG_BLS12381G2_XMD:SHA-256_SSWU_RO_NUL_'


class NblsError(RuntimeError):
    pass


def lib_path():
    return os.environ.get('NBLS_LIBRARY') or os.path.join(_HERE, 'libnbls.so')


def load_library():
    p = lib_path()
    if not os.path.exists(p):
        raise NblsError('libnbls.so is not built (run __graft_entry__.build() or make -C noble-bls12-381_amd/csrc)')
# ... 876 lines not shown
        self._chk(self.lib.nbls_verify_aggregates_indexed(self.h, keyset.h, n, b''.join(sigs96), blob, offs, idx, koffs, dst, len(dst), seed, C.byref(ok), st))
        return bool(ok.value), (st.raw[:n] if per_set else None)

    def _shared_args(self, what, sigs96, msgs, msg_index, sets, seed):
        n = len(sigs96)
        if len(msg_index) != n or len(sets) != n or (seed is not None and len(seed) != 32):
            raise NblsError('%s: %d signatures, %d message indices, %d keys or key sets, seed of %s bytes' % (what, n, len(msg_index), len(sets), None if seed is None else len(seed)))
        if _np is not None and isinstance(msg_index, _np.ndarray) and msg_index.dtype == _np.uint32 and msg_index.ndim == 1:
            a = _np.ascontiguousarray(msg_index)
            idx = (C.c_uint32 * n).from_buffer(a if a.flags.writeable else a.copy())
        else:
            if n and not 0 <= min(msg_index) <= max(msg_index) <= 0xffffffff:
                raise NblsError('%s: a message index outside 0 .. 2^32 - 1' % what)
            idx = self._u32(msg_index)
        blob, offs = self._pack(msgs)
        return n, blob, offs, idx

    def verify_multiple_shared(self, sigs96, msgs, msg_index, pks48, dst=DST_DEFAULT, seed=None, per_set=True):
        n, blob, offs, idx = self._shared_args('verify_multiple_shared', sigs96, msgs, msg_index, pks48, seed)
        ok = C.c_int(0)
        st = C.create_string_buffer(max(n, 1)) if per_set else None
        self._chk(self.lib.nbls_verify_multiple_shared(self.h, n, b''.join(sigs96), len(msgs), blob, offs, idx, b''.join(pks48), dst, len(dst), seed, C.byref(ok), st))
        return bool(ok.value), (st.raw[:n] if per_set else None)

    def verify_aggregates_shared(self, sigs96, msgs, msg_index, key_sets, dst=DST_DEFAULT, seed=None, per_set=True):
        n, blob, offs, idx = self._shared_args('verify_aggregates_shared', sigs96, msgs, msg_index, key_sets, seed)
        koffs = self._key_offsets(key_sets)
        pks = b''.join(b''.join(k) for k in key_sets)
        ok = C.c_int(0)
        st = C.create_string_buffer(max(n, 1)) if per_set else None
        self._chk(self.lib.nbls_verify_aggregates_shared(self.h, n, b''.join(sigs96), len(msgs), blob, offs, idx, pks, koffs, dst, len(dst), seed, C.byref(ok), st))
        return bool(ok.value), (st.raw[:n] if per_set else None)

    def verify_aggregates_indexed_shared(self, keyset, sigs96, msgs, msg_index, index_sets, dst=DST_DEFAULT, seed=None, per_set=True):
        n, blob, offs, idx = self._shared_args('verify_aggregates_indexed_shared', sigs96, msgs, msg_index, index_sets, seed)
        if keyset.h is None:
            raise NblsError('verify_aggregates_indexed_shared: the key table is closed')
        koffs = self._key_offsets(index_sets)
        kidx = self._u32([i for s in index_sets for i in s])
        ok = C.c_int(0)
        st = C.create_string_buffer(max(n, 1)) if per_set else None
        self._chk(self.lib.nbls_verify_aggregates_indexed_shared(self.h, keyset.h, n, b''.join(sigs96), len(msgs), blob, offs, idx, kidx, koffs, dst, len(dst), seed, C.byref(ok), st))
        return bool(ok.value), (st.raw[:n] if per_set else None)

    def verify_batch_dev(self, n, d_sig, d_uniform, d_pk, stream=None):
        ok = C.c_int(0)
        self._chk(self.lib.nbls_verify_batch_dev_inputs(self.h, n, d_sig, d_uniform, d_pk, C.byref(ok), None, stream))
        return bool(ok.value)

    def verify_batch_msgs_dev(self, n, d_sig, d_msgs, d_offsets, d_pk, dst=DST_DEFAULT, stream=None):
        ok = C.c_int32(0)
        self._chk(self.lib.nbls_verify_batch_msgs_dev(self.h, n, d_sig, d_msgs, d_offsets, d_pk, dst, len(dst), C.byref(ok), stream))
        return bool(ok.value)

    def verify_batch_partial_dev(self, n, d_sig, d_uniform, d_pk, d_out, stream=None):
        z = C.c_int(0)
        self._chk(self.lib.nbls_verify_batch_partial_dev(self.h, n, d_sig or None, d_uniform, d_pk, d_out, C.byref(z), None, stream))
        return bool(z.value)

    def pairing_batch_dev(self, n, d_g1, d_g2, d_out, with_final_exp=True, stream=None):
        self._chk(self.lib.nbls_pairing_batch_dev(self.h, n, d_g1, d_g2, int(with_final_exp), d_out, stream))

    def miller_product_dev(self, n, d_g1, d_g2, d_out, final_exp=True, stream=None):
        self._chk(self.lib.nbls_miller_product_dev(self.h, n, d_g1, d_g2, int(final_exp), d_out, stream))

    def final_exp_batch_dev(self, n, d_in, d_out, stream=None):
        self._chk(self.lib.nbls_final_exp_batch_dev(self.h, n, d_in, d_out, stream))

    def fp12_product_final_dev(self, n, d_in, d_out, final_exp=True, stream=None):
        self._chk(self.lib.nbls_fp12_product_final_dev(self.h, n, d_in, int(final_exp), d_out, stream))

    def set_expc_min(self, n):
        self._chk(self.lib.nbls_set_tuning(self.h, 3, n))

    def set_split_miller_min(self, n):
        self._chk(self.lib.nbls_set_tuning(self.h, 1, n))

    def set_halves_min(self, n):
        self._chk(self.lib.nbls_set_tuning(self.h, 2, n))

    def set_chain_max(self, n):
        self._chk(self.lib.nbls_set_tuning(self.h, 4, n))

    def set_sac_max(self, n):
        self._chk(self.lib.nbls_set_tuning(self.h, 8, n))

    def set_wide_max(self, n):
        self._chk(self.lib.nbls_set_tuning(self.h, 10, n))

    def set_ls_max(self, ls_max=None, ls2_max=None):
        if ls_max is not None: self._chk(self.lib.nbls_set_tuning(self.h, 13, int(ls_max)))
        if ls2_max is not None: self._chk(self.lib.nbls_set_tuning(self.h, 14, int(ls2_max)))

    def set_inv_wide_max(self, n):
        self._chk(self.lib.nbls_set_tuning(self.h, 12, int(n)))

    def set_h2c_norm_min(self, n):
        self._chk(self.lib.nbls_set_tuning(self.h, 11, int(n)))

    def set_pt_ls2_max(self, n):
        self._chk(self.lib.nbls_set_tuning(self.h, 9, n))

    def set_poly_slab(self, n):
        self._chk(self.lib.nbls_set_tuning(self.h, 15, int(n)))

    def set_msm_batch(self, window=None, big=None, slab=None):
        for key, v in ((16, window), (17, big), (18, slab)):
            if v is not None:
                self._chk(self.lib.nbls_set_tuning(self.h, key, int(v)))

    def set_cells_chunk(self, blobs):
        self._chk(self.lib.nbls_set_tuning(self.h, 20, int(blobs)))

    def set_groth16_chunk(self, proofs):
        self._chk(self.lib.nbls_set_tuning(self.h, 22, int(proofs)))

    def set_verify_pipeline(self, chunks=None, last_pct=None, pipe_min=None):
        for key, v in ((5, chunks), (6, last_pct), (7, pipe_min)):
            if v is not None:
                self._chk(self.lib.nbls_set_tuning(self.h, key, v))

    def synchronize(self):
        self._chk(self.lib.nbls_device_synchronize(self.h))

    def program_stats(self, name):
        o = (C.c_uint32 * 8)()
        self._chk(self.lib.nbls_program_stats(self.h, PROGRAMS.index(name), o))
        keys = ['steps', 'dot_steps', 'lin_steps', 'dot_ops', 'products', 'lin_ops', 'slots', 'lds_bytes']
        return dict(zip(keys, list(o)))

    def program_kernel(self, name):
        k = self.lib.nbls_program_kernel(self.h, PROGRAMS.index(name))
        if k is None:
            raise NblsError('nbls_program_kernel(%s) failed' % name)
        return k.decode()

    def extra_program_kernel(self, name):
        k = self.lib.nbls_extra_program_kernel(self.h, name.encode())
        if k is None:
            raise NblsError('nbls_extra_program_kernel(%s) failed' % name)
        return k.decode()

    def extra_program_launches(self, name):
        self.lib.nbls_extra_program_launches.restype = C.c_longlong
        self.lib.nbls_extra_program_launches.argtypes = [C.c_void_p, C.c_char_p]
        return self.lib.nbls_extra_program_launches(self.h, name.encode())

    def kernel_bindings(self):
        return {p: self.program_kernel(p) for p in PROGRAMS}

    def device_synchronize(self):
        self._chk(self.lib.nbls_device_synchronize(self.h))

    def timing_enable(self, on=True):
        self._chk(self.lib.nbls_timing_enable(self.h, int(on)))

    def tower_op(self, field, op, a, b=None, c=None, d=None, param=0):
        esz = 48 * field
        n = len(a) // esz
        out = C.create_string_buffer(n * esz)
        args = [C.c_char_p(x) if x is not None else None for x in (a, b, c, d)]
        self._chk(self.lib.nbls_tower_op_batch(self.h, C.c_int(field), C.c_int(op), C.c_int(param), C.c_size_t(n), args[0], args[1], args[2], args[3], out))
        return out.raw

    FIELD_KINDS = {'sqrt': 0, 'fp2_sqrt': 1, 'fp2_sqrt_div': 2, 'swu': 3, 'inv': 4}

    def field_kernel_raw(self, kind, form, n, raw, out=None):
        kind = self.FIELD_KINDS[kind] if isinstance(kind, str) else int(kind)
        size = 64 * n * (2 if kind in (1, 2) else 1)
        if len(raw) < size:
            raise NblsError('field_kernel_raw: %d bytes for %d elements' % (len(raw), n))
        if out is None:
            out = C.create_string_buffer(max(size, 1))
        elif len(out) < size:
            raise NblsError('field_kernel_raw: output buffer of %d bytes for %d elements' % (len(out), n))
        self._chk(self.lib.nbls_field_kernel_raw(self.h, kind, int(form), n, raw, out))
        return out.raw

    def config_describe(self):
        return self.lib.nbls_config_describe().decode()

    def timing_read(self):
        n = len(PROGRAMS) + 1
        ms = (C.c_float * n)()
        cnt = (C.c_uint32 * n)()
        self._chk(self.lib.nbls_timing_read(self.h, ms, cnt))
        names = PROGRAMS + ['fp_inv']
        return {names[i]: (ms[i], cnt[i]) for i in range(n) if cnt[i]}


class MultiEngine:

    def __init__(self, devices=None):
        self.lib = load_library()
        h = C.c_void_p()
        if devices is None:
            r = self.lib.nbls_init_multi(0, None, C.byref(h))
        else:
            ids = (C.c_int * len(devices))(*devices)
            r = self.lib.nbls_init_multi(len(devices), ids, C.byref(h))
        if r != 0:
            raise NblsError('nbls_init_multi failed: %s (code %d)' % (self.lib.nbls_strerror(r).decode(), r))
        self.h = h
        self.n_devices = self.lib.nbls_multi_device_count(h)

    def close(self):
        if getattr(self, 'h', None):
            self.lib.nbls_destroy_multi(self.h)
            self.h = None

    def __del__(self):
        try:
            self.close()
        except Exception:
            pass

    def _chk(self, r):
        if r != 0:
            raise NblsError('%s (code %d)' % (self.lib.nbls_strerror(r).decode(), r))

    def pairing_batch(self, g1_aff, g2_aff, with_final_exp=True, validate=False):
        n = len(g1_aff) // 96
        out = C.create_string_buffer(max(576 * n, 1)); st = C.create_string_buffer(max(n, 1))
        self._chk(self.lib.nbls_multi_pairing_batch(self.h, n, g1_aff, g2_aff, int(with_final_exp), int(validate), out, st))
        return out.raw[:576 * n], st.raw[:n]

    def miller_product(self, g1_aff, g2_aff, final_exp=True, validate=False):
        n = len(g1_aff) // 96
        out = C.create_string_buffer(576); st = C.create_string_buffer(max(n, 1))
# ... 9 lines not shown
```

Baseline: 2.579 million pairings/s.

## Fuse final-exponentiation tail expx with fe_final into chained AOT launches

Adds a new extra program, fe_final12, that is compiled into the expx AOT kernel so the last expx and the final-exponentiation finish can run as one chained launch. An optional mode also pairs each expx with the following mid step in a single chained launch. The pooled-context default turns both modes on, which cuts kernel launches and the HBM round trips for the Fp12 intermediates in the final exponentiation. In exchange the expx kernel grows and now carries extra signatures, which could raise register or LDS pressure for the plain expx path.

```diff
diff --git a/include/nbls.h b/include/nbls.h
--- a/include/nbls.h
+++ b/include/nbls.h
@@ -290,12 +290,14 @@
 #define NBLS_TUNE_MSMB_SLAB 18
 #define NBLS_TUNE_CELLS_CHUNK 20
 #define NBLS_TUNE_G16_CHUNK 22
+#define NBLS_TUNE_FE_TAIL_CHAIN 24
 int nbls_set_tuning(nbls_ctx* ctx, int key, long long value);
 int nbls_program_count(void);
 const char* nbls_program_name(int prog);
 const char* nbls_program_kernel(nbls_ctx* ctx, int prog);
 const char* nbls_extra_program_kernel(nbls_ctx* ctx, const char* name);
 long long nbls_extra_program_launches(nbls_ctx* ctx, const char* name);
+long long nbls_chain_launches(nbls_ctx* ctx);
 int nbls_aot_kernel_private_bytes(int k);
 int nbls_timing_enable(nbls_ctx* ctx, int on);
 int nbls_timing_read(nbls_ctx* ctx, float* ms , uint32_t* counts );
diff --git a/noble-bls12-381_amd/csrc/aot.h b/noble-bls12-381_amd/csrc/aot.h
--- a/noble-bls12-381_amd/csrc/aot.h
+++ b/noble-bls12-381_amd/csrc/aot.h
@@ -6,7 +6,7 @@
 
 #define NBLS_AOT_PARTS 8
 #define NBLS_AOT_KERNELS(X)                                                  \
-  X(0, expx, P_EXPX, P_FE_MID1, P_FE_MID2, P_COUNT)                          \
+  X(0, expx, P_EXPX, P_FE_MID1, P_FE_MID2, extra_key(XP_FE_FINAL12))         \
   X(0, acc_fe, P_ACC_FE, P_ACC_RAW, P_ACC_BYTES, P_COUNT)                    \
   X(0, lines_pq, P_LINES_PQ, P_COUNT, P_COUNT, P_COUNT)                      \
   X(0, acc4_raw, P_ACC4_RAW, P_ACC8_RAW, P_ACC2_RAW, P_COUNT)                \
diff --git a/noble-bls12-381_amd/csrc/aot_gen.cpp b/noble-bls12-381_amd/csrc/aot_gen.cpp
--- a/noble-bls12-381_amd/csrc/aot_gen.cpp
+++ b/noble-bls12-381_amd/csrc/aot_gen.cpp
@@ -35,6 +35,7 @@
   };
   for (ProgId id : hot) place(get_program(id));
   place(get_extra_program(XP_LINES_FE));
+  place(get_extra_program(XP_FE_FINAL12));
   fclose(f);
   return 0;
 }
@@ -56,7 +57,7 @@
       printf("\n");
     }
   };
-#define HIST(PART, NAME, P0, P1, P2, P3) { std::vector<const Program*> progs; for (ProgId id : {P0, P1, P2, P3}) if (id != P_COUNT) progs.push_back(&get_program(id)); emit(#NAME, progs); }
+#define HIST(PART, NAME, P0, P1, P2, P3) { std::vector<const Program*> progs; for (ProgId id : {P0, P1, P2, P3}) if (id != P_COUNT) progs.push_back(&program_by_key(id)); emit(#NAME, progs); }
   NBLS_AOT_KERNELS(HIST)
 #undef HIST
 #define HIST(PART, NAME, E0, E1) { std::vector<const Program*> progs; for (ExtraProg id : {E0, E1}) if (id != XP_COUNT) progs.push_back(&get_extra_program(id)); emit(#NAME, progs); }
@@ -96,7 +97,7 @@
 #define GEN(PART, NAME, P0, P1, P2, P3)                                                            \
   {                                                                                                \
     std::vector<const Program*> progs;                                                             \
-    for (ProgId id : {P0, P1, P2, P3}) if (id != P_COUNT) progs.push_back(&get_program(id));       \
+    for (ProgId id : {P0, P1, P2, P3}) if (id != P_COUNT) progs.push_back(&program_by_key(id));    \
     emit(#NAME, progs);                                                                            \
   }
   NBLS_AOT_KERNELS(GEN)
diff --git a/noble-bls12-381_amd/csrc/aot_kernel.hip b/noble-bls12-381_amd/csrc/aot_kernel.hip
--- a/noble-bls12-381_amd/csrc/aot_kernel.hip
+++ b/noble-bls12-381_amd/csrc/aot_kernel.hip
@@ -155,7 +155,10 @@
     if (!attr_set[dev].load(std::memory_order_acquire)) {
       std::lock_guard<std::mutex> g(attr_mu);
       if (!attr_set[dev].load(std::memory_order_relaxed)) {
-        for (int i = 0; i < g_nkernels; i++) (void)hipFuncSetAttribute(g_kernels[i].fn, hipFuncAttributeMaxDynamicSharedMemorySize, 160 * 1024);
+        for (int i = 0; i < g_nkernels; i++) {
+          const hipError_t e = hipFuncSetAttribute(g_kernels[i].fn, hipFuncAttributeMaxDynamicSharedMemorySize, 160 * 1024);
+          if (e != hipSuccess) { (void)hipGetLastError(); return (int)e; }
+        }
         attr_set[dev].store(true, std::memory_order_release);
       }
     }
diff --git a/noble-bls12-381_amd/csrc/aot_layout.inc b/noble-bls12-381_amd/csrc/aot_layout.inc
--- a/noble-bls12-381_amd/csrc/aot_layout.inc
+++ b/noble-bls12-381_amd/csrc/aot_layout.inc
@@ -66,3 +66,5 @@
 AOT_LAYOUT_ROW(g2_to_affine, 8, 8, 9, 0xfdb5a3b2u)
 AOT_LAYOUT_POS(lines_fe, 4, 7, 3, 15, 20, 0, 14, 23, 12, 25, 6, 11, 19, 13, 22, 17, 1, 9, 2, 21, 5, 18, 8, 10, 24, 16, 21, 22, 11, 4, 20, 25, 12, 5, 8, 0, 10, 24, 23, 13, 1, 15, 16, 7, 18, 19, 6, 17, 3, 2, 14, 9, 18, 9, 12, 16, 3, 11, 20, 0, 23, 13, 10, 8, 21, 2, 14, 6, 5, 22, 7, 19, 25, 15, 17, 4, 24, 1, 7, 3, 20, 8, 1, 19, 5, 22, 15, 25, 17, 21, 2, 13, 9, 14, 16, 0, 18, 12, 4, 11, 24, 23, 10, 6, 6, 19, 23, 5, 14, 21, 4, 7, 24, 22, 12, 13, 10, 11, 3, 9, 17, 15, 18, 8, 20, 2, 25, 16, 0, 1, 23, 1, 14, 18, 2, 16, 12, 20, 24, 25, 4, 7, 10, 21, 17, 0, 19, 9, 11, 5, 15, 3, 6, 22, 8, 13)
 AOT_LAYOUT_ROW(lines_fe, 6, 26, 286, 0x5d3bf329u)
+AOT_LAYOUT_POS(fe_final12, 31, 11, 3, 2, 21, 14, 34, 32, 16, 13, 10, 4, 5, 19, 6, 26, 25, 33, 15, 9, 28, 24, 8, 35, 18, 12, 27, 17, 29, 23, 22, 20, 7, 1, 0, 30, 1, 29, 25, 24, 26, 15, 13, 35, 30, 11, 21, 34, 28, 9, 5, 4, 6, 12, 8, 27, 22, 7, 3, 20, 0, 23, 14, 16, 17, 10, 31, 19, 32, 18, 2, 33, 24, 12, 14, 9, 0, 13, 11, 5, 25, 18, 32, 3, 7, 34, 8, 35, 27, 2, 26, 16, 17, 10, 30, 6, 19, 33, 20, 31, 4, 21, 28, 1, 22, 23, 29, 15, 6, 3, 1, 0, 27, 4, 22, 23, 8, 11, 34, 5, 16, 12, 10, 17, 26, 31, 32, 30, 15, 33, 9, 24, 28, 35, 25, 2, 29, 7, 21, 18, 19, 13, 20, 14, 19, 30, 3, 26, 13, 14, 29, 24, 22, 21, 1, 32, 17, 11, 9, 20, 33, 6, 15, 31, 34, 28, 27, 7, 25, 18, 23, 8, 10, 2, 35, 16, 12, 4, 5, 0)
+AOT_LAYOUT_ROW(fe_final12, 5, 36, 59, 0xc559c939u)
diff --git a/noble-bls12-381_amd/csrc/aot_sigs.inc b/noble-bls12-381_amd/csrc/aot_sigs.inc
--- a/noble-bls12-381_amd/csrc/aot_sigs.inc
+++ b/noble-bls12-381_amd/csrc/aot_sigs.inc
@@ -1,21 +1,25 @@
 #define AOT_SIGS_expx(X) \
-  X(0, 4, 0, 0x00, 0, 0x00000000u, 0x00000000u, 10) \
-  X(1, 12, 1, 0x00, 0, 0x00000000u, 0x00000000u, 1) \
-  X(2, 2, 2, 0x00, 0, 0x00000000u, 0x00000000u, 11) \
+  X(0, 4, 0, 0x00, 0, 0x00000000u, 0x00000000u, 19) \
+  X(1, 12, 1, 0x00, 0, 0x00000000u, 0x00000000u, 4) \
+  X(2, 2, 2, 0x00, 0, 0x00000000u, 0x00000000u, 22) \
   X(3, 12, 3, 0x04, 1, 0x000a0a0bu, 0x00000000u, 2) \
-  X(4, 12, 6, 0x04, 0, 0x020a0a0au, 0x00000002u, 5) \
-  X(5, 2, 3, 0x08, 1, 0x00000000u, 0x00000000u, 5) \
-  X(6, 12, 3, 0x04, 1, 0x000a0a0au, 0x00000000u, 7) \
+  X(4, 12, 6, 0x04, 0, 0x020a0a0au, 0x00000002u, 11) \
+  X(5, 2, 3, 0x08, 1, 0x00000000u, 0x00000000u, 6) \
+  X(6, 12, 3, 0x04, 1, 0x000a0a0au, 0x00000000u, 15) \
   X(7, 12, 3, 0x0c, 1, 0x000a0a0bu, 0x00000000u, 61) \
   X(8, 12, 1, 0x04, 0, 0x00000002u, 0x00000000u, 1) \
   X(9, 5, 0, 0x00, 0, 0x00000000u, 0x00000000u, 5) \
   X(10, 12, 2, 0x0e, 1, 0x00000a0bu, 0x00000000u, 2) \
   X(11, 12, 6, 0x0e, 1, 0x020a0a0au, 0x00000202u, 1) \
-  X(12, 2, 2, 0x00, 1, 0x00000000u, 0x00000000u, 1) \
+  X(12, 2, 2, 0x00, 1, 0x00000000u, 0x00000000u, 3) \
   X(13, 12, 6, 0x04, 1, 0x020a0a0au, 0x00000002u, 2) \
-  X(14, 2, 3, 0x00, 1, 0x00000000u, 0x00000000u, 2) \
+  X(14, 2, 3, 0x00, 1, 0x00000000u, 0x00000000u, 9) \
   X(15, 2, 2, 0x08, 0, 0x00000000u, 0x00000000u, 2) \
-  X(16, 12, 6, 0x0e, 1, 0x020a0a0au, 0x00000002u, 1)
+  X(16, 12, 6, 0x0e, 1, 0x020a0a0au, 0x00000002u, 1) \
+  X(17, 12, 2, 0x04, 0, 0x00000002u, 0x00000000u, 6) \
+  X(18, 2, 1, 0x00, 1, 0x00000000u, 0x00000000u, 3) \
+  X(19, 12, 6, 0x04, 0, 0x020a0a0au, 0x00000202u, 2) \
+  X(20, 3, 0, 0x00, 0, 0x00000000u, 0x00000000u, 1)
 #define AOT_SIGS_acc_fe(X) \
   X(0, 4, 0, 0x00, 0, 0x00000000u, 0x00000000u, 105) \
   X(1, 12, 5, 0x04, 0, 0x020a0a0au, 0x00000000u, 3) \
diff --git a/noble-bls12-381_amd/csrc/config.h b/noble-bls12-381_amd/csrc/config.h
--- a/noble-bls12-381_amd/csrc/config.h
+++ b/noble-bls12-381_amd/csrc/config.h
@@ -4,4 +4,5 @@
 long env_long(const char* name, long dflt);
 bool env_set(const char* name);
 std::string env_describe();
+inline unsigned fe_tail_chain_default(unsigned unset) { const long v = env_long("NBLS_FE_TAIL_CHAIN", -1); return v < 0 ? unset : (unsigned)v & 3u; }
 }
diff --git a/noble-bls12-381_amd/csrc/nbls_internal.h b/noble-bls12-381_amd/csrc/nbls_internal.h
--- a/noble-bls12-381_amd/csrc/nbls_internal.h
+++ b/noble-bls12-381_amd/csrc/nbls_internal.h
@@ -182,6 +182,8 @@
   size_t inv_wide_max = (size_t)env_long("NBLS_INV_WIDE_MAX", 4096);
   size_t ls_max = ::ls_max(), ls2_max = ::ls2_max();
   size_t chain_max = (size_t)env_long("NBLS_CHAIN_MAX", 8192);
+  unsigned fe_tail_chain = fe_tail_chain_default(0);
+  unsigned long long chain_launches = 0;
   u32* qp_table = nullptr;
   uint8_t* kzg_tables[26 + 13 * 7] = {nullptr};
   uint8_t* unit_lines = nullptr;
diff --git a/noble-bls12-381_amd/csrc/nbls_multi.cpp b/noble-bls12-381_amd/csrc/nbls_multi.cpp
--- a/noble-bls12-381_amd/csrc/nbls_multi.cpp
+++ b/noble-bls12-381_amd/csrc/nbls_multi.cpp
@@ -209,6 +209,7 @@
   return NBLS_OK;
 }
 
+static const unsigned POOL_FE_TAIL_CHAIN = 3;
 static int g_queues_set_by_library = 0;
 __attribute__((constructor)) static void nbls_on_load() {
   if (getenv("NBLS_KEEP_HW_QUEUES")) return;
@@ -243,6 +244,7 @@
       nbls_set_tuning(c, NBLS_TUNE_SPLIT_MILLER_MIN, 0);
       if (nbls::env_long("NBLS_PIPELINE_CHAIN", 0) != 1) nbls_set_tuning(c, NBLS_TUNE_CHAIN_MAX, 0);
       nbls_set_tuning(c, NBLS_TUNE_LS_MAX, 0); nbls_set_tuning(c, NBLS_TUNE_LS2_MAX, 0);
+      nbls_set_tuning(c, NBLS_TUNE_FE_TAIL_CHAIN, nbls::fe_tail_chain_default(POOL_FE_TAIL_CHAIN));
       nbls_set_tuning(c, NBLS_TUNE_INV_WIDE_MAX, 256);
     }
   }
diff --git a/noble-bls12-381_amd/csrc/pipelines_pairing.cpp b/noble-bls12-381_amd/csrc/pipelines_pairing.cpp
--- a/noble-bls12-381_amd/csrc/pipelines_pairing.cpp
+++ b/noble-bls12-381_amd/csrc/pipelines_pairing.cpp
@@ -38,12 +38,21 @@
                             {P_EXPX, {B(3, T[4], F12), B(5, T[6], F12)}},
                             {P_FE_MID2, {B(3, T[6], F12), B(5, T[1], F12), B(6, T[5], F12)}},
                             {P_EXPX, {B(3, T[5], F12), B(5, T[6], F12)}}};
-  if (n < ctx->expc_min && n < ctx->chain_max && !w.beside && ls_variant(ctx, P_EXPX, n) == P_EXPX && !wide_applies(ctx, ctx->prog[P_EXPX], (int)P_EXPX, n)) {
+  const BufList fin = {B(0, T[0], F12), B(1, T[1], F12), B(2, T[2], F12), B(3, T[3], F12), B(4, T[4], F12), B(5, T[5], F12), B(6, T[6], F12), B(7, d_out, 576)};
+  const bool plain_expx = n < ctx->expc_min && ls_variant(ctx, P_EXPX, n) == P_EXPX && !wide_applies(ctx, ctx->prog[P_EXPX], (int)P_EXPX, n);
+  if (plain_expx && n < ctx->chain_max && !w.beside) {
     if ((r = run_chain(ctx, n, mid, 7, s))) return r;
-  } else for (const ChainLink& l : mid) {
-    if ((r = l.id == P_EXPX ? expx(ctx, w, n, (uint8_t*)l.bufs.a[0].ptr, (uint8_t*)l.bufs.a[1].ptr, s) : run(ctx, l.id, n, l.bufs, s))) return r;
-  }
-  return run(ctx, P_FE_FINAL, n, {B(0, T[0], F12), B(1, T[1], F12), B(2, T[2], F12), B(3, T[3], F12), B(4, T[4], F12), B(5, T[5], F12), B(6, T[6], F12), B(7, d_out, 576)}, s);
+    return run(ctx, P_FE_FINAL, n, fin, s);
+  }
+  const unsigned tail = plain_expx ? ctx->fe_tail_chain : 0u;
+  for (int k = 0; k < 7; k++) {
+    const ChainLink& l = mid[k];
+    if (l.id != P_EXPX) { if ((r = run(ctx, l.id, n, l.bufs, s))) return r; continue; }
+    if (k == 6 && (tail & 1)) { const ChainLink last[2] = {l, {extra_key(XP_FE_FINAL12), fin}}; return run_chain(ctx, n, last, 2, s); }
+    if ((tail & 2) && k < 6 && mid[k + 1].id != P_EXPX) { if ((r = run_chain(ctx, n, mid + k, 2, s))) return r; k++; continue; }
+    if ((r = expx(ctx, w, n, (uint8_t*)l.bufs.a[0].ptr, (uint8_t*)l.bufs.a[1].ptr, s))) return r;
+  }
+  return run(ctx, P_FE_FINAL, n, fin, s);
 }
 int finish_single(nbls_ctx* ctx, const Window& w, uint8_t* f_raw, int final_exp, void* d_out, hipStream_t s) {
   int r;
diff --git a/noble-bls12-381_amd/csrc/programs.cpp b/noble-bls12-381_amd/csrc/programs.cpp
--- a/noble-bls12-381_amd/csrc/programs.cpp
+++ b/noble-bls12-381_amd/csrc/programs.cpp
@@ -213,6 +213,7 @@
 static const int MILLER_W = env_int("NBLS_MILLER_W", 16);
 static const int G1_W = env_int("NBLS_G1_W", 4), G2_W = env_int("NBLS_G2_W", 8), G2MUL_W = env_int("NBLS_G2MUL_W", 8), G1MUL_W = env_int("NBLS_G1MUL_W", 4);
 static const int EXPX_W = env_int("NBLS_EXPX_W", 12);
+static const int FE_FINAL12_WINDOW = 50;
 static const int LINES_W = env_int("NBLS_LINES_W", 10), ACC_W = env_int("NBLS_ACC_W", 12), ACC_WINDOW = env_int("NBLS_ACC_WINDOW", 330);
 
 static bool aot_listed(ProgId id) {
@@ -863,6 +864,11 @@
     trace_lines_fe(Px, Py, Qx, Qy, 3);
     return B.compile("lines_fe", LINES_W);
   }
+  if (id == XP_FE_FINAL12) {
+    B.sched_window = env_int("NBLS_FE_FINAL12_WINDOW", FE_FINAL12_WINDOW);
+    output_fp12(trace_fe_final_chain([&](int i) { return inputw_fp12(i - 1, 0); }), 7, 0);
+    return B.compile("fe_final12", 12);
+  }
   if (id == XP_DBLADD_G1) {
     auto ld = [&](int buf) { return Pt<SFp>{inputw(buf, 0), inputw(buf, 48), inputw(buf, 96)}; };
     Pt<SFp> r = pt_add(pt_dbl(ld(3)), ld(4));
diff --git a/noble-bls12-381_amd/csrc/programs.h b/noble-bls12-381_amd/csrc/programs.h
--- a/noble-bls12-381_amd/csrc/programs.h
+++ b/noble-bls12-381_amd/csrc/programs.h
@@ -81,9 +81,13 @@
 static const int MSM_WINDOW_BITS = 12;
 const Program& get_program(ProgId id);
 const Program* get_tower_program(int field, int op, int param, int part);
-enum ExtraProg { XP_POLY_G1_16 = 0, XP_POLY_G1_256, XP_POLY_G2_16, XP_POLY_G2_256, XP_DBLADD_G1, XP_DBLADD_G2, XP_LINES_FE, XP_ENDO_G1, XP_COUNT };
+enum ExtraProg { XP_POLY_G1_16 = 0, XP_POLY_G1_256, XP_POLY_G2_16, XP_POLY_G2_256, XP_DBLADD_G1, XP_DBLADD_G2, XP_LINES_FE, XP_ENDO_G1, XP_FE_FINAL12, XP_COUNT };
+static inline ProgId extra_key(ExtraProg e) { return (ProgId)((int)P_COUNT + 1 + (int)e); }
+static inline bool key_is_extra(ProgId id) { return (int)id > (int)P_COUNT; }
+static inline ExtraProg key_extra(ProgId id) { return (ExtraProg)((int)id - (int)P_COUNT - 1); }
 static const int XP_NUMBERED = XP_DBLADD_G1;
 const Program& get_extra_program(ExtraProg id);
+static inline const Program& program_by_key(ProgId id) { return key_is_extra(id) ? get_extra_program(key_extra(id)) : get_program(id); }
 bool lines_fe_enabled();
 void print_stats(const Program& p);
 }
diff --git a/noble-bls12-381_amd/csrc/runtime.cpp b/noble-bls12-381_amd/csrc/runtime.cpp
--- a/noble-bls12-381_amd/csrc/runtime.cpp
+++ b/noble-bls12-381_amd/csrc/runtime.cpp
@@ -135,23 +135,31 @@
   int r;
   bool fuse = chains_enabled() && !checked_mode() && count <= (size_t)AOT_MAX_SEGS;
   int k = -1; u32 W = 0, G = 0, lds = 0;
+  auto dev = [&](const ChainLink* l) -> DevProgram& { return key_is_extra(l->id) ? ctx->extra[key_extra(l->id)] : ctx->prog[l->id]; };
   for (const ChainLink* l = links; l < links + count; l++) {
-    if ((r = upload(ctx, l->id))) return r;
-    const DevProgram& d = ctx->prog[l->id];
+    if ((r = key_is_extra(l->id) ? upload_extra(ctx, key_extra(l->id)) : upload(ctx, l->id))) return r;
+    const DevProgram& d = dev(l);
     if (d.aot < 0 || (k >= 0 && (d.aot != k || d.p->W != W || d.p->G != G))) fuse = false;
     k = d.aot; W = d.p->W; G = d.p->G; lds = std::max(lds, d.aot_lds);
   }
-  if (!fuse) { for (const ChainLink* l = links; l < links + count; l++) if ((r = run(ctx, l->id, n, l->bufs, s))) return r; return NBLS_OK; }
+  if (!fuse) {
+    for (const ChainLink* l = links; l < links + count; l++)
+      if ((r = key_is_extra(l->id) ? run_dev(ctx, dev(l), -1, n, l->bufs, s, nullptr, nullptr) : run(ctx, l->id, n, l->bufs, s))) return r;
+    return NBLS_OK;
+  }
   AotArgs a; memset(&a, 0, sizeof a);
   for (const ChainLink* l = links; l < links + count; l++) {
     IOBuf bufs[MAX_BUFS];
     if (!bind_bufs(bufs, l->bufs)) return NBLS_EINVAL;
-    aot_seg(a.seg[a.nseg++], ctx->prog[l->id], bufs);
+    DevProgram& d = dev(l);
+    d.launches++;
+    aot_seg(a.seg[a.nseg++], d, bufs);
   }
   a.W = W; a.G = G; a.n_items = (u32)n; a.qp_table = ctx->qp_table;
   int e;
-  { Timed timed(ctx, (int)links->id, s); e = nbls_aot_launch(k, &a, lds, s); }
+  { Timed timed(ctx, key_is_extra(links->id) ? -1 : (int)links->id, s); e = nbls_aot_launch(k, &a, lds, s); }
   if (e) { ctx->last_hip = e; return NBLS_EHIP; }
+  ctx->chain_launches++;
   return NBLS_OK;
 }
 
diff --git a/noble-bls12-381_amd/csrc/tuning.cpp b/noble-bls12-381_amd/csrc/tuning.cpp
--- a/noble-bls12-381_amd/csrc/tuning.cpp
+++ b/noble-bls12-381_amd/csrc/tuning.cpp
@@ -130,6 +130,7 @@
     case NBLS_TUNE_MSMB_SLAB: if (value < 0) return NBLS_EINVAL; ctx->msmb_slab = (size_t)value; return NBLS_OK;
     case NBLS_TUNE_CELLS_CHUNK: if (value < 0) return NBLS_EINVAL; ctx->cells_chunk = (size_t)value; return NBLS_OK;
     case NBLS_TUNE_G16_CHUNK: if (value < 0) return NBLS_EINVAL; ctx->g16_chunk = (size_t)value; return NBLS_OK;
+    case NBLS_TUNE_FE_TAIL_CHAIN: if (value < 0 || value > 3) return NBLS_EINVAL; ctx->fe_tail_chain = (unsigned)value; return NBLS_OK;
     default: return NBLS_EINVAL;
   }
 }
@@ -157,6 +158,7 @@
   for (int i = 0; i < (int)XP_COUNT; i++) if (get_extra_program((ExtraProg)i).name == name) return (long long)ctx->extra[i].launches;
   return -1;
 }
+EXPORT long long nbls_chain_launches(nbls_ctx* ctx) { if (!ctx) return -1; std::lock_guard<std::recursive_mutex> g(ctx->mu); return (long long)ctx->chain_launches; }
 EXPORT int nbls_aot_kernel_private_bytes(int k) { return nbls_aot_private_bytes(k); }
 EXPORT int nbls_program_count(void) { return (int)P_COUNT; }
 EXPORT const char* nbls_program_name(int prog) { return prog >= 0 && prog < P_COUNT ? get_program((ProgId)prog).name.c_str() : nullptr; }
diff --git a/noble-bls12-381_amd/engine.py b/noble-bls12-381_amd/engine.py
--- a/noble-bls12-381_amd/engine.py
+++ b/noble-bls12-381_amd/engine.py
@@ -982,6 +982,9 @@
     def set_chain_max(self, n):
         self._chk(self.lib.nbls_set_tuning(self.h, 4, n))
 
+    def set_fe_tail_chain(self, bits):
+        self._chk(self.lib.nbls_set_tuning(self.h, 24, int(bits)))
+
     def set_sac_max(self, n):
         self._chk(self.lib.nbls_set_tuning(self.h, 8, n))
 
@@ -1045,6 +1048,11 @@
         self.lib.nbls_extra_program_launches.restype = C.c_longlong
         self.lib.nbls_extra_program_launches.argtypes = [C.c_void_p, C.c_char_p]
         return self.lib.nbls_extra_program_launches(self.h, name.encode())
+
+    def chain_launches(self):
+        self.lib.nbls_chain_launches.restype = C.c_longlong
+        self.lib.nbls_chain_launches.argtypes = [C.c_void_p]
+        return self.lib.nbls_chain_launches(self.h)
 
     def kernel_bindings(self):
         return {p: self.program_kernel(p) for p in PROGRAMS}
```

Measured after the change: 2.635 million pairings/s (median of 6 runs). +2.2%, better.
